# SkyTNT/midi-model

Hardware: AMD Instinct MI355X
Metric: MIDI events/sec, training step (fwd+bwd+clip+AdamW), tv2o-medium, seq=2048 (higher is better)
Workload: dtype bf16; 1 GPU; tv2o-medium bf16 training step, per-GPU batch 16 x 2048 events x 8 tokens (BASELINE.json configs[1]); random-init weights, synthetic events; global_batch=16, seq_len=2048, parallelism=dp1, accumulate_grad_batches=1, optimizer=AdamW bf16-true + global-norm clip 1.0

## Files before the change

### include/midihip.h

```cpp
#ifndef MIDIHIP_H
#define MIDIHIP_H
#include <stdint.h>
#ifdef __cplusplus
extern "C" {
#endif

#define MH_F32 0
#define MH_BF16 1

#define MH_OK 0
#define MH_ERR_ARG (-1)
#define MH_ERR_LAUNCH (-2)
#define MH_ERR_UNSUPPORTED (-3)

const char* mh_last_error(void);
int mh_version(void);
int mh_ab_builds(void);
int mh_set_option(const char* name, int value);
int mh_get_option(const char* name);

int mh_gemm_nt(const void* A, int64_t lda, const void* B, int64_t ldb, void* C, int64_t ldc, const void* R,
               int64_t ldr, int64_t M, int64_t N, int64_t K, float alpha, float beta, int dtype, int splitk,
               void* workspace, void* stream);
int mh_gemm(const void* A, int64_t lda, int transA, const void* B, int64_t ldb, int transB, void* C, int64_t ldc,
            const void* R, int64_t ldr, int64_t M, int64_t N, int64_t K, float alpha, float beta, int dtype, int splitk,
            void* workspace, void* stream);
int mh_gemm_swiglu(const void* A, int64_t lda, const void* W, int64_t ldw, void* GU, int64_t ldgu, void* ACT,
                   int64_t ldact, int64_t M, int64_t I, int64_t K, int dtype, void* stream);
int mh_gemm_rope(const void* A, int64_t lda, const void* W, int64_t ldw, void* C, int64_t ldc, const void* table,
                 int64_t npos, int64_t S, int64_t pos0, int head_dim, int64_t M, int64_t N, int64_t K, int dtype, void* stream);
int mh_gemm_dswiglu(const void* A, int64_t lda, const void* B, int64_t ldb, const void* GU, int64_t ldgu, void* DGU,
                    int64_t lddgu, int64_t M, int64_t I, int64_t K, int dtype, void* stream);
int mh_gemm_rowss(const void* A, int64_t lda, const void* B, int64_t ldb, void* C, int64_t ldc, const void* R, int64_t ldr,
                  float* rowss, int64_t M, int64_t N, int64_t K, int dtype, void* stream);
int mh_row_rstd(const void* x, int64_t ldx, const float* parts, int nparts, int64_t M, int D, float eps, float* rstd, int dtype,
                void* stream);
int mh_gemm_rope_scaled(const void* A, int64_t lda, const void* W, int64_t ldw, void* C, int64_t ldc, const void* table,
                        int64_t npos, int64_t S, int64_t pos0, int head_dim, const float* rowscale, int64_t M, int64_t N, int64_t K,
                        int dtype, void* stream);
int mh_gemm_swiglu_scaled(const void* A, int64_t lda, const void* W, int64_t ldw, void* GU, int64_t ldgu, void* ACT, int64_t ldact,
                          const float* rowscale, int64_t M, int64_t I, int64_t K, int dtype, void* stream);
int mh_gemm_nt_scaled(const void* A, int64_t lda, const void* B, int64_t ldb, void* C, int64_t ldc, const float* rowscale, int64_t M,
                      int64_t N, int64_t K, int dtype, void* stream);
int mh_gemm_dswiglu_scaled(const void* A, int64_t lda, const void* B, int64_t ldb, const void* GU, int64_t ldgu, void* DGU,
                           int64_t lddgu, const float* rowscale, int64_t M, int64_t I, int64_t K, int dtype, void* stream);
int mh_splitk_fold_blocks(int64_t M);
int mh_gemm_splitk_reduce_fold(const void* workspace, void* C, int64_t ldc, const void* R, int64_t ldr, int64_t M, int64_t N,
                               int splitk, float alpha, float beta, const void* wnorm, const void* W, int64_t ldw, float* colpart,
                               int dtype, void* stream);
int mh_rmsnorm_bwd_folded(const void* x, const float* rstd, const void* t, const void* dres, void* dx, int64_t M, int D, int dtype,
                          void* stream);
int mh_scale_cols(const void* W, int64_t ldw, const void* w, void* out, int64_t ldo, int64_t Nr, int K, int dtype, void* stream);
int mh_scale_cols_batched(const int64_t* jobs, int njobs, int K, int dtype, void* stream);
int mh_gemm_splitk_reduce(const void* workspace, void* C, int64_t ldc, const void* R, int64_t ldr, int64_t M,
                          int64_t N, int splitk, float alpha, float beta, int dtype, void* stream);
#define MH_SKINNY_PLAIN 0
#define MH_SKINNY_GATEUP 1
int mh_gemm_skinny(const void* A, int64_t lda, const void* W, int64_t ldw, void* C, int64_t ldc, const void* R,
                   int64_t ldr, int mode, float norm_eps, const int64_t* row_ids, const int64_t* res_ids, int64_t M,
                   int64_t N, int64_t K, int dtype, void* stream);
int mh_transpose(const void* in, int64_t ldi, void* out, int64_t ldo, int64_t rows, int64_t cols, int dtype,
                 void* stream);

int mh_embed_sum_fwd(const int64_t* tok, const void* table, void* out, int64_t M, int T, int64_t V, int D,
                     int dtype, void* stream);
int mh_concat_tok_fwd(const void* hidden, const int64_t* tok, int64_t ldtok, const void* table, void* out,
                      int64_t M, int T, int64_t V, int D, int dtype, void* stream);
int mh_embed_scatter_bwd(const int64_t* tok, int64_t ldtok, int T, const void* dout, int rows_per_m, int jstride,
                         int j0, float* dtable_f32, int64_t M, int64_t V, int D, int64_t pad_id, int dtype,
                         void* stream);
int mh_embed_segment_bwd(const int64_t* src_rows, const int64_t* seg_start, const void* dout, int64_t ld,
                         float* dtable_f32, int64_t V, int D, int64_t n_occ, int64_t pad_id, int dtype, void* stream);
int mh_token_segments_chunk(void);
int mh_token_segments(const int64_t* tok, int64_t ldtok, int64_t n_rows, int n_cols, int64_t V, int64_t row_mul,
                      int64_t col_mul, int64_t add, int64_t* src_rows, int64_t* seg_start, int32_t* work, void* stream);
int mh_cast_from_f32(const float* src, void* dst, int64_t n, int accumulate, int dtype, void* stream);
int mh_copy_rows(const void* src, int64_t src_ld, void* dst, int64_t dst_ld, int64_t M, int D, int accumulate,
                 int dtype, void* stream);

int mh_collate_windows(const int16_t* tokens, int64_t n_events, const int64_t* win_start, const int64_t* win_len,
                       int64_t* out, int64_t B, int64_t L, int T, int64_t pad_id, void* stream);

int mh_augment_piece_stats(const int16_t* tokens, const int64_t* piece_off, int64_t n_pieces, const int32_t* tab,
                           int32_t* stats, void* stream);
int mh_augment_collate_windows(const int16_t* tokens, int64_t n_events, const int64_t* win_start, const int64_t* win_len,
                               const int64_t* win_piece, const int32_t* shifts, const int32_t* stats, const int32_t* tab,
                               int64_t* out, int64_t B, int64_t L, int T, int64_t pad_id, void* stream);

int mh_rmsnorm_fwd(const void* x, const void* w, void* y, float* rstd, int64_t M, int D, float eps, int dtype,
                   void* stream);
int mh_rmsnorm_bwd_blocks(int64_t M);
int mh_rmsnorm_bwd(const void* x, const void* w, const float* rstd, const void* dy, const void* dres, void* dx,
                   float* dw_partial, int64_t M, int D, int dtype, void* stream);
int mh_colsum(float* partial , int64_t nblk, void* out, int D, int accumulate, int dtype, void* stream);

int mh_rope(void* qkv, const float* cos_t, const float* sin_t, int64_t M, int64_t S, int64_t pos0, int H, int hd,
            int dir, int dtype, void* stream);

int mh_attn_prep_fwd(const void* qkv, void* vt, int64_t B, int64_t S, int H, int dtype, void* stream);
int mh_attn_fwd(const void* qkv, const void* vt, void* o, float* lse, int64_t B, int64_t S, int H, float scale,
                int dtype, void* stream);
int mh_attn_prep_bwd(const void* qkv, const void* o, const void* dout, float* delta, void* qt, void* kt, void* dot,
                     int64_t B, int64_t S, int H, int dtype, void* stream);
int mh_attn_bwd(const void* qkv, const void* dout, const float* lse, const float* delta, const void* qt,
                const void* kt, const void* dot, void* dqkv, int64_t B, int64_t S, int H, float scale,
                const float* cos_t, const float* sin_t, int dtype, void* stream);
int mh_attn_bwd_o(const void* qkv, const void* o, const void* dout, const float* lse, float* delta, void* dqkv, int64_t B,
                  int64_t S, int H, float scale, const float* cos_t, const float* sin_t, int dtype, void* stream);
int mh_attn_bwd_o_scaled(const void* qkv, const void* o, const void* dout, const float* lse, float* delta, void* dqkv,
                         const float* rowscale, int64_t B, int64_t S, int H, float scale, const float* cos_t, const float* sin_t,
                         int dtype, void* stream);
int mh_attn_fwd_timeline(const void* qkv, void* o, float* lse, int64_t B, int64_t S, int H, float scale, int lazy,
                         uint32_t* stamps, void* stream);
int mh_attn_fwd_plain(const void* qkv, void* o, float* lse, int64_t B, int64_t S, int H, float scale, int dtype,
                      void* stream);
int mh_attn_bwd_plain(const void* qkv, const void* dout, const float* lse, const float* delta, void* dqkv, int64_t B,
                      int64_t S, int H, float scale, int dtype, void* stream);

int mh_tokattn_fwd(const void* qkv, void* o, int64_t N, int T, int H, float scale, const float* cos_t, const float* sin_t,
                   int dtype, void* stream);
int mh_tokattn_bwd(const void* qkv, const void* dout, void* dqkv, int64_t N, int T, int H, float scale, const float* cos_t,
                   const float* sin_t, int dtype, void* stream);
int mh_tokattn_bwd_scaled(const void* qkv, const void* dout, void* dqkv, const float* rowscale, int64_t N, int T, int H, float scale,
                          const float* cos_t, const float* sin_t, int dtype, void* stream);

int mh_swiglu_fwd(const void* gu, void* a, int64_t M, int I, int dtype, void* stream);
int mh_swiglu_bwd(const void* gu, const void* da, void* dgu, int64_t M, int I, int dtype, void* stream);

int mh_cross_entropy(const void* logits, int64_t ldl, const int64_t* target, float* row_loss, void* dlogits,
                     const float* scale_dev, int64_t* argmax_out, int64_t R, int V, int64_t ignore, int dtype,
                     void* stream);
int mh_sum_f32(const float* x, int64_t n, float* out, void* stream);
int mh_count_valid(const int64_t* target, int64_t n, int64_t ignore, float* count, float* inv, void* stream);

int mh_sumsq(const void* g, int64_t n, float* partial1024, float* out, int accumulate, int dtype, void* stream);
int mh_clip_coef(const float* sumsq, float max_norm, float* coef, float* norm, void* stream);
int mh_adamw(void* p, const void* g, void* m, void* v, int64_t n, float lr, float beta1, float beta2, float eps,
             float weight_decay, float bias_corr1, float bias_corr2, const float* coef_dev, int dtype, void* stream);
int mh_adamw_master(float* p32, void* p_lo, const float* g32, float* m, float* v, int64_t n, float lr, float beta1,
                    float beta2, float eps, float weight_decay, float bias_corr1, float bias_corr2, const float* coef_dev,
                    int dtype_lo, void* stream);
int mh_grad_fold_f32(const void* src, float* dst, int64_t n, int accumulate, int dtype, void* stream);

int mh_kv_append(void* qkv, const float* cos_t, const float* sin_t, void* kcache, void* vcache, int64_t B, int H,
                 int hd, int64_t Lmax, int64_t pos, const int32_t* pos_dev, int dtype, void* stream);
int mh_attn_decode(const void* qkv, const void* kcache, const void* vcache, void* o, int64_t B, int H, int hd,
                   int64_t Lmax, int64_t len, float scale, const int32_t* pos_dev, int dtype, void* stream);
int mh_attn_decode_append(const void* qkv, const float* cos_t, const float* sin_t, void* kcache, void* vcache, void* o,
                          int64_t B, int H, int hd, int64_t Lmax, int64_t pos, float scale, const int32_t* pos_dev,
                          int dtype, void* stream);
#define MH_ATTN_PREFIX_CHUNK 256
int mh_attn_prefix_chunk(void);
int mh_attn_prefix_partial(const void* qkv, const float* cos_t, const float* sin_t, const void* kpre, const void* vpre,
                           float* ws, int64_t ws_floats, int64_t B, int H, int hd, int64_t Pmax, int64_t pre_len, int64_t pos,
                           float scale, const int32_t* pre_len_dev, const int32_t* pos_dev, int dtype, void* stream);
int mh_attn_decode_append_shared(const void* qkv, const float* cos_t, const float* sin_t, void* ksuf, void* vsuf,
                                 const float* ws, int64_t ws_floats, void* o, int64_t B, int H, int hd, int64_t Lsuf,
                                 int64_t Pmax, int64_t pre_len, int64_t pos, float scale, const int32_t* pre_len_dev,
                                 const int32_t* pos_dev, int dtype, void* stream);
int mh_kv_store_rows(const void* qkv, void* kcache, void* vcache, int64_t B, int64_t S, int H, int hd, int64_t Lmax,
                     int64_t pos0, int dtype, void* stream);
int mh_kv_gather_rows(const void* kcache, const void* vcache, void* qkv, int64_t B, int64_t n, int64_t Stot, int H, int hd,
                      int64_t Lmax, int dtype, void* stream);
int mh_attn_fwd_tail(const void* qkv, void* o, float* lse, int64_t B, int64_t S, int H, float scale, int64_t q_start,
                     int dtype, void* stream);
int mh_kv_store_prefill(const void* qkv, void* kcache, void* vcache, int64_t B, int64_t S, int H, int hd,
                        int64_t Lmax, int dtype, void* stream);

int mh_masked_softmax(const void* logits, int64_t ldl, const int32_t* lo, const int32_t* hi,
                      const uint8_t* first_mask, float* probs, int64_t B, int V, float temp, int dtype,
                      void* stream);
int mh_sample_top_p_k(const void* logits, int64_t ldl, const uint8_t* first_mask, const uint8_t* ban_mask, int first_lo,
                      int first_hi,
                      const int32_t* lo_tab, const int32_t* hi_tab, int tab_stride, int max_range, const int64_t* ev,
                      int pos, const float* q, int64_t* out,
                      int64_t out_stride, int64_t* out_b, int64_t* out_c, int64_t B, int V, float temp, float top_p,
                      int top_k, int fill_rest, int64_t fill_id, int dtype, void* stream);
// ... 13 lines not shown
```

### midi-model_amd/csrc/attention_mfma3.hip

```cpp
#include <stdlib.h>

#include "attn_mfma_common.h"

static int attn_env_int(const char* name, int dflt) {
  const char* v = getenv(name);
  return (v && *v) ? atoi(v) : dflt;
}
thread_local int g_attn_v3 = attn_env_int("MH_ATTN_V3", 255);
thread_local int g_attn_passes = attn_env_int("MH_ATTN_PASSES", 5);
thread_local int g_attn_v3_wps = attn_env_int("MH_ATTN_V3_WPS", 0);
thread_local const float* g_attn_bwd_rowscale = nullptr;

__device__ inline bf16x8 ldsv(const char* p) { return *reinterpret_cast<const bf16x8*>(p); }
typedef __attribute__((ext_vector_type(2))) float f32x2;
typedef __attribute__((ext_vector_type(2))) __bf16 bf16x2;
__device__ inline bf16x8 pack8_pk(const f32x16& v, int base) {
  union {
    bf16x8 v;
    bf16x2 h[4];
  } r;
#pragma unroll
  for (int i = 0; i < 4; ++i) r.h[i] = __builtin_convertvector(f32x2{v[base + 2 * i], v[base + 2 * i + 1]}, bf16x2);
  return r.v;
}
__device__ inline float xhalf_max(float v) {
  const int iv = __float_as_int(v);
  const auto pr = __builtin_amdgcn_permlane32_swap(iv, iv, false, false);
  return fmaxf(__int_as_float(pr[0]), __int_as_float(pr[1]));
}

constexpr float LZ_BOUND = 1099511627776.f;
__device__ inline uint64_t tl_now() {
  uint64_t t;
  asm volatile("s_memtime %0" : "=s"(t));
  return t;
}
template <bool MASK, bool TR, bool LZ = false, bool TL = false>
__device__ inline void fwd3_tile(const char* tK, const char* tV, const int (&trof)[2][2], const int (&foff)[4],
                                 const bf16x8 (&qf)[4], f32x16 (&oacc)[2], float& m, float& l, int hi, int qrel, float sc,
                                 uint64_t* ts = nullptr) {
  bf16x8 kf[2][4];
#pragma unroll
  for (int s = 0; s < 4; ++s)
#pragma unroll
    for (int kb = 0; kb < 2; ++kb) kf[kb][s] = ldsv(tK + foff[s] + kb * 4096);
  __builtin_amdgcn_sched_barrier(0);
  if constexpr (TL) ts[2] = tl_now();
  f32x16 sacc[2] = {zero16(), zero16()};
#pragma unroll
  for (int s = 0; s < 4; ++s)
#pragma unroll
    for (int kb = 0; kb < 2; ++kb) sacc[kb] = mfma32(kf[kb][s], qf[s], sacc[kb]);
  bf16x8 vf[4][2];
  u32x2 vr[4][2][2];
  if (TR) {
    unsigned tv[2][2];
#pragma unroll
    for (int db = 0; db < 2; ++db)
#pragma unroll
      for (int half = 0; half < 2; ++half) tv[db][half] = lds_addr32(tV) + (unsigned)trof[db][half];
#pragma unroll
    for (int db = 0; db < 2; ++db)
#pragma unroll
// ... 338 lines not shown
  } else {
#pragma unroll
    for (int t = 0; t < 2; ++t)
#pragma unroll
      for (int hb = 0; hb < 2; ++hb) ktf[t][hb] = ldsv(tKT + foff[2 * KB + t] + hb * 4096);
  }
  __builtin_amdgcn_sched_barrier(0);
#pragma unroll
  for (int r = 0; r < 16; ++r) {
    float p = fast_exp2(__builtin_fmaf(sacc[r], sc, -lse2));
    if (MASK) {
      if (KB * 32 + 16 * (r >> 3) + (r & 7) > qrel - 8 * hi) p = 0.f;
    }
    sacc[r] = p * pacc[r];
  }
  const bf16x8 dsf0 = pack8_pk(sacc, 0), dsf1 = pack8_pk(sacc, 8);
  if (TR) {
    asm volatile("s_waitcnt lgkmcnt(0)" ::: "memory");
    __builtin_amdgcn_sched_barrier(0);
#pragma unroll
    for (int hb = 0; hb < 2; ++hb) dqacc[hb] = mfma32(join8(kr[0][hb][0], kr[0][hb][1]), dsf0, dqacc[hb]);
#pragma unroll
    for (int hb = 0; hb < 2; ++hb) dqacc[hb] = mfma32(join8(kr[1][hb][0], kr[1][hb][1]), dsf1, dqacc[hb]);
  } else {
#pragma unroll
    for (int hb = 0; hb < 2; ++hb) dqacc[hb] = mfma32(ktf[0][hb], dsf0, dqacc[hb]);
#pragma unroll
    for (int hb = 0; hb < 2; ++hb) dqacc[hb] = mfma32(ktf[1][hb], dsf1, dqacc[hb]);
  }
}

template <bool MASK, bool TR>
__device__ inline void dq3_tile(const char* tK, const char* tV, const char* tKT, const int (&trof)[2][2], const int (&foff)[4],
                                const bf16x8 (&qf)[4], const bf16x8 (&dof)[4], f32x16 (&dqacc)[2], int hi, int qrel, float sc,
                                float lse2, const f32x16& dlt) {
  unsigned tkt[2][2];
#pragma unroll
  for (int hb = 0; hb < 2; ++hb)
#pragma unroll
    for (int half = 0; half < 2; ++half) tkt[hb][half] = lds_addr32(tK) + (unsigned)trof[hb][half];
  dq3_half<MASK, TR, 0>(tK, tV, tKT, tkt, foff, qf, dof, dqacc, hi, qrel, sc, lse2, dlt);
  dq3_half<MASK, TR, 1>(tK, tV, tKT, tkt, foff, qf, dof, dqacc, hi, qrel, sc, lse2, dlt);
}

template <int WPS, bool TR>
__global__ __launch_bounds__(256, WPS) void attn_bwd_dq3_kernel(const bf16* __restrict__ qkv, const bf16* __restrict__ dout,
                                                              const float* __restrict__ lse, const float* __restrict__ delta,
                                                              const bf16* __restrict__ kt_, bf16* __restrict__ dqkv, int S,
                                                              int Sp, int H, float scale, int BH, int nqt,
                                                              const float* __restrict__ cos_t,
                                                              const float* __restrict__ sin_t,
                                                              const bf16* __restrict__ o_ ,
                                                              float* __restrict__ delta_w,
                                                              const float* __restrict__ rowscale ) {
  extern __shared__ __attribute__((aligned(16))) char smem[];
  constexpr int NT = TR ? 2 : 3;
  const int tid = threadIdx.x, lane = tid & 63;
  const int wave = __builtin_amdgcn_readfirstlane(tid >> 6);
  int bh_, tile_;
  if (!attn_work(BH, nqt, bh_, tile_)) return;
  const int64_t bh = bh_;
  const int64_t b = bh / H;
  const int h = (int)(bh - b * H);
  const int64_t D = (int64_t)H * HD, D3 = 3 * D;
  const int q0 = (nqt - 1 - tile_) * 128;
  const int qw0 = q0 + wave * 32;
  const int li = lane & 31, hi = lane >> 5;
  const int qrow = qw0 + li;
  const int qld = (qrow < S) ? qrow : S - 1;
  const float sc = scale * LOG2E;

  const bf16* kbase = qkv + b * S * D3 + D + (int64_t)h * HD;
  const bf16* vbase = kbase + D;
  const bf16* ktbase = TR ? nullptr : kt_ + bh * HD * Sp;

  bf16x8 qf[4], dof[4];
  float dl = 0.f;
  {
    const bf16* qp = qkv + (b * S + qld) * D3 + (int64_t)h * HD + 8 * hi;
    const bf16* dp = dout + (b * S + qld) * D + (int64_t)h * HD + 8 * hi;
    bf16x8 of[4];
    if (o_ != nullptr) {
      const bf16* op = o_ + (b * S + qld) * D + (int64_t)h * HD + 8 * hi;
#pragma unroll
      for (int s = 0; s < 4; ++s) of[s] = *reinterpret_cast<const bf16x8*>(op + 16 * s);
    }
#pragma unroll
    for (int s = 0; s < 4; ++s) {
      qf[s] = *reinterpret_cast<const bf16x8*>(qp + 16 * s);
      const bf16x8 d = *reinterpret_cast<const bf16x8*>(dp + 16 * s);
#pragma unroll
      for (int e = 0; e < 8; ++e) dof[s][e] = -d[e];
      if (o_ != nullptr) {
#pragma unroll
        for (int e = 0; e < 8; ++e) dl = __builtin_fmaf((float)d[e], (float)of[s][e], dl);
      }
    }
  }
  float lse2 = lse[bh * Sp + qld] * LOG2E;
  if (o_ != nullptr) {
    dl += __shfl_xor(dl, 32, 64);
    if (hi == 0 && qrow < S) {
      delta_w[bh * Sp + qrow] = dl;
      delta_w[(int64_t)BH * Sp + bh * Sp + qrow] = -lse2;
    }
  } else {
    dl = delta[bh * Sp + qld];
// ... 12 lines not shown
  {
    const int pli = pi32(li);
#pragma unroll
    for (int s = 0; s < 4; ++s) foff[s] = lds_tile_off(pli, 2 * s + hi);
  }

  const int iD3 = (int)D3;
  int trof[2][2];
  tr_frag_offsets(lane, trof);
  stage64u(kbase, iD3, 0, S - 1, 0, smem, wave, lane);
  stage64u(vbase, iD3, 0, S - 1, 0, smem + TILE64, wave, lane);
  if (!TR) stage64u(ktbase, Sp, 0, HD - 1, 0, smem + 2 * TILE64, wave, lane);
#pragma unroll
  for (int s = 0; s < 4; ++s) {
    asm volatile("" : "+v"(qf[s]));
    asm volatile("" : "+v"(dof[s]));
  }
  asm volatile("" : "+v"(lse2));
  asm volatile("" : "+v"(dlt));
  stage_wait_all();
    __syncthreads();
  auto stage_next = [&](int kt) {
    if (kt + 1 <= kt_last) {
      char* nxt = smem + ((kt + 1) & 1) * NT * TILE64;
      stage64u(kbase, iD3, (kt + 1) * 64, S - 1, 0, nxt, wave, lane);
      stage64u(vbase, iD3, (kt + 1) * 64, S - 1, 0, nxt + TILE64, wave, lane);
      if (!TR) stage64u(ktbase, Sp, 0, HD - 1, (kt + 1) * 64, nxt + 2 * TILE64, wave, lane);
    }
  };
  int kt = 0;
  for (; kt < n_full; ++kt) {
    stage_next(kt);
    const char* cur = smem + (kt & 1) * NT * TILE64;
    dq3_tile<false, TR>(cur, cur + TILE64, cur + 2 * TILE64, trof, foff, qf, dof, dqacc, hi, 0, sc, lse2, dlt);
    stage_wait_all();
    __syncthreads();
  }
  if (kt <= kt_last) {
    stage_next(kt);
    const char* cur = smem + (kt & 1) * NT * TILE64;
    dq3_tile<true, TR>(cur, cur + TILE64, cur + 2 * TILE64, trof, foff, qf, dof, dqacc, hi, qrow - kt * 64, sc, lse2, dlt);
    stage_wait_all();
    __syncthreads();
    ++kt;
  }
  for (; kt <= kt_last; ++kt) {
    stage_next(kt);
    stage_wait_all();
    __syncthreads();
  }
  if (qrow < S) {
    bf16* orow = dqkv + (b * S + qrow) * D3 + (int64_t)h * HD;
    const float rsc = rowscale != nullptr ? rowscale[b * S + qrow] : 1.f;
    store_grad_row(orow, dqacc, -scale * rsc, hi, cos_t, sin_t, qrow);
  }
}

template <bool MASK, bool TR, int QB, bool PS>
__device__ inline void dkv3_half(const char* tQ, const char* tDO, const char* tQT, const char* tDOT, const char* tLD,
                                 const unsigned (&tq)[2][2], const unsigned (&tdo)[2][2], const int (&foff)[4],
                                 const bf16x8 (&kf)[4], const bf16x8 (&vf)[4] , f32x16 (&dkacc)[2], f32x16 (&dvacc)[2],
                                 int hi, int krel, int qlim, float sc) {
  bf16x8 qf[4], dof[4];
#pragma unroll
  for (int s = 0; s < 4; ++s) {
    qf[s] = ldsv(tQ + foff[s] + QB * 4096);
    dof[s] = ldsv(tDO + foff[s] + QB * 4096);
  }
  __builtin_amdgcn_sched_barrier(0);
  f32x16 pacc;
#pragma unroll
  for (int i = 0; i < 4; ++i) {
    const f32x4 d4 = *reinterpret_cast<const f32x4*>(tLD + 1024 + (QB * 32 + 16 * (i >> 1) + 8 * hi + 4 * (i & 1)) * 4);
#pragma unroll
    for (int e = 0; e < 4; ++e) pacc[4 * i + e] = d4[e];
  }
  __builtin_amdgcn_sched_barrier(0);
  f32x16 sacc = zero16();
#pragma unroll
  for (int s = 0; s < 4; ++s) {
    sacc = mfma32(qf[s], kf[s], sacc);
    pacc = mfma32(dof[s], vf[s], pacc);
  }
  bf16x8 dotf[2][2], qtf[2][2];
  u32x2 dor[2][2][2], qr[2][2][2];
  f32x4 la[2][2];
#define MH_DKV_REQUEST(T)                                                                      \
  {                                                                                            \
    if (TR) {                                                                                  \
      _Pragma("unroll") for (int xb = 0; xb < 2; ++xb) _Pragma("unroll") for (int half = 0; half < 2; ++half) { \
        dor[T][xb][half] = ds_tr16<(2 * QB + (T)) * 2048>(tdo[xb][half]);                      \
        qr[T][xb][half] = ds_tr16<(2 * QB + (T)) * 2048>(tq[xb][half]);                        \
      }                                                                                        \
    } else {                                                                                   \
      _Pragma("unroll") for (int xb = 0; xb < 2; ++xb) {                                       \
        dotf[T][xb] = ldsv(tDOT + foff[2 * QB + (T)] + xb * 4096);                             \
        qtf[T][xb] = ldsv(tQT + foff[2 * QB + (T)] + xb * 4096);                               \
      }                                                                                        \
    }                                                                                          \
    _Pragma("unroll") for (int v4 = 0; v4 < 2; ++v4)                                           \
        la[T][v4] = *reinterpret_cast<const f32x4*>(tLD + (QB * 32 + 16 * (T) + 8 * hi + 4 * v4) * 4); \
  }
  MH_DKV_REQUEST(0)
  __builtin_amdgcn_sched_barrier(0);
#pragma unroll
  for (int t = 0; t < 2; ++t) {
#pragma unroll
// ... 2 lines not shown
      for (int e = 0; e < 4; ++e) {
        const int r = 8 * t + 4 * v4 + e;
        float p = fast_exp2(__builtin_fmaf(sacc[r], sc, PS ? la[t][v4][e] : -la[t][v4][e] * LOG2E));
        float ds = p * pacc[r];
        if (MASK) {
          const int q = QB * 32 + 16 * t + 4 * v4 + e;
          const bool ok = (q >= krel - 8 * hi) && (q < qlim - 8 * hi);
          p = ok ? p : 0.f;
          ds = ok ? ds : 0.f;
        }
        sacc[r] = p;
        pacc[r] = ds;
      }
    const bf16x8 pf = pack8_pk(sacc, 8 * t), dsf = pack8_pk(pacc, 8 * t);
    if (t == 0) {
      MH_DKV_REQUEST(1)
      if (TR) asm volatile("s_waitcnt lgkmcnt(10)" ::: "memory");
    } else if (TR) {
      asm volatile("s_waitcnt lgkmcnt(0)" ::: "memory");
    }
    __builtin_amdgcn_sched_barrier(0);
#pragma unroll
    for (int xb = 0; xb < 2; ++xb) {
      dvacc[xb] = mfma32(TR ? join8(dor[t][xb][0], dor[t][xb][1]) : dotf[t][xb], pf, dvacc[xb]);
      dkacc[xb] = mfma32(TR ? join8(qr[t][xb][0], qr[t][xb][1]) : qtf[t][xb], dsf, dkacc[xb]);
    }
  }
#undef MH_DKV_REQUEST
}

template <bool MASK, bool TR, bool PS>
__device__ inline void dkv3_tile(const char* tQ, const char* tDO, const char* tQT, const char* tDOT, const char* tLD,
                                 const int (&trof)[2][2], const int (&foff)[4], const bf16x8 (&kf)[4], const bf16x8 (&vf)[4],
                                 f32x16 (&dkacc)[2], f32x16 (&dvacc)[2], int hi, int krel, int qlim, float sc) {
  unsigned tq[2][2], tdo[2][2];
#pragma unroll
  for (int xb = 0; xb < 2; ++xb)
#pragma unroll
    for (int half = 0; half < 2; ++half) {
      tq[xb][half] = lds_addr32(tQ) + (unsigned)trof[xb][half];
      tdo[xb][half] = lds_addr32(tDO) + (unsigned)trof[xb][half];
    }
  dkv3_half<MASK, TR, 0, PS>(tQ, tDO, tQT, tDOT, tLD, tq, tdo, foff, kf, vf, dkacc, dvacc, hi, krel, qlim, sc);
  dkv3_half<MASK, TR, 1, PS>(tQ, tDO, tQT, tDOT, tLD, tq, tdo, foff, kf, vf, dkacc, dvacc, hi, krel, qlim, sc);
}

template <bool TR, bool PS = false >
__global__ __launch_bounds__(256, 2) void attn_bwd_dkv3_kernel(const bf16* __restrict__ qkv, const bf16* __restrict__ dout,
                                                               const float* __restrict__ lse, const float* __restrict__ delta,
                                                               const bf16* __restrict__ qt_, const bf16* __restrict__ dot_,
                                                               bf16* __restrict__ dqkv, int S, int Sp, int H, float scale,
                                                               int BH, int nkt, const float* __restrict__ cos_t,
                                                               const float* __restrict__ sin_t,
                                                               const float* __restrict__ rowscale ) {
  constexpr int NT = TR ? 2 : 4, STG = NT * TILE64 + 2048;
  extern __shared__ __attribute__((aligned(16))) char smem[];
  const int tid = threadIdx.x, lane = tid & 63;
  const int wave = __builtin_amdgcn_readfirstlane(tid >> 6);
  int bh_, tile_;
  if (!attn_work(BH, nkt, bh_, tile_)) return;
  const int64_t bh = bh_;
  const int64_t b = bh / H;
  const int h = (int)(bh - b * H);
  const int64_t D = (int64_t)H * HD, D3 = 3 * D;
  const int k0 = tile_ * 128;
  const int kw0 = k0 + wave * 32;
  const int li = lane & 31, hi = lane >> 5;
  const int krow = kw0 + li;
  const int kld = (krow < S) ? krow : S - 1;
  const float sc = scale * LOG2E;

  const bf16* qbase = qkv + b * S * D3 + (int64_t)h * HD;
  const bf16* dobase = dout + b * S * D + (int64_t)h * HD;
  const bf16* qtbase = TR ? nullptr : qt_ + bh * HD * Sp;
  const bf16* dotbase = TR ? nullptr : dot_ + bh * HD * Sp;
  const float* lse_b = lse + bh * Sp;
  const float* delta_b = delta + bh * Sp;

  bf16x8 kf[4], vf[4];
  {
    const bf16* kp = qkv + (b * S + kld) * D3 + D + (int64_t)h * HD + 8 * hi;
#pragma unroll
    for (int s = 0; s < 4; ++s) {
      kf[s] = *reinterpret_cast<const bf16x8*>(kp + 16 * s);
      const bf16x8 v = *reinterpret_cast<const bf16x8*>(kp + D + 16 * s);
#pragma unroll
      for (int e = 0; e < 8; ++e) vf[s][e] = -v[e];
    }
  }
  f32x16 dkacc[2] = {zero16(), zero16()}, dvacc[2] = {zero16(), zero16()};
  int foff[4];
  {
    const int pli = pi32(li);
#pragma unroll
    for (int s = 0; s < 4; ++s) foff[s] = lds_tile_off(pli, 2 * s + hi);
  }
  const int qt_first = k0 / 64, qt_last = (S - 1) / 64;

  auto stage_all = [&](int qt, char* dst) {
    stage64u(qbase, (int)D3, qt * 64, S - 1, 0, dst, wave, lane);
    stage64u(dobase, (int)D, qt * 64, S - 1, 0, dst + TILE64, wave, lane);
    if (!TR) {
      stage64u(qtbase, Sp, 0, HD - 1, qt * 64, dst + 2 * TILE64, wave, lane);
      stage64u(dotbase, Sp, 0, HD - 1, qt * 64, dst + 3 * TILE64, wave, lane);
    }
    if (wave < 2) {
      const float* base = (wave == 0 ? lse_b : delta_b) + (int64_t)qt * 64;
// ... 3 lines not shown
  int trof[2][2];
  tr_frag_offsets(lane, trof);
  if (qt_first <= qt_last) stage_all(qt_first, smem);
#pragma unroll
  for (int s = 0; s < 4; ++s) {
    asm volatile("" : "+v"(kf[s]));
    asm volatile("" : "+v"(vf[s]));
  }
  stage_wait_all();
    __syncthreads();
  const int nT = qt_last - qt_first + 1;
  const int a = kw0 >> 6;
  int n_skip = a - qt_first;
  if (n_skip > nT) n_skip = nT;
  const int n_mask = (a <= qt_last) ? 1 : 0;
  int n_full = ((S >> 6) < qt_last + 1 ? (S >> 6) : qt_last + 1) - (a + 1);
  if (n_full < 0) n_full = 0;
  const int n_tail = nT - n_skip - n_mask - n_full;
  int qt = qt_first;
  auto head = [&](int q) {
    if (q + 1 <= qt_last) stage_all(q + 1, smem + (((q - qt_first) & 1) ^ 1) * STG);
    return smem + ((q - qt_first) & 1) * STG;
  };
  for (int i = 0; i < n_skip; ++i, ++qt) {
    head(qt);
    stage_wait_all();
    __syncthreads();
  }
  if (n_mask) {
    const char* cur = head(qt);
    dkv3_tile<true, TR, PS>(cur, cur + TILE64, cur + 2 * TILE64, cur + 3 * TILE64, cur + NT * TILE64, trof, foff, kf, vf, dkacc, dvacc, hi,
                    krow - qt * 64, S - qt * 64, sc);
    stage_wait_all();
    __syncthreads();
    ++qt;
  }
  for (int i = 0; i < n_full; ++i, ++qt) {
    const char* cur = head(qt);
    dkv3_tile<false, TR, PS>(cur, cur + TILE64, cur + 2 * TILE64, cur + 3 * TILE64, cur + NT * TILE64, trof, foff, kf, vf, dkacc, dvacc, hi, 0,
                     64, sc);
    stage_wait_all();
    __syncthreads();
  }
  if (n_tail > 0) {
    const char* cur = head(qt);
    dkv3_tile<true, TR, PS>(cur, cur + TILE64, cur + 2 * TILE64, cur + 3 * TILE64, cur + NT * TILE64, trof, foff, kf, vf, dkacc, dvacc, hi,
                    krow - qt * 64, S - qt * 64, sc);
    stage_wait_all();
    __syncthreads();
  }
  if (krow < S) {
    bf16* krow_out = dqkv + (b * S + krow) * D3 + D + (int64_t)h * HD;
    const float rsc = rowscale != nullptr ? rowscale[b * S + krow] : 1.f;
    store_grad_row(krow_out, dkacc, -scale * rsc, hi, cos_t, sin_t, krow);
    store_grad_row(krow_out + D, dvacc, rsc, hi, nullptr, nullptr, 0);
  }
}

int mh_attn_fwd_mfma3(const void* qkv, const void* vt, void* o, float* lse, int64_t B, int64_t S, int H, float scale,
                      hipStream_t st, int64_t q_start) {
  MH_REQUIRE(S * 3 * H * HD < (int64_t(1) << 31), "attn_fwd: sequence too long (32-bit panel offsets)");
  MH_REQUIRE(q_start >= 0 && q_start < S, "attn_fwd: q_start %ld outside the sequence", (long)q_start);
  const int64_t Sp = (S + 63) / 64 * 64;
  const int nt_all = (int)((S + 127) / 128), BH0 = (int)(B * H);
  MH_REQUIRE(BH0 < (1 << 24), "attn_fwd: too many (batch, head) pairs");
  const int BH = BH0 | ((g_attn_passes & 127) << 24);
  const int nt = nt_all - (int)(q_start / 128);
  const unsigned grid = (unsigned)(nt * 8 * ((BH0 + 7) / 8));
#define MH_FWD(WPS, TR_, LZ_)                                                                                                    \
  attn_fwd3_kernel<WPS, TR_, 2, LZ_><<<grid, 256, 4 * TILE64, st>>>((const bf16*)qkv, (const bf16*)vt, (bf16*)o, lse, (int)S, (int)Sp, H, \
                                                                 scale * LOG2E, BH, nt, nt_all)
#define MH_FWD3S(WPS, TR_, LZ_)                                                                                                  \
  attn_fwd3_kernel<WPS, TR_, 3, LZ_><<<grid, 256, 6 * TILE64, st>>>((const bf16*)qkv, (const bf16*)vt, (bf16*)o, lse, (int)S, (int)Sp, \
                                                                  H, scale * LOG2E, BH, nt, nt_all)
  const bool tr = (vt == nullptr);
  const bool lz = (g_attn_v3 & 128) != 0;
  if (tr && g_attn_v3_wps == 4) {
    if (lz) MH_FWD(4, true, true); else MH_FWD(4, true, false);
  } else if (tr && (g_attn_v3 & 64)) {
    if (lz) {
      if (g_attn_v3_wps == 3) MH_FWD3S(3, true, true); else MH_FWD3S(2, true, true);
    } else {
      if (g_attn_v3_wps == 3) MH_FWD3S(3, true, false); else MH_FWD3S(2, true, false);
    }
  } else if (tr) {
    if (g_attn_v3_wps == 3) MH_FWD(3, true, false); else MH_FWD(2, true, false);
  } else {
    if (g_attn_v3_wps == 2) MH_FWD(2, false, false); else MH_FWD(3, false, false);
  }
#undef MH_FWD
#undef MH_FWD3S
  MH_LAUNCH_CHECK();
  return MH_OK;
}

extern "C" int mh_attn_fwd_timeline(const void* qkv, void* o, float* lse, int64_t B, int64_t S, int H, float scale, int lazy,
                                    uint32_t* stamps, void* stream) {
#ifdef MH_AB_BUILDS
  MH_REQUIRE(stamps != nullptr && S >= 128 && S * 3 * H * HD < (int64_t(1) << 31), "attn_fwd_timeline: bad arguments");
  hipStream_t st = (hipStream_t)stream;
  const int64_t Sp = (S + 63) / 64 * 64;
  const int nt_all = (int)((S + 127) / 128), BH0 = (int)(B * H), nt = nt_all;
  const int BH = BH0 | ((g_attn_passes & 127) << 24);
  const unsigned grid = (unsigned)(nt * 8 * ((BH0 + 7) / 8));
  if (lazy)
    attn_fwd3_kernel<2, true, 3, true, true><<<grid, 256, 6 * TILE64 + TL_BYTES, st>>>((const bf16*)qkv, (const bf16*)stamps, (bf16*)o, lse, (int)S,
                                                                                   (int)Sp, H, scale * LOG2E, BH, nt, nt_all);
  else
    attn_fwd3_kernel<2, true, 3, false, true><<<grid, 256, 6 * TILE64 + TL_BYTES, st>>>((const bf16*)qkv, (const bf16*)stamps, (bf16*)o, lse, (int)S,
                                                                                    (int)Sp, H, scale * LOG2E, BH, nt, nt_all);
  MH_LAUNCH_CHECK();
  return MH_OK;
#else
  mh_set_error("attn_fwd_timeline: only in the A/B library (libmidihip_ab.so)");
  return MH_ERR_UNSUPPORTED;
#endif
}

int mh_attn_bwd_mfma3(const void* qkv, const void* dout, const float* lse, const float* delta, const void* qt, const void* kt,
                      const void* dot, void* dqkv, int64_t B, int64_t S, int H, float scale, const float* cos_t,
                      const float* sin_t, int which ,
                      hipStream_t st, const void* o ) {
  MH_REQUIRE(o == nullptr || (which & 14) == 14, "attn_bwd: delta inside the dQ kernel needs the third form of both kernels");
  MH_REQUIRE(S * 3 * H * HD < (int64_t(1) << 31), "attn_bwd: sequence too long (32-bit panel offsets)");
  const bool tr = (which & 8) != 0;
  MH_REQUIRE(tr || (qt != nullptr && kt != nullptr && dot != nullptr), "attn_bwd(bf16): needs the transposed copies (mh_attn_prep_bwd)");
  const int64_t Sp = (S + 63) / 64 * 64;
  const int nt = (int)((S + 127) / 128), BH0 = (int)(B * H);
  MH_REQUIRE(BH0 < (1 << 24), "attn_bwd: too many (batch, head) pairs");
  const int BH = BH0 | ((g_attn_passes & 127) << 24);
  const unsigned grid = (unsigned)(nt * 8 * ((BH0 + 7) / 8));
#define MH_DQ(WPS, TR_)                                                                                                     \
  attn_bwd_dq3_kernel<WPS, TR_><<<grid, 256, (TR_ ? 4 : 6) * TILE64, st>>>((const bf16*)qkv, (const bf16*)dout, lse, delta,     \
                                                                        (const bf16*)kt, (bf16*)dqkv, (int)S, (int)Sp, H, scale, \
                                                                        BH, nt, cos_t, sin_t, (const bf16*)o,         \
                                                                        const_cast<float*>(delta), g_attn_bwd_rowscale)
  if (which & 2) {
    if (g_attn_v3_wps == 2) {
      if (tr) MH_DQ(2, true); else MH_DQ(2, false);
    } else {
      if (tr) MH_DQ(3, true); else MH_DQ(3, false);
    }
    MH_LAUNCH_CHECK();
  }
#undef MH_DQ
  if (which & 4) {
    if (tr && o != nullptr)
      attn_bwd_dkv3_kernel<true, true><<<grid, 256, 2 * (2 * TILE64 + 2048), st>>>((const bf16*)qkv, (const bf16*)dout,
                                                                                 delta + (int64_t)BH0 * Sp, delta, nullptr, nullptr,
                                                                                 (bf16*)dqkv, (int)S, (int)Sp, H, scale, BH, nt,
                                                                                 cos_t, sin_t, g_attn_bwd_rowscale);
    else if (tr)
      attn_bwd_dkv3_kernel<true><<<grid, 256, 2 * (2 * TILE64 + 2048), st>>>((const bf16*)qkv, (const bf16*)dout, lse, delta, nullptr,
                                                                           nullptr, (bf16*)dqkv, (int)S, (int)Sp, H, scale, BH, nt,
                                                                           cos_t, sin_t, g_attn_bwd_rowscale);
    else
      attn_bwd_dkv3_kernel<false><<<grid, 256, 2 * DKV_STAGE, st>>>((const bf16*)qkv, (const bf16*)dout, lse, delta, (const bf16*)qt,
                                                                  (const bf16*)dot, (bf16*)dqkv, (int)S, (int)Sp, H, scale, BH, nt,
                                                                  cos_t, sin_t, g_attn_bwd_rowscale);
    MH_LAUNCH_CHECK();
  }
  return MH_OK;
}
```

### midi-model_amd/csrc/attention_small.hip

```cpp
#include "common.h"

#define DISPATCH_T(dtype, CALL)                                    \
  do {                                                             \
    if ((dtype) == MH_BF16) { using T = bf16; CALL; }              \
    else if ((dtype) == MH_F32) { using T = float; CALL; }         \
    else { mh_set_error("bad dtype %d", (int)(dtype)); return MH_ERR_ARG; } \
  } while (0)

template <typename T> __device__ inline void ld4(const T* p, float (&o)[4]);
template <> __device__ inline void ld4<float>(const float* p, float (&o)[4]) {
  f32x4 v = *reinterpret_cast<const f32x4*>(p);
  o[0] = v[0]; o[1] = v[1]; o[2] = v[2]; o[3] = v[3];
}
template <> __device__ inline void ld4<bf16>(const bf16* p, float (&o)[4]) {
  bf16x4 v = *reinterpret_cast<const bf16x4*>(p);
  o[0] = (float)v[0]; o[1] = (float)v[1]; o[2] = (float)v[2]; o[3] = (float)v[3];
}
template <typename T> __device__ inline void st4(T* p, const float (&o)[4]);
template <> __device__ inline void st4<float>(float* p, const float (&o)[4]) {
  *reinterpret_cast<f32x4*>(p) = f32x4{o[0], o[1], o[2], o[3]};
}
template <> __device__ inline void st4<bf16>(bf16* p, const float (&o)[4]) {
  bf16x4 v;
  v[0] = (bf16)o[0]; v[1] = (bf16)o[1]; v[2] = (bf16)o[2]; v[3] = (bf16)o[3];
// ... 86 lines not shown
      }
#pragma unroll
      for (int t = 0; t < TN; ++t) qraw[t] = ldraw<T>(base + t * D3, lane);
#pragma unroll
      for (int t = 0; t < TN; ++t) {
        unpack(kraw[t], k[t]);
        unpack(vraw[t], v[t]);
        if (rot) rope_row<T>(k[t], rope_c, rope_s, t, lane, 1.f, true);
      }
    } else {
#pragma unroll
      for (int t = 0; t < TK; ++t) {
        if (t < Tn) {
          ldp<T>(base + t * D3 + D, lane, k[t]);
          ldp<T>(base + t * D3 + 2 * D, lane, v[t]);
          if (rot) rope_row<T>(k[t], rope_c, rope_s, t, lane, 1.f, true);
        }
      }
    }
#pragma unroll
    for (int i = 0; i < TK; ++i) {
      if (TN ? i >= TN : i >= Tn) break;
      float q[4];
      if constexpr (TN != 0) unpack(qraw[i], q);
      else ldp<T>(base + i * D3, lane, q);
      if (rot) rope_row<T>(q, rope_c, rope_s, i, lane, 1.f, true);
      float s[TK];
      float mx = -INFINITY;
#pragma unroll
      for (int j = 0; j <= i; ++j) {
        float p = q[0] * k[j][0] + q[1] * k[j][1] + q[2] * k[j][2] + q[3] * k[j][3];
        s[j] = wave_sum_fast(p) * scale;
        mx = fmaxf(mx, s[j]);
      }
      float den = 0.f;
#pragma unroll
      for (int j = 0; j <= i; ++j) {
        s[j] = __expf(s[j] - mx);
        den += s[j];
      }
      const float inv = 1.f / den;
      float acc[4] = {0.f, 0.f, 0.f, 0.f};
#pragma unroll
      for (int j = 0; j <= i; ++j) {
        const float p = s[j] * inv;
#pragma unroll
        for (int e = 0; e < 4; ++e) acc[e] += p * v[j][e];
      }
      stp<T>(o + (n * Tn + i) * D + (int64_t)h * 256, lane, acc);
    }
  }
}

template <typename T, int TN, bool BR>
__global__ __launch_bounds__(256) void tokattn_bwd_kernel(const T* __restrict__ qkv, const T* __restrict__ dout,
                                                          T* __restrict__ dqkv, int64_t NH, int Tn, int H, float scale,
                                                          const float* __restrict__ cos_t, const float* __restrict__ sin_t,
                                                          const float* __restrict__ rowscale ) {
  const int lane = threadIdx.x & 63;
  const int64_t D = (int64_t)H * 256, D3 = 3 * D;
  __shared__ float rope_c[TK * 128], rope_s[TK * 128];
  const bool rot = cos_t != nullptr;
  if (rot) {
    for (int i = threadIdx.x; i < Tn * 128; i += 256) {
      rope_c[i] = rnd<T>(cos_t[i]);
      rope_s[i] = rnd<T>(sin_t[i]);
    }
    __syncthreads();
  }
  for (int64_t w = (int64_t)blockIdx.x * 4 + (threadIdx.x >> 6); w < NH; w += (int64_t)gridDim.x * 4) {
    const int64_t n = w / H;
    const int h = (int)(w - n * H);
    const int64_t off = (int64_t)h * 256;
    const T* base = qkv + n * Tn * D3 + off;
    T* ob = dqkv + n * Tn * D3 + off;
    float k[TK][4], v[TK][4], dk[TK][4], dv[TK][4];
    RawRow<T> qraw[TN ? TN : 1], doraw[TN ? TN : 1];
    const float rs_lane = (rowscale != nullptr && lane < Tn) ? rowscale[n * Tn + lane] : 1.f;
#pragma unroll
    for (int t = 0; t < TK; ++t)
#pragma unroll
      for (int e = 0; e < 4; ++e) dk[t][e] = dv[t][e] = 0.f;
    if constexpr (TN != 0) {
      RawRow<T> kraw[TN ? TN : 1], vraw[TN ? TN : 1];
#pragma unroll
      for (int t = 0; t < TN; ++t) {
        kraw[t] = ldraw<T>(base + t * D3 + D, lane);
        vraw[t] = ldraw<T>(base + t * D3 + 2 * D, lane);
      }
#pragma unroll
      for (int t = 0; t < TN; ++t) {
        qraw[t] = ldraw<T>(base + t * D3, lane);
        doraw[t] = ldraw<T>(dout + (n * Tn + t) * D + off, lane);
      }
#pragma unroll
      for (int t = 0; t < TN; ++t) {
        unpack(kraw[t], k[t]);
        unpack(vraw[t], v[t]);
        if (rot) rope_row<T>(k[t], rope_c, rope_s, t, lane, 1.f, true);
      }
    } else {
#pragma unroll
      for (int t = 0; t < TK; ++t) {
        if (t < Tn) {
          ldp<T>(base + t * D3 + D, lane, k[t]);
          ldp<T>(base + t * D3 + 2 * D, lane, v[t]);
          if (rot) rope_row<T>(k[t], rope_c, rope_s, t, lane, 1.f, true);
        }
      }
    }
#pragma unroll
    for (int i = 0; i < TK; ++i) {
      if (TN ? i >= TN : i >= Tn) break;
      float q[4], dO[4], dq[4] = {0.f, 0.f, 0.f, 0.f};
      if constexpr (TN != 0) {
        unpack(qraw[i], q);
        unpack(doraw[i], dO);
      } else {
        ldp<T>(base + i * D3, lane, q);
        ldp<T>(dout + (n * Tn + i) * D + off, lane, dO);
      }
      if (rot) rope_row<T>(q, rope_c, rope_s, i, lane, 1.f, true);
      float p[TK], dp[TK];
      float mx = -INFINITY;
      if constexpr (BR) {
#pragma unroll
        for (int j = 0; j <= i; j += 2) {
          const bool two = j + 1 <= i;
          const int j1 = two ? j + 1 : j;
          const float a0 = q[0] * k[j][0] + q[1] * k[j][1] + q[2] * k[j][2] + q[3] * k[j][3];
          const float b0 = dO[0] * v[j][0] + dO[1] * v[j][1] + dO[2] * v[j][2] + dO[3] * v[j][3];
          const float a1 = two ? q[0] * k[j1][0] + q[1] * k[j1][1] + q[2] * k[j1][2] + q[3] * k[j1][3] : 0.f;
          const float b1 = two ? dO[0] * v[j1][0] + dO[1] * v[j1][1] + dO[2] * v[j1][2] + dO[3] * v[j1][3] : 0.f;
          const float r4 = wave_sum4(a0, b0, a1, b1);
          p[j] = wave_sum4_get<0>(r4) * scale;
          dp[j] = wave_sum4_get<1>(r4);
          mx = fmaxf(mx, p[j]);
          if (two) {
            p[j1] = wave_sum4_get<2>(r4) * scale;
            dp[j1] = wave_sum4_get<3>(r4);
            mx = fmaxf(mx, p[j1]);
          }
        }
      } else {
#pragma unroll
      for (int j = 0; j <= i; ++j) {
        float a = q[0] * k[j][0] + q[1] * k[j][1] + q[2] * k[j][2] + q[3] * k[j][3];
        float b = dO[0] * v[j][0] + dO[1] * v[j][1] + dO[2] * v[j][2] + dO[3] * v[j][3];
        p[j] = wave_sum_fast(a) * scale;
        dp[j] = wave_sum_fast(b);
        mx = fmaxf(mx, p[j]);
      }
      }
      float den = 0.f;
#pragma unroll
      for (int j = 0; j <= i; ++j) {
        p[j] = __expf(p[j] - mx);
        den += p[j];
      }
      const float inv = 1.f / den;
      float dsum = 0.f;
#pragma unroll
      for (int j = 0; j <= i; ++j) {
        p[j] *= inv;
        dsum += p[j] * dp[j];
      }
#pragma unroll
      for (int j = 0; j <= i; ++j) {
        const float ds = p[j] * (dp[j] - dsum) * scale;
#pragma unroll
        for (int e = 0; e < 4; ++e) {
          dq[e] += ds * k[j][e];
          dk[j][e] += ds * q[e];
          dv[j][e] += p[j] * dO[e];
        }
      }
      if (rot) rope_row<T>(dq, rope_c, rope_s, i, lane, -1.f, false);
      if (rowscale != nullptr) {
        const float rsc = __shfl(rs_lane, i, 64);
#pragma unroll
        for (int e = 0; e < 4; ++e) dq[e] *= rsc;
      }
      stp<T>(ob + i * D3, lane, dq);
    }
#pragma unroll
    for (int t = 0; t < TK; ++t) {
      if (TN ? t < TN : t < Tn) {
        if (rot) rope_row<T>(dk[t], rope_c, rope_s, t, lane, -1.f, false);
        if (rowscale != nullptr) {
          const float rsc = __shfl(rs_lane, t, 64);
#pragma unroll
          for (int e = 0; e < 4; ++e) {
            dk[t][e] *= rsc;
            dv[t][e] *= rsc;
          }
        }
        stp<T>(ob + t * D3 + D, lane, dk[t]);
        stp<T>(ob + t * D3 + 2 * D, lane, dv[t]);
      }
    }
  }
}

extern "C" int mh_tokattn_fwd(const void* qkv, void* o, int64_t N, int Tn, int H, float scale, const float* cos_t,
                              const float* sin_t, int dtype, void* stream) {
  MH_REQUIRE(N > 0 && Tn >= 1 && Tn <= TK && H >= 1, "tokattn_fwd: bad shape N=%ld T=%d H=%d", (long)N, Tn, H);
  const int64_t NH = N * H;
  int64_t g = (NH + 3) / 4;
  if (g > 32768) g = 32768;
  if (Tn == TK)
    DISPATCH_T(dtype, (tokattn_fwd_kernel<T, TK><<<(int)g, 256, 0, (hipStream_t)stream>>>((const T*)qkv, (T*)o, NH, Tn, H, scale,
                                                                                          cos_t, sin_t)));
  else
    DISPATCH_T(dtype, (tokattn_fwd_kernel<T, 0><<<(int)g, 256, 0, (hipStream_t)stream>>>((const T*)qkv, (T*)o, NH, Tn, H, scale,
                                                                                         cos_t, sin_t)));
  MH_LAUNCH_CHECK();
  return MH_OK;
}

thread_local int g_tokattn_bwd_batched = 1;
static int tokattn_bwd_any(const void* qkv, const void* dout, void* dqkv, const float* rowscale, int64_t N, int Tn, int H, float scale,
                           const float* cos_t, const float* sin_t, int dtype, void* stream) {
  MH_REQUIRE(N > 0 && Tn >= 1 && Tn <= TK && H >= 1, "tokattn_bwd: bad shape");
  const int64_t NH = N * H;
  int64_t g = (NH + 3) / 4;
  if (g > 32768) g = 32768;
  if (Tn == TK && g_tokattn_bwd_batched)
    DISPATCH_T(dtype, (tokattn_bwd_kernel<T, TK, true><<<(int)g, 256, 0, (hipStream_t)stream>>>(
                          (const T*)qkv, (const T*)dout, (T*)dqkv, NH, Tn, H, scale, cos_t, sin_t, rowscale)));
  else if (Tn == TK)
    DISPATCH_T(dtype, (tokattn_bwd_kernel<T, TK, false><<<(int)g, 256, 0, (hipStream_t)stream>>>(
                          (const T*)qkv, (const T*)dout, (T*)dqkv, NH, Tn, H, scale, cos_t, sin_t, rowscale)));
  else
    DISPATCH_T(dtype, (tokattn_bwd_kernel<T, 0, false><<<(int)g, 256, 0, (hipStream_t)stream>>>(
                          (const T*)qkv, (const T*)dout, (T*)dqkv, NH, Tn, H, scale, cos_t, sin_t, rowscale)));
  MH_LAUNCH_CHECK();
  return MH_OK;
}
extern "C" int mh_tokattn_bwd(const void* qkv, const void* dout, void* dqkv, int64_t N, int Tn, int H, float scale,
                              const float* cos_t, const float* sin_t, int dtype, void* stream) {
  return tokattn_bwd_any(qkv, dout, dqkv, nullptr, N, Tn, H, scale, cos_t, sin_t, dtype, stream);
}
extern "C" int mh_tokattn_bwd_scaled(const void* qkv, const void* dout, void* dqkv, const float* rowscale, int64_t N, int Tn, int H,
                                     float scale, const float* cos_t, const float* sin_t, int dtype, void* stream) {
  MH_REQUIRE(rowscale != nullptr, "tokattn_bwd_scaled: rowscale is NULL");
  return tokattn_bwd_any(qkv, dout, dqkv, rowscale, N, Tn, H, scale, cos_t, sin_t, dtype, stream);
}

template <typename T>
__global__ __launch_bounds__(256) void kv_append_kernel(T* __restrict__ qkv, const float* __restrict__ cos_t,
                                                        const float* __restrict__ sin_t, T* __restrict__ kc,
                                                        T* __restrict__ vc, int64_t B, int H, int hd, int64_t Lmax,
                                                        int64_t pos, const int32_t* __restrict__ pos_dev) {
  if (pos_dev != nullptr) pos = *pos_dev;
  if (pos >= Lmax) return;
  const int half = hd / 2;
  const int64_t total = B * H * half;
  const int64_t D = (int64_t)H * hd;
  for (int64_t it = (int64_t)blockIdx.x * 256 + threadIdx.x; it < total; it += (int64_t)gridDim.x * 256) {
    const int i = (int)(it % half);
    const int64_t bh = it / half;
    const int h = (int)(bh % H);
    const int64_t b = bh / H;
    const float c = rnd<T>(cos_t[pos * half + i]), s = rnd<T>(sin_t[pos * half + i]);
    T* row = qkv + b * 3 * D + (int64_t)h * hd;
    const float q1 = to_f(row[i]), q2 = to_f(row[i + half]);
    row[i] = from_f<T>(q1 * c - q2 * s);
    row[i + half] = from_f<T>(q2 * c + q1 * s);
    const float k1 = to_f(row[D + i]), k2 = to_f(row[D + i + half]);
    const T kr1 = from_f<T>(k1 * c - k2 * s), kr2 = from_f<T>(k2 * c + k1 * s);
    row[D + i] = kr1;
    row[D + i + half] = kr2;
    T* kd = kc + ((b * H + h) * Lmax + pos) * hd;
    T* vd = vc + ((b * H + h) * Lmax + pos) * hd;
    kd[i] = kr1;
    kd[i + half] = kr2;
    vd[i] = row[2 * D + i];
    vd[i + half] = row[2 * D + i + half];
  }
}

extern "C" int mh_kv_append(void* qkv, const float* cos_t, const float* sin_t, void* kcache, void* vcache, int64_t B,
                            int H, int hd, int64_t Lmax, int64_t pos, const int32_t* pos_dev, int dtype, void* stream) {
  MH_REQUIRE(B > 0 && H > 0 && hd % 2 == 0 && ((pos >= 0 && pos < Lmax) || pos_dev != nullptr),
             "kv_append: bad args (pos=%ld Lmax=%ld)", (long)pos, (long)Lmax);
  const int64_t total = B * H * (hd / 2);
  DISPATCH_T(dtype, (kv_append_kernel<T><<<(int)((total + 255) / 256), 256, 0, (hipStream_t)stream>>>(
                        (T*)qkv, cos_t, sin_t, (T*)kcache, (T*)vcache, B, H, hd, Lmax, pos, pos_dev)));
  MH_LAUNCH_CHECK();
  return MH_OK;
}

template <typename T>
__global__ __launch_bounds__(256) void kv_store_prefill_kernel(const T* __restrict__ qkv, T* __restrict__ kc,
                                                               T* __restrict__ vc, int64_t B, int64_t S, int H, int hd,
                                                               int64_t Lmax, int64_t pos0) {
  constexpr int N = Pack<T>::N;
  const int cph = hd / N;
  const int64_t total = B * S * H * cph;
// ... 651 lines not shown
  return MH_OK;
}

extern "C" int mh_attn_fwd_plain(const void* qkv, void* o, float* lse, int64_t B, int64_t S, int H, float scale,
                                 int dtype, void* stream) {
  MH_REQUIRE(B > 0 && S > 0 && H > 0 && B * H < 65536, "attn_fwd: bad shape");
  DISPATCH_T(dtype, return attn_plain_fwd<T>(qkv, o, lse, B, S, H, scale, (hipStream_t)stream));
}

extern "C" int mh_attn_bwd_plain(const void* qkv, const void* dout, const float* lse, const float* delta, void* dqkv,
                                 int64_t B, int64_t S, int H, float scale, int dtype, void* stream) {
  MH_REQUIRE(B > 0 && S > 0 && H > 0 && B * H < 65536, "attn_bwd: bad shape");
  DISPATCH_T(dtype, return attn_plain_bwd<T>(qkv, dout, lse, delta, dqkv, B, S, H, scale, (hipStream_t)stream));
}

extern "C" int mh_attn_fwd(const void* qkv, const void* vt, void* o, float* lse, int64_t B, int64_t S, int H, float scale,
                           int dtype, void* stream) {
  MH_REQUIRE(B > 0 && S > 0 && H > 0 && B * H < 65536, "attn_fwd: bad shape");
  if (dtype == MH_BF16) return mh_attn_fwd_mfma(qkv, vt, o, lse, B, S, H, scale, (hipStream_t)stream, 0);
  if (dtype == MH_F32) return attn_plain_fwd<float>(qkv, o, lse, B, S, H, scale, (hipStream_t)stream);
  mh_set_error("attn_fwd: bad dtype");
  return MH_ERR_ARG;
}

extern "C" int mh_attn_fwd_tail(const void* qkv, void* o, float* lse, int64_t B, int64_t S, int H, float scale, int64_t q_start,
                                int dtype, void* stream) {
  MH_REQUIRE(B > 0 && S > 0 && H > 0 && B * H < 65536 && q_start >= 0 && q_start < S, "attn_fwd_tail: bad shape");
  if (dtype == MH_BF16) return mh_attn_fwd_mfma(qkv, nullptr, o, lse, B, S, H, scale, (hipStream_t)stream, q_start);
  if (dtype == MH_F32) return attn_plain_fwd<float>(qkv, o, lse, B, S, H, scale, (hipStream_t)stream, q_start);
  mh_set_error("attn_fwd_tail: bad dtype");
  return MH_ERR_ARG;
}

extern "C" int mh_rope(void* qkv, const float* cos_t, const float* sin_t, int64_t M, int64_t S, int64_t pos0, int H, int hd,
                       int dir, int dtype, void* stream);

extern "C" int mh_attn_bwd(const void* qkv, const void* dout, const float* lse, const float* delta, const void* qt,
                           const void* kt, const void* dot, void* dqkv, int64_t B, int64_t S, int H, float scale,
                           const float* cos_t, const float* sin_t, int dtype, void* stream) {
  MH_REQUIRE(B > 0 && S > 0 && H > 0 && B * H < 65536, "attn_bwd: bad shape");
  MH_REQUIRE((cos_t == nullptr) == (sin_t == nullptr), "attn_bwd: cos and sin tables come together");
  if (dtype == MH_BF16)
    return mh_attn_bwd_mfma(qkv, dout, lse, delta, qt, kt, dot, dqkv, B, S, H, scale, cos_t, sin_t, (hipStream_t)stream);
  if (dtype == MH_F32) {
    int rc = attn_plain_bwd<float>(qkv, dout, lse, delta, dqkv, B, S, H, scale, (hipStream_t)stream);
    if (rc == MH_OK && cos_t != nullptr) rc = mh_rope(dqkv, cos_t, sin_t, B * S, S, 0, H, 64, -1, dtype, stream);
    return rc;
  }
  mh_set_error("attn_bwd: bad dtype");
  return MH_ERR_ARG;
}

extern thread_local const float* g_attn_bwd_rowscale;
extern thread_local int g_attn_v3;
extern "C" int mh_attn_bwd_o_scaled(const void* qkv, const void* o, const void* dout, const float* lse, float* delta, void* dqkv,
                                    const float* rowscale, int64_t B, int64_t S, int H, float scale, const float* cos_t,
                                    const float* sin_t, int dtype, void* stream) {
  MH_REQUIRE(rowscale != nullptr, "attn_bwd_o_scaled: rowscale is NULL");
  MH_REQUIRE((g_attn_v3 & 46) == 46, "attn_bwd_o_scaled: needs the third form of the backward kernels (attn_v3 bits 1, 2, 3, 5)");
  g_attn_bwd_rowscale = rowscale;
  const int rc = mh_attn_bwd_o(qkv, o, dout, lse, delta, dqkv, B, S, H, scale, cos_t, sin_t, dtype, stream);
  g_attn_bwd_rowscale = nullptr;
  return rc;
}

extern "C" int mh_attn_bwd_o(const void* qkv, const void* o, const void* dout, const float* lse, float* delta, void* dqkv,
                             int64_t B, int64_t S, int H, float scale, const float* cos_t, const float* sin_t, int dtype,
                             void* stream) {
  MH_REQUIRE(B > 0 && S > 0 && H > 0 && B * H < 65536, "attn_bwd_o: bad shape");
  MH_REQUIRE((cos_t == nullptr) == (sin_t == nullptr), "attn_bwd_o: cos and sin tables come together");
  MH_REQUIRE(dtype == MH_BF16, "attn_bwd_o: bf16 only (fp32: mh_attn_prep_bwd + mh_attn_bwd)");
  return mh_attn_bwd_o_mfma(qkv, o, dout, lse, delta, dqkv, B, S, H, scale, cos_t, sin_t, (hipStream_t)stream);
}
```

### midi-model_amd/csrc/attn_mfma_common.h

```cpp
#pragma once
#include "common.h"

constexpr int HD = 64;
constexpr int TILE64 = 64 * 128;
constexpr int DKV_STAGE = 4 * TILE64 + 2048;
constexpr float LOG2E = 1.4426950408889634f;
constexpr float RESCALE_THR = 4.0f;

__device__ inline f32x16 mfma32(const bf16x8& a, const bf16x8& b, f32x16 c) {
  return __builtin_amdgcn_mfma_f32_32x32x16_bf16(a, b, c, 0, 0, 0);
}
__device__ inline f32x16 zero16() {
  f32x16 z;
#pragma unroll
  for (int i = 0; i < 16; ++i) z[i] = 0.f;
  return z;
}
__device__ inline bf16x8 lds_frag(const char* tile, int row, int chunk) {
  return *reinterpret_cast<const bf16x8*>(tile + lds_tile_off(row, chunk));
}
__device__ inline bf16x8 pack8(const f32x16& v, int base) {
  bf16x8 o;
#pragma unroll
  for (int e = 0; e < 8; ++e) o[e] = (bf16)v[base + e];
// ... 26 lines not shown
}
__device__ inline void stage_wait_all() { asm volatile("s_waitcnt vmcnt(0)" ::: "memory"); }
__device__ inline unsigned lds_u32(const void* p) {
  return (unsigned)(uintptr_t)(__attribute__((address_space(3))) const char*)p;
}
__device__ inline void stage64u(const bf16* __restrict__ base, int ld, int row0, int row_clamp, int col0, char* lds_tile,
                                int wave, int lane) {
  const int rsub = lane >> 3, pc = lane & 7;
  const unsigned lds0 = __builtin_amdgcn_readfirstlane(lds_u32(lds_tile));
#pragma unroll
  for (int it = 0; it < 2; ++it) {
    const int g8 = wave + 4 * it;
    const int r = g8 * 8 + rsub;
    const int c = pc ^ lds_swz(r);
    int grow = row0 + r;
    grow = grow > row_clamp ? row_clamp : grow;
    const unsigned off = (unsigned)(grow * ld + col0 + c * 8) * 2u;
    glds16_s(base, off, lds0 + g8 * 1024);
  }
}

typedef __attribute__((ext_vector_type(2))) unsigned int u32x2;
template <int OFF>
__device__ inline u32x2 ds_tr16(unsigned lds_addr) {
  u32x2 r;
  asm volatile("ds_read_b64_tr_b16 %0, %1 offset:%2" : "=v"(r) : "v"(lds_addr), "i"(OFF));
  return r;
}
__device__ inline unsigned lds_addr32(const char* p) {
  return (unsigned)(uintptr_t)(__attribute__((address_space(3))) const char*)p;
}
__device__ inline bf16x8 join8(const u32x2& a, const u32x2& b) {
  union {
    bf16x8 v;
    u32x2 h[2];
  } u;
  u.h[0] = a;
  u.h[1] = b;
  return u.v;
}

__device__ inline void tr_frag_offsets(int lane, int (&voff)[2][2]) {
  const int p = lane & 15, gb = (lane >> 4) & 1, hi = lane >> 5;
#pragma unroll
  for (int xb = 0; xb < 2; ++xb)
#pragma unroll
    for (int half = 0; half < 2; ++half) {
      const int row = 8 * hi + 4 * half + (p >> 2);
      const int col = xb * 32 + 16 * gb + 8 * (p & 1) + 4 * ((p >> 1) & 1);
      voff[xb][half] = lds_tile_off(row, col >> 3) + (col & 7) * 2;
    }
}

__device__ inline void store_grad_row(bf16* orow, const f32x16 (&acc)[2], float scale, int hi, const float* cos_t,
                                      const float* sin_t, int pos) {
#pragma unroll
  for (int r8 = 0; r8 < 2; ++r8) {
    bf16x8 v0, v1;
#pragma unroll
    for (int e = 0; e < 8; ++e) {
      v0[e] = (bf16)(acc[0][8 * r8 + e] * scale);
      v1[e] = (bf16)(acc[1][8 * r8 + e] * scale);
    }
    if (cos_t != nullptr) {
      const int i0 = 16 * r8 + 8 * hi;
      const f32x4 c0 = *reinterpret_cast<const f32x4*>(cos_t + pos * 32 + i0), c1 = *reinterpret_cast<const f32x4*>(cos_t + pos * 32 + i0 + 4);
      const f32x4 s0 = *reinterpret_cast<const f32x4*>(sin_t + pos * 32 + i0), s1 = *reinterpret_cast<const f32x4*>(sin_t + pos * 32 + i0 + 4);
#pragma unroll
      for (int e = 0; e < 8; ++e) {
        const float c = (float)(bf16)(e < 4 ? c0[e] : c1[e - 4]), sn = -(float)(bf16)(e < 4 ? s0[e] : s1[e - 4]);
        const float x1 = (float)v0[e], x2 = (float)v1[e];
        v0[e] = (bf16)(x1 * c - x2 * sn);
        v1[e] = (bf16)(x2 * c + x1 * sn);
      }
    }
    *reinterpret_cast<bf16x8*>(orow + 16 * r8 + 8 * hi) = v0;
    *reinterpret_cast<bf16x8*>(orow + 32 + 16 * r8 + 8 * hi) = v1;
  }
}

__device__ inline bool attn_work(int& BH, int ntile, int& bh, int& tile) {
  int P = BH >> 24;
  BH &= 0xffffff;
  P = P < 1 ? 1 : (P > ntile ? ntile : P);
  const int lin = blockIdx.x, xcd = lin & 7;
  int i = lin >> 3;
  const int nG = (BH + 7) >> 3;
  int lo = 0, n = ntile;
  for (int p = 0; p < P; ++p) {
    lo = p * ntile / P;
    n = (p + 1) * ntile / P - lo;
    if (i < nG * n) break;
    i -= nG * n;
  }
  const int g = i / n;
  bh = g * 8 + xcd;
  tile = lo + (i - g * n);
  return bh < BH;
}
```

### midi-model_amd/csrc/elementwise.hip

```cpp
#include "common.h"

#define DISPATCH_T(dtype, CALL)                                    \
  do {                                                             \
    if ((dtype) == MH_BF16) { using T = bf16; CALL; }              \
    else if ((dtype) == MH_F32) { using T = float; CALL; }         \
    else { mh_set_error("bad dtype %d", (int)(dtype)); return MH_ERR_ARG; } \
  } while (0)

static inline int grid_for(int64_t items, int per_block, int cap = 1 << 20) {
  int64_t g = (items + per_block - 1) / per_block;
  if (g < 1) g = 1;
  if (g > cap) g = cap;
  return (int)g;
}

template <typename T>
__global__ __launch_bounds__(256) void embed_sum_fwd_kernel(const int64_t* __restrict__ tok, const T* __restrict__ table,
                                                            T* __restrict__ out, int64_t M, int TT, int D, int64_t V) {
  constexpr int N = Pack<T>::N;
  const int lane = threadIdx.x & 63;
  const int64_t wave0 = (int64_t)blockIdx.x * 4 + (threadIdx.x >> 6);
  for (int64_t m = wave0; m < M; m += (int64_t)gridDim.x * 4) {
    constexpr int TMAXI = 8;
    int64_t ids[TMAXI];
// ... 489 lines not shown
  else
    DISPATCH_T(dtype, (rmsnorm_fwd_kernel<T><<<grid_for(M, 4, 65536), 256, 0, (hipStream_t)stream>>>(
                          (const T*)x, (const T*)w, (T*)y, rstd, M, D, eps)));
#undef MH_RMSF
  MH_LAUNCH_CHECK();
  return MH_OK;
}

__global__ __launch_bounds__(256) void rstd_from_parts_kernel(const float* __restrict__ parts, int nparts, int64_t M, float inv_d,
                                                              float eps, float* __restrict__ rstd) {
  __shared__ float acc[4][64];
  const int r = threadIdx.x & 63, q = threadIdx.x >> 6;
  const int64_t m = (int64_t)blockIdx.x * 64 + r;
  float ss = 0.f;
  if (m < M) {
#pragma unroll 4
    for (int p = q; p < nparts; p += 4) ss += parts[(int64_t)p * M + m];
  }
  acc[q][r] = ss;
  __syncthreads();
  if (q == 0 && m < M) rstd[m] = rsqrtf((acc[0][r] + acc[1][r] + acc[2][r] + acc[3][r]) * inv_d + eps);
}
template <typename T>
__global__ __launch_bounds__(256) void row_rstd_kernel(const T* __restrict__ x, int64_t ldx, int64_t M, int D, float eps,
                                                       float* __restrict__ rstd) {
  constexpr int N = Pack<T>::N;
  const int lane = threadIdx.x & 63;
  for (int64_t m = (int64_t)blockIdx.x * 4 + (threadIdx.x >> 6); m < M; m += (int64_t)gridDim.x * 4) {
    const T* xr = x + m * ldx;
    float ss = 0.f;
    for (int c = lane * N; c < D; c += 64 * N) {
      Pack<T> v = ld16(xr + c);
#pragma unroll
      for (int e = 0; e < N; ++e) ss += v.get(e) * v.get(e);
    }
    ss = wave_sum(ss);
    if (lane == 0) rstd[m] = rsqrtf(ss / (float)D + eps);
  }
}
extern "C" int mh_row_rstd(const void* x, int64_t ldx, const float* parts, int nparts, int64_t M, int D, float eps, float* rstd,
                           int dtype, void* stream) {
  MH_REQUIRE(M > 0 && D > 0 && rstd != nullptr && ((x != nullptr) != (parts != nullptr)), "row_rstd: give x OR parts (M=%ld D=%d)", (long)M, D);
  if (parts != nullptr) {
    MH_REQUIRE(nparts > 0 && (int64_t)nparts * 64 == D, "row_rstd: nparts = %d must be D / 64 (D = %d): one sum of squares per 64 columns", nparts, D);
    rstd_from_parts_kernel<<<(unsigned)((M + 63) / 64), 256, 0, (hipStream_t)stream>>>(parts, nparts, M, 1.0f / (float)D, eps, rstd);
  } else {
    MH_REQUIRE(D % 8 == 0 && ldx % 8 == 0 && ldx >= D && ((uintptr_t)x & 15) == 0, "row_rstd: rows must be 16-byte aligned");
    DISPATCH_T(dtype, (row_rstd_kernel<T><<<grid_for(M, 4, 65536), 256, 0, (hipStream_t)stream>>>((const T*)x, ldx, M, D, eps, rstd)));
  }
  MH_LAUNCH_CHECK();
  return MH_OK;
}

constexpr int RMS_BWD_MAX_BLOCKS = 1024;
extern "C" int mh_rmsnorm_bwd_blocks(int64_t M) {
  int64_t g = (M + 3) / 4;
  return (int)(g < RMS_BWD_MAX_BLOCKS ? (g < 1 ? 1 : g) : RMS_BWD_MAX_BLOCKS);
}

template <typename T>
__global__ __launch_bounds__(256) void rmsnorm_bwd_kernel(const T* __restrict__ x, const T* __restrict__ w,
                                                          const float* __restrict__ rstd, const T* __restrict__ dy,
                                                          const T* dres, T* dx, float* __restrict__ dw_partial,
                                                          int64_t M, int D) {
  constexpr int N = Pack<T>::N;
  extern __shared__ __attribute__((aligned(16))) float dw_acc[];
  const int lane = threadIdx.x & 63, wv = threadIdx.x >> 6;
  float* mine = dw_acc + wv * D;
  for (int c = lane; c < D; c += 64) mine[c] = 0.f;
  __syncthreads();
  for (int64_t m = (int64_t)blockIdx.x * 4 + wv; m < M; m += (int64_t)gridDim.x * 4) {
    const T* xr = x + m * D;
    const T* gr = dy + m * D;
    const float r = rstd[m];
    float dot = 0.f;
    for (int c = lane * N; c < D; c += 64 * N) {
      Pack<T> xv = ld16(xr + c), gv = ld16(gr + c), wv_ = ld16(w + c);
#pragma unroll
      for (int e = 0; e < N; ++e) dot += gv.get(e) * wv_.get(e) * (xv.get(e) * r);
    }
    dot = wave_sum(dot) / (float)D;
    for (int c = lane * N; c < D; c += 64 * N) {
      Pack<T> xv = ld16(xr + c), gv = ld16(gr + c), wv_ = ld16(w + c), o;
      Pack<T> rv;
      if (dres != nullptr) rv = ld16(dres + m * D + c);
#pragma unroll
      for (int e = 0; e < N; ++e) {
        const float xh = xv.get(e) * r;
        float d = r * (gv.get(e) * wv_.get(e) - xh * dot);
        if (dres != nullptr) d += rv.get(e);
        o.set(e, d);
        mine[c + e] += gv.get(e) * rnd<T>(xh);
      }
      st16(dx + m * D + c, o);
    }
  }
  __syncthreads();
  for (int c = threadIdx.x; c < D; c += 256)
    dw_partial[(int64_t)blockIdx.x * D + c] = dw_acc[c] + dw_acc[D + c] + dw_acc[2 * D + c] + dw_acc[3 * D + c];
}

template <typename T, int NCH, bool NT>
__global__ __launch_bounds__(256) void rmsnorm_bwd_reg_kernel(const T* __restrict__ x, const T* __restrict__ w,
                                                              const float* __restrict__ rstd, const T* __restrict__ dy,
                                                              const T* dres, T* dx, float* __restrict__ dw_partial,
                                                              int64_t M, int D) {
// ... 388 lines not shown
```

### midi-model_amd/csrc/gemm.hip

```cpp
#include <type_traits>

#include "common.h"

__device__ __attribute__((aligned(16))) char g_zero16[16];

template <typename T> struct Mma;
template <> struct Mma<bf16> {
  __device__ static inline f32x4 run(const Pack<bf16>& a, const Pack<bf16>& b, f32x4 c) {
    return __builtin_amdgcn_mfma_f32_16x16x32_bf16(a.v, b.v, c, 0, 0, 0);
  }
};
template <> struct Mma<float> {
  __device__ static inline f32x4 run(const Pack<float>& a, const Pack<float>& b, f32x4 c) {
#pragma unroll
    for (int e = 0; e < 4; ++e) c = __builtin_amdgcn_mfma_f32_16x16x4f32(a.v[e], b.v[e], c, 0, 0, 0);
    return c;
  }
};

constexpr int BM = 128, BN = 128;
constexpr int TILE_BYTES = 128 * 128;

template <typename T>
__device__ inline void stage_tile(const T* __restrict__ base, int64_t ld, int64_t row0, int64_t nrows, int64_t k0,
// ... 250 lines not shown
}

template <bool FOLD>
__global__ __launch_bounds__(256) void splitk_reduce4_kernel(const float* __restrict__ ws, bf16* __restrict__ C, int64_t ldc,
                                                             const bf16* R, int64_t ldr, int64_t M, int64_t N, int splitk,
                                                             float alpha, float beta, const bf16* __restrict__ wnorm,
                                                             const bf16* __restrict__ W, int64_t ldw, float* __restrict__ colpart);

template <typename T>
static int splitk_reduce_launch(const void* workspace, void* C, int64_t ldc, const void* R, int64_t ldr, int64_t M,
                                int64_t N, int splitk, float alpha, float beta, hipStream_t st) {
  MH_REQUIRE(M > 0 && N > 0 && splitk >= 1 && workspace != nullptr, "splitk_reduce: bad args");
  if constexpr (std::is_same<T, bf16>::value) {
    if (N % 4 == 0 && ldc % 4 == 0 && (R == nullptr || ldr % 4 == 0) && (((uintptr_t)C | (uintptr_t)R) & 7) == 0 &&
        ((uintptr_t)workspace & 15) == 0) {
      const int64_t rows_y = M < 2048 ? M : 2048;
      dim3 grid((unsigned)((N / 4 + 255) / 256), (unsigned)rows_y);
      splitk_reduce4_kernel<false><<<grid, 256, 0, st>>>((const float*)workspace, (bf16*)C, ldc, (const bf16*)R, ldr, M, N, splitk, alpha,
                                                         beta, nullptr, nullptr, 0, nullptr);
      MH_LAUNCH_CHECK();
      return MH_OK;
    }
  }
  const int64_t total = M * N;
  const int blocks = (int)((total + 255) / 256 < 4096 ? (total + 255) / 256 : 4096);
  splitk_reduce_kernel<T><<<blocks, 256, 0, st>>>((const float*)workspace, (T*)C, ldc, (const T*)R, ldr, M, N, splitk,
                                                  alpha, beta);
  MH_LAUNCH_CHECK();
  return MH_OK;
}

extern "C" int mh_gemm_splitk_reduce(const void* workspace, void* C, int64_t ldc, const void* R, int64_t ldr, int64_t M,
                                     int64_t N, int splitk, float alpha, float beta, int dtype, void* stream) {
  hipStream_t st = (hipStream_t)stream;
  if (dtype == MH_BF16) return splitk_reduce_launch<bf16>(workspace, C, ldc, R, ldr, M, N, splitk, alpha, beta, st);
  if (dtype == MH_F32) return splitk_reduce_launch<float>(workspace, C, ldc, R, ldr, M, N, splitk, alpha, beta, st);
  mh_set_error("splitk_reduce: bad dtype %d", dtype);
  return MH_ERR_ARG;
}

extern "C" int mh_gemm(const void* A, int64_t lda, int transA, const void* B, int64_t ldb, int transB, void* C,
                       int64_t ldc, const void* R, int64_t ldr, int64_t M, int64_t N, int64_t K, float alpha, float beta,
                       int dtype, int splitk, void* workspace, void* stream) {
  hipStream_t st = (hipStream_t)stream;
  if (dtype == MH_BF16)
    return gemm_launch<bf16>(A, lda, transA, B, ldb, transB, C, ldc, R, ldr, M, N, K, alpha, beta, splitk, workspace, st);
  if (dtype == MH_F32)
    return gemm_launch<float>(A, lda, transA, B, ldb, transB, C, ldc, R, ldr, M, N, K, alpha, beta, splitk, workspace, st);
  mh_set_error("gemm: bad dtype %d", dtype);
  return MH_ERR_ARG;
}

int mh_gemm_pp256_dswiglu_bf16(const void* A, int64_t lda, const void* B, int64_t ldb, const void* GU, int64_t ldgu,
                               void* DGU, int64_t lddgu, int64_t M, int64_t I, int64_t K, hipStream_t st, const float* rowscale);
int mh_gemm_pp256_scaled_bf16(const void* A, int64_t lda, const void* B, int64_t ldb, void* C, int64_t ldc, int64_t M, int64_t N,
                              int64_t K, const float* rowscale, hipStream_t st);

int mh_gemm_pp256_swiglu_bf16(const void* A, int64_t lda, const void* W, int64_t ldw, void* GU, int64_t ldgu, void* ACT,
                              int64_t ldact, int64_t M, int64_t I, int64_t K, hipStream_t st, const float* rowscale);

static int gemm_swiglu_any(const void* A, int64_t lda, const void* W, int64_t ldw, void* GU, int64_t ldgu, void* ACT,
                           int64_t ldact, const float* rowscale, int64_t M, int64_t I, int64_t K, int dtype, void* stream);

extern "C" int mh_gemm_swiglu(const void* A, int64_t lda, const void* W, int64_t ldw, void* GU, int64_t ldgu, void* ACT,
                              int64_t ldact, int64_t M, int64_t I, int64_t K, int dtype, void* stream) {
  return gemm_swiglu_any(A, lda, W, ldw, GU, ldgu, ACT, ldact, nullptr, M, I, K, dtype, stream);
}
extern "C" int mh_gemm_swiglu_scaled(const void* A, int64_t lda, const void* W, int64_t ldw, void* GU, int64_t ldgu, void* ACT,
                                     int64_t ldact, const float* rowscale, int64_t M, int64_t I, int64_t K, int dtype, void* stream) {
  MH_REQUIRE(rowscale != nullptr && ((uintptr_t)rowscale & 15) == 0, "gemm_swiglu_scaled: rowscale must be a 16-byte aligned fp32 [M]");
  return gemm_swiglu_any(A, lda, W, ldw, GU, ldgu, ACT, ldact, rowscale, M, I, K, dtype, stream);
}

static int gemm_swiglu_any(const void* A, int64_t lda, const void* W, int64_t ldw, void* GU, int64_t ldgu, void* ACT,
                           int64_t ldact, const float* rowscale, int64_t M, int64_t I, int64_t K, int dtype, void* stream) {
  MH_REQUIRE(dtype == MH_BF16 && g_mh_gemm_variant != 0,
             "gemm_swiglu: served by the production bf16 kernel only (use mh_gemm + mh_swiglu_fwd otherwise)");
  MH_REQUIRE(M > 0 && I > 0 && K > 0 && I % 128 == 0, "gemm_swiglu: bad shape M=%ld I=%ld K=%ld (I must be a multiple of 128)",
             (long)M, (long)I, (long)K);
  MH_REQUIRE(lda % 8 == 0 && ldw % 8 == 0 && ldact % 8 == 0 && lda >= K && ldw >= K && ldact >= I &&
                 (GU == nullptr || (ldgu % 8 == 0 && ldgu >= 2 * I)),
             "gemm_swiglu: leading dimensions must be multiples of 8 elements and cover the rows");
  MH_REQUIRE((((uintptr_t)A | (uintptr_t)W | (uintptr_t)GU | (uintptr_t)ACT) & 15) == 0, "gemm_swiglu: 16-byte alignment");
  return mh_gemm_pp256_swiglu_bf16(A, lda, W, ldw, GU, ldgu, ACT, ldact, M, I, K, (hipStream_t)stream, rowscale);
}

int mh_gemm_pp256_rope_bf16(const void* A, int64_t lda, const void* W, int64_t ldw, void* C, int64_t ldc, const void* table,
                            int64_t S, int64_t pos0, int64_t M, int64_t N, int64_t K, hipStream_t st, const float* rowscale);

static int gemm_rope_any(const void* A, int64_t lda, const void* W, int64_t ldw, void* C, int64_t ldc, const void* table,
                         int64_t npos, int64_t S, int64_t pos0, int head_dim, const float* rowscale, int64_t M, int64_t N, int64_t K,
                         int dtype, void* stream);

extern "C" int mh_gemm_rope(const void* A, int64_t lda, const void* W, int64_t ldw, void* C, int64_t ldc, const void* table,
                            int64_t npos, int64_t S, int64_t pos0, int head_dim, int64_t M, int64_t N, int64_t K, int dtype,
                            void* stream) {
  return gemm_rope_any(A, lda, W, ldw, C, ldc, table, npos, S, pos0, head_dim, nullptr, M, N, K, dtype, stream);
}
extern "C" int mh_gemm_rope_scaled(const void* A, int64_t lda, const void* W, int64_t ldw, void* C, int64_t ldc, const void* table,
                                   int64_t npos, int64_t S, int64_t pos0, int head_dim, const float* rowscale, int64_t M, int64_t N,
                                   int64_t K, int dtype, void* stream) {
  MH_REQUIRE(rowscale != nullptr && ((uintptr_t)rowscale & 15) == 0, "gemm_rope_scaled: rowscale must be a 16-byte aligned fp32 [M]");
  return gemm_rope_any(A, lda, W, ldw, C, ldc, table, npos, S, pos0, head_dim, rowscale, M, N, K, dtype, stream);
}

static int gemm_rope_any(const void* A, int64_t lda, const void* W, int64_t ldw, void* C, int64_t ldc, const void* table,
                         int64_t npos, int64_t S, int64_t pos0, int head_dim, const float* rowscale, int64_t M, int64_t N, int64_t K,
                         int dtype, void* stream) {
  MH_REQUIRE(dtype == MH_BF16 && g_mh_gemm_variant != 0,
             "gemm_rope: served by the production bf16 kernel only (use mh_gemm + mh_rope otherwise)");
  MH_REQUIRE(M > 0 && K > 0 && N > 0 && N % 192 == 0 && head_dim == 64,
             "gemm_rope: bad shape M=%ld N=%ld K=%ld head_dim=%d (N = 3 * heads * 64)", (long)M, (long)N, (long)K, head_dim);
  MH_REQUIRE(S > 0 && pos0 >= 0 && pos0 + (S < M ? S : M) <= npos && npos < (int64_t(1) << 31), "gemm_rope: table too short");
  MH_REQUIRE(S < (int64_t(1) << 31), "gemm_rope: S = %ld does not fit the 32 bits it travels in", (long)S);
  MH_REQUIRE(lda % 8 == 0 && ldw % 8 == 0 && ldc % 8 == 0 && lda >= K && ldw >= K && ldc >= N,
             "gemm_rope: leading dimensions must be multiples of 8 elements and cover the rows");
  MH_REQUIRE((((uintptr_t)A | (uintptr_t)W | (uintptr_t)C | (uintptr_t)table) & 15) == 0, "gemm_rope: 16-byte alignment");
  return mh_gemm_pp256_rope_bf16(A, lda, W, ldw, C, ldc, table, S, pos0, M, N, K, (hipStream_t)stream, rowscale);
}

int mh_gemm_pp256_rowss_bf16(const void* A, int64_t lda, const void* B, int64_t ldb, void* C, int64_t ldc, const void* R,
                             int64_t ldr, int64_t M, int64_t N, int64_t K, float* rowss, hipStream_t st);

extern "C" int mh_gemm_rowss(const void* A, int64_t lda, const void* B, int64_t ldb, void* C, int64_t ldc, const void* R,
                             int64_t ldr, float* rowss, int64_t M, int64_t N, int64_t K, int dtype, void* stream) {
  MH_REQUIRE(dtype == MH_BF16 && g_mh_gemm_variant != 0, "gemm_rowss: served by the production bf16 kernel only");
  MH_REQUIRE(M > 0 && N > 0 && K > 0 && N % 64 == 0 && rowss != nullptr, "gemm_rowss: bad shape M=%ld N=%ld K=%ld (N must be a multiple of 64)",
             (long)M, (long)N, (long)K);
  MH_REQUIRE(lda % 8 == 0 && ldb % 8 == 0 && ldc % 8 == 0 && lda >= K && ldb >= K && ldc >= N && (R == nullptr || (ldr % 8 == 0 && ldr >= N)),
             "gemm_rowss: leading dimensions must be multiples of 8 elements and cover the rows");
  MH_REQUIRE((((uintptr_t)A | (uintptr_t)B | (uintptr_t)C | (uintptr_t)R) & 15) == 0, "gemm_rowss: 16-byte alignment");
  MH_REQUIRE(((M + 255) / 256) * ((N + 255) / 256) < (1ll << 30), "gemm_rowss: too many tiles");
  return mh_gemm_pp256_rowss_bf16(A, lda, B, ldb, C, ldc, R, ldr, M, N, K, rowss, (hipStream_t)stream);
}

extern "C" int mh_gemm_dswiglu(const void* A, int64_t lda, const void* B, int64_t ldb, const void* GU, int64_t ldgu,
                               void* DGU, int64_t lddgu, int64_t M, int64_t I, int64_t K, int dtype, void* stream) {
  MH_REQUIRE(dtype == MH_BF16 && g_mh_gemm_variant != 0,
             "gemm_dswiglu: served by the production bf16 kernel only (use mh_gemm + mh_swiglu_bwd otherwise)");
  MH_REQUIRE(M > 0 && I > 0 && K > 0 && I % 8 == 0, "gemm_dswiglu: bad shape M=%ld I=%ld K=%ld", (long)M, (long)I, (long)K);
  MH_REQUIRE(lda % 8 == 0 && ldb % 8 == 0 && ldgu % 8 == 0 && lddgu % 8 == 0 && lda >= K && ldb >= I && ldgu >= 2 * I &&
                 lddgu >= 2 * I,
             "gemm_dswiglu: leading dimensions must be multiples of 8 elements and cover the rows");
  MH_REQUIRE((((uintptr_t)A | (uintptr_t)B | (uintptr_t)GU | (uintptr_t)DGU) & 15) == 0, "gemm_dswiglu: 16-byte alignment");
  return mh_gemm_pp256_dswiglu_bf16(A, lda, B, ldb, GU, ldgu, DGU, lddgu, M, I, K, (hipStream_t)stream, nullptr);
}

extern "C" int mh_gemm_dswiglu_scaled(const void* A, int64_t lda, const void* B, int64_t ldb, const void* GU, int64_t ldgu,
                                      void* DGU, int64_t lddgu, const float* rowscale, int64_t M, int64_t I, int64_t K, int dtype,
                                      void* stream) {
  MH_REQUIRE(dtype == MH_BF16 && g_mh_gemm_variant != 0, "gemm_dswiglu_scaled: served by the production bf16 kernel only");
  MH_REQUIRE(rowscale != nullptr && ((uintptr_t)rowscale & 15) == 0, "gemm_dswiglu_scaled: rowscale must be a 16-byte aligned fp32 [M]");
  MH_REQUIRE(M > 0 && I > 0 && K > 0 && I % 8 == 0, "gemm_dswiglu_scaled: bad shape M=%ld I=%ld K=%ld", (long)M, (long)I, (long)K);
  MH_REQUIRE(lda % 8 == 0 && ldb % 8 == 0 && ldgu % 8 == 0 && lddgu % 8 == 0 && lda >= K && ldb >= I && ldgu >= 2 * I &&
                 lddgu >= 2 * I,
             "gemm_dswiglu_scaled: leading dimensions must be multiples of 8 elements and cover the rows");
  MH_REQUIRE((((uintptr_t)A | (uintptr_t)B | (uintptr_t)GU | (uintptr_t)DGU) & 15) == 0, "gemm_dswiglu_scaled: 16-byte alignment");
  return mh_gemm_pp256_dswiglu_bf16(A, lda, B, ldb, GU, ldgu, DGU, lddgu, M, I, K, (hipStream_t)stream, rowscale);
}

extern "C" int mh_gemm_nt_scaled(const void* A, int64_t lda, const void* B, int64_t ldb, void* C, int64_t ldc,
                                 const float* rowscale, int64_t M, int64_t N, int64_t K, int dtype, void* stream) {
  MH_REQUIRE(dtype == MH_BF16 && g_mh_gemm_variant != 0, "gemm_nt_scaled: served by the production bf16 kernel only");
  MH_REQUIRE(rowscale != nullptr && ((uintptr_t)rowscale & 15) == 0, "gemm_nt_scaled: rowscale must be a 16-byte aligned fp32 [M]");
  MH_REQUIRE(M > 0 && N > 0 && K > 0, "gemm_nt_scaled: empty problem");
  MH_REQUIRE(lda % 8 == 0 && ldb % 8 == 0 && lda >= K && ldb >= K && ldc >= N, "gemm_nt_scaled: leading dimensions");
  MH_REQUIRE((((uintptr_t)A | (uintptr_t)B) & 15) == 0, "gemm_nt_scaled: 16-byte alignment");
  MH_REQUIRE(((M + 255) / 256) * ((N + 255) / 256) < (1ll << 30), "gemm_nt_scaled: too many tiles");
  return mh_gemm_pp256_scaled_bf16(A, lda, B, ldb, C, ldc, M, N, K, rowscale, (hipStream_t)stream);
}

constexpr int SKF_MAX_BLOCKS = 1024;
extern "C" int mh_splitk_fold_blocks(int64_t M) { return (int)(M < SKF_MAX_BLOCKS ? (M < 1 ? 1 : M) : SKF_MAX_BLOCKS); }

template <bool FOLD>
__global__ __launch_bounds__(256) void splitk_reduce4_kernel(const float* __restrict__ ws, bf16* __restrict__ C, int64_t ldc,
                                                             const bf16* R, int64_t ldr, int64_t M, int64_t N, int splitk,
                                                             float alpha, float beta, const bf16* __restrict__ wnorm,
                                                             const bf16* __restrict__ W, int64_t ldw, float* __restrict__ colpart) {
  const int64_t c = ((int64_t)blockIdx.x * 256 + threadIdx.x) * 4;
  if (c >= N) return;
  const int64_t total = M * N;
  float wn[4] = {1.f, 1.f, 1.f, 1.f}, cs[4] = {0.f, 0.f, 0.f, 0.f};
  if constexpr (FOLD) {
    const bf16x4 w4 = *reinterpret_cast<const bf16x4*>(wnorm + c);
#pragma unroll
    for (int e = 0; e < 4; ++e) wn[e] = (float)w4[e];
  }
  const bool use_r = (R != nullptr && beta != 0.f);
  for (int64_t m = blockIdx.y; m < M; m += gridDim.y) {
    f32x4 s = *reinterpret_cast<const f32x4*>(ws + m * N + c);
    if (splitk <= 8) {
      f32x4 p[7];
#pragma unroll
      for (int z = 1; z < 8; ++z)
        if (z < splitk) p[z - 1] = *reinterpret_cast<const f32x4*>(ws + (int64_t)z * total + m * N + c);
#pragma unroll
      for (int z = 1; z < 8; ++z)
        if (z < splitk) {
#pragma unroll
          for (int e = 0; e < 4; ++e) s[e] += p[z - 1][e];
        }
    } else {
      for (int z = 1; z < splitk; ++z) {
        const f32x4 p = *reinterpret_cast<const f32x4*>(ws + (int64_t)z * total + m * N + c);
#pragma unroll
        for (int e = 0; e < 4; ++e) s[e] += p[e];
      }
    }
    float x[4];
#pragma unroll
// ... 100 lines not shown
```

### midi-model_amd/csrc/gemm_pp256.hip

```cpp
#include <limits.h>

#include <type_traits>

#include "common.h"

namespace {

__device__ __attribute__((aligned(16))) char g_zero16[16];

constexpr int QBM = 256, QBN = 256, QBK = 32;
constexpr int OP_BYTES = 256 * 64;
constexpr int STAGE_BYTES = 2 * OP_BYTES;
constexpr int NSTAGE = 4;
constexpr int LDS_BYTES = NSTAGE * STAGE_BYTES;
constexpr int NWAVE = 8;
constexpr int NI = 2;

typedef __attribute__((ext_vector_type(4))) short s16x4_t;

__device__ inline int tswz(int krow) { return (krow & 3) | ((krow >> 1) & 4); }
__device__ inline int xswz(int row) { return (0x1230 >> (((row >> 2) & 3) * 4)) & 3; }

struct StageCtx {
  const bf16* p[NI];
// ... 24 lines not shown
    c.klim[it] = (r < nrows) ? (int)kend - krow : INT_MIN;
  }
}
template <bool TR>
__device__ inline bf16x8 frag(const char* tile, int row0, int fi, int fg) {
  if constexpr (!TR) {
    const int row = row0 + fi;
    return *reinterpret_cast<const bf16x8*>(tile + row * 64 + ((fg ^ xswz(row)) << 4));
  } else {
    typedef __attribute__((ext_vector_type(2))) unsigned int u32x2_t;
    union {
      bf16x8 v;
      u32x2_t h[2];
    } u;
#pragma unroll
    for (int t = 0; t < 2; ++t) {
      const int krow = fg * 8 + t * 4 + (fi >> 2);
      const int off = krow * 512 + (((row0 >> 4) ^ tswz(krow)) << 5) + ((fi & 3) << 3);
      const unsigned addr = (unsigned)(uintptr_t)(__attribute__((address_space(3))) const char*)(tile + off);
      asm volatile("ds_read_b64_tr_b16 %0, %1" : "=v"(u.h[t]) : "v"(addr));
    }
    return u.v;
  }
}

typedef __attribute__((ext_vector_type(4))) unsigned int u32x4;
__device__ inline __amdgpu_buffer_rsrc_t tile_rsrc(const void* base, int64_t bytes) {
  const unsigned n = bytes <= 0 ? 0u : (bytes > 0xfffffff0ll ? 0xfffffff0u : (unsigned)bytes);
  const uint64_t b = (uint64_t)(uintptr_t)base;
  const uint64_t bu = (uint64_t)(unsigned)__builtin_amdgcn_readfirstlane((int)(unsigned)b) |
                      ((uint64_t)(unsigned)__builtin_amdgcn_readfirstlane((int)(unsigned)(b >> 32)) << 32);
  return __builtin_amdgcn_make_buffer_rsrc(reinterpret_cast<void*>((uintptr_t)bu), 0, (unsigned)__builtin_amdgcn_readfirstlane((int)n), 0x00020000);
}
template <int AUX>
__device__ inline void tile_store_(const u32x4& v, __amdgpu_buffer_rsrc_t r, unsigned voff) {
  __builtin_amdgcn_raw_buffer_store_b128(v, r, voff, 0, AUX);
}
#define tile_store(v, r, voff, aux) tile_store_<aux>(v, r, voff)
__device__ inline u32x4 as_u32x4(const bf16x8& v) {
  union {
    bf16x8 b;
    u32x4 u;
  } x;
  x.b = v;
  return x.u;
}
__device__ inline bf16x8 as_bf16x8(const u32x4& v) {
  union {
    bf16x8 b;
    u32x4 u;
  } x;
  x.u = v;
  return x.b;
}

constexpr int P8_REGION = 128 * 128;
constexpr int P8_BUF = 4 * P8_REGION;
constexpr int P8_DBG_BYTES = 8 * 2048;

template <int EPI, int ABL, bool TB>
__device__ __forceinline__ void p8_main_loop(char* smem, const bf16* __restrict__ A, int64_t lda, const bf16* __restrict__ B,
                                             int64_t ldb, int64_t M, int64_t N, int64_t m0, int64_t n0, int64_t kbeg, int64_t kend,
                                             int wave, int lane, const void* __restrict__ zero16, f32x4 (&acc)[4][8]) {
  constexpr bool TL = (ABL & 128) != 0;
  constexpr int LA = 7;
  const int grp = wave >> 2, wn = wave & 3;
  const int fi = lane & 15, fg = lane >> 4;
  const int nt = (kend > kbeg) ? (int)((kend - kbeg + 63) / 64) : 0;
  const int nreg = 4 * nt;

  int tl_n = 0;
  auto stamp = [&]() {
    if constexpr (TL) {
      const uint64_t c = __builtin_readcyclecounter();
      if (lane == 0 && tl_n < 252) *reinterpret_cast<uint64_t*>(smem + 2 * P8_BUF + wave * 2048 + tl_n * 8) = c;
      ++tl_n;
    }
  };
  auto mark = [&](int slot) {
    if constexpr (TL) {
      const uint64_t c = __builtin_readcyclecounter();
      if (lane == 0) *reinterpret_cast<uint64_t*>(smem + 2 * P8_BUF + wave * 2048 + slot * 8) = c;
    }
  };
  mark(252);

  const bf16* pa[2];
  const bf16* pb[2];
  int kla[2][2], klb[2][2];
  const int64_t hoff_a = 64 * lda, hoff_b = TB ? 32 * ldb : (EPI == 2) ? (N / 2) * ldb : 32 * ldb;
#pragma unroll
  for (int it = 0; it < 2; ++it) {
    const int lr = (wave * 2 + it) * 8 + (lane >> 3);
    const int ch = (lane & 7) ^ ((lr >> 1) & 7);
    const int64_t ra = m0 + (lr >> 6) * 128 + (lr & 63);
    pa[it] = A + (ra < M ? ra : 0) * lda + ch * 8;
    kla[0][it] = (ra < M) ? (int)kend - ch * 8 : INT_MIN;
    kla[1][it] = (ra + 64 < M) ? (int)kend - ch * 8 : INT_MIN;
    if constexpr (TB) {
      const int krow = (wave + NWAVE * it) * 2 + (lane >> 5), pc = lane & 31;
      const int lg = (pc >> 1) ^ tswz(krow);
      const int64_t r = n0 + lg * 16 + (pc & 1) * 8;
      pb[it] = B + (int64_t)krow * ldb + (r < N ? r : 0);
      klb[0][it] = (r < N) ? (int)kend - krow : INT_MIN;
      klb[1][it] = (r < N) ? (int)kend - krow - 32 : INT_MIN;
    } else {
// ... 115 lines not shown
  };
  auto wait_next = [&](int q, auto steady) {
    if constexpr (decltype(steady)::value) asm volatile("s_waitcnt vmcnt(8)" ::: "memory");
    else if (q + 1 < 2 * nt) wait_out(issued_after(q) - need(q + 1));
    stamp();
  };
  auto tile_g0 = [&](int t, auto steady) {
#pragma unroll
    for (int p = 0; p < 2; ++p) {
      stamp();
      load_slot(t, p, steady);
      bar();
      stamp();
      mfma_phase(p);
      wait_next(2 * t + p, steady);
      bar();
    }
  };
  auto tile_g1 = [&](int t, auto steady) {
#pragma unroll
    for (int p = 0; p < 2; ++p) {
      stamp();
      if (2 * t + p > 0) mfma_phase(p ^ 1);
      else stamp();
      bar();
      stamp();
      load_slot(t, p, steady);
      wait_next(2 * t + p, steady);
      bar();
    }
  };

#pragma unroll
  for (int s = 0; s < LA; ++s)
    if (s < nreg) issue(s);
  if (nt > 0) wait_out((nreg < LA ? nreg : LA) - need(0));
  bar();
  mark(253);
  const int nsteady = nt > 2 ? nt - 2 : 0;
  if (grp == 0) {
    for (int t = 0; t < nsteady; ++t) tile_g0(t, std::true_type{});
    for (int t = nsteady; t < nt; ++t) tile_g0(t, std::false_type{});
  } else {
    for (int t = 0; t < nsteady; ++t) tile_g1(t, std::true_type{});
    for (int t = nsteady; t < nt; ++t) tile_g1(t, std::false_type{});
    if (nt > 0) mfma_phase(1);
  }
  mark(254);
  if constexpr (TL) {
    asm volatile("s_waitcnt lgkmcnt(0)" ::: "memory");
  }
}

template <bool TA, bool TB, int ABL, int EPI, int ML, int NRM>
__global__ __launch_bounds__(512, 2) void gemm_pp256_kernel(const bf16* __restrict__ A, int64_t lda,
                                                            const bf16* __restrict__ B, int64_t ldb, bf16* C, int64_t ldc,
                                                            const bf16* R, int64_t ldr, int64_t M, int64_t N, int64_t K,
                                                            float alpha, float beta, int tiles_n, int nwg,
                                                            int64_t k_per_split, float* __restrict__ ws,
                                                            const void* __restrict__ zero16, float* aux, int lean_epi) {
  static_assert(NRM == 0 || (ML == 1 && ABL == 0 && !TA && (!TB || (EPI == 1 && NRM == 2))), "the norm forms ride on the K-step-64 loops only");
  static_assert(NRM != 1 || EPI == 0, "sum-of-squares partials come out of the plain epilogue");
  extern __shared__ __attribute__((aligned(16))) char smem[];
  const int tid = threadIdx.x, lane = tid & 63;
  const int wave = __builtin_amdgcn_readfirstlane(tid >> 6);
  const int grp = wave >> 2;
  const int wn = wave & 3;

  const int nitems = nwg * (int)gridDim.z;
  const int lin = blockIdx.x + nwg * (int)blockIdx.z;
  const int q = nitems >> 3, r8 = nitems & 7, xcd = lin & 7;
  const int item = (xcd < r8 ? xcd * (q + 1) : r8 * (q + 1) + (xcd - r8) * q) + (lin >> 3);
  const int zslice = item / nwg;
  int tm, tn;
  gemm_tile_of(item - zslice * nwg, nwg / tiles_n, tiles_n, 4, tm, tn);
  const int64_t m0 = (int64_t)tm * QBM, n0 = (int64_t)tn * (EPI == 2 ? 128 : QBN);

  const int64_t kbeg = (int64_t)zslice * k_per_split;
  const int64_t kend = (kbeg + k_per_split < K) ? kbeg + k_per_split : K;

  f32x4 acc[4][8];
#pragma unroll
  for (int a = 0; a < 4; ++a)
#pragma unroll
    for (int b = 0; b < 8; ++b) acc[a][b] = f32x4{0.f, 0.f, 0.f, 0.f};
  const int fi = lane & 15, fg = lane >> 4;
  auto bar = [&]() {
    __builtin_amdgcn_sched_barrier(0);
    __builtin_amdgcn_s_barrier();
    __builtin_amdgcn_sched_barrier(0);
  };

  if constexpr (ML >= 1) {
    if constexpr (NRM == 2) {
      if (wave == 0) {
        const int64_t r = m0 + lane * 4;
        glds16((r + 4 <= M) ? (const void*)(aux + r) : zero16, smem + LDS_BYTES);
      }
    }
    p8_main_loop<EPI, ABL, TB>(smem, A, lda, B, ldb, M, N, m0, n0, kbeg, kend, wave, lane, zero16, acc);
    if constexpr ((ABL & 128) != 0) {
      __syncthreads();
      if (blockIdx.x == 0 && blockIdx.z == 0)
        for (int i = tid; i < P8_DBG_BYTES / 8; i += 512)
          reinterpret_cast<uint64_t*>(ws)[i] = reinterpret_cast<const uint64_t*>(smem + 2 * P8_BUF)[i];
      __syncthreads();
    }
  } else {
  const int nt = (kend > kbeg) ? (int)((kend - kbeg + QBK - 1) / QBK) : 0;
  StageCtx ca, cb;
  if constexpr (TA) stage_init_t(ca, A, lda, m0, M, kend, wave, lane);
  else stage_init_n(ca, A, lda, m0, M, kend, wave, lane, (ABL & 8) != 0);
  if constexpr (TB) stage_init_t(cb, B, ldb, n0, N, kend, wave, lane);
  else stage_init_n(cb, B, ldb, n0, N, kend, wave, lane, (ABL & 8) != 0, EPI == 2 ? N / 2 - 128 : 0);
  auto issue_one = [&](int t, int j) {
    char* buf = smem + (t & (NSTAGE - 1)) * STAGE_BYTES + (j >> 1) * OP_BYTES + (wave + NWAVE * (j & 1)) * 1024;
    const int k0 = (int)kbeg + t * QBK;
    const StageCtx& c = (j >> 1) ? cb : ca;
    const bool tr = (j >> 1) ? TB : TA;
    const int64_t ld = (j >> 1) ? ldb : lda;
    const bf16* p = c.p[j & 1] + (tr ? (int64_t)k0 * ld : (int64_t)k0);
    const void* src = (k0 < c.klim[j & 1]) ? (const void*)p : zero16;
    glds16(src, buf);
  };
#pragma unroll
  for (int s0 = 0; s0 < 3; ++s0)
    if (s0 < nt) {
#pragma unroll
      for (int j = 0; j < 4; ++j) issue_one(s0, j);
    }

  bf16x8 fx[8], fw[4];
  auto load_frags = [&](int t) {
    const char* tA = smem + (t & (NSTAGE - 1)) * STAGE_BYTES;
    const char* tB = tA + OP_BYTES;
    if ((ABL & 2) && t > 0) return;
#pragma unroll
    for (int f = 0; f < 4; ++f)
      fw[f] = frag<TB>(tB, EPI == 2 ? (f >> 1) * 128 + wn * 32 + (f & 1) * 16 : wn * 64 + f * 16, fi, fg);
#pragma unroll
    for (int f = 0; f < 8; ++f) fx[f] = frag<TA>(tA, grp * 128 + f * 16, fi, fg);
  };
  auto mfma_all = [&](int t) {
    __builtin_amdgcn_s_setprio(1);
#pragma unroll
    for (int fn = 0; fn < 4; ++fn) {
#pragma unroll
// ... 9 lines not shown
  };
  auto load_segment = [&](int t) {
    load_frags(t);
    if (t + 3 < nt && !(ABL & 1)) {
#pragma unroll
      for (int j = 0; j < 4; ++j) issue_one(t + 3, j);
    }
    asm volatile("s_waitcnt lgkmcnt(0)" ::: "memory");
    __builtin_amdgcn_sched_barrier(0);
  };
  constexpr bool MIDBAR = ((ABL & 64) != 0) == (TA || TB);
  if (grp == 0) {
    for (int t = 0; t < nt; ++t) {
      wait_step(t);
      bar();
      load_segment(t);
      if (MIDBAR) bar();
      mfma_all(t);
    }
    bar();
  } else {
    for (int t = 0; t < nt; ++t) {
      wait_step(t);
      bar();
      if (t > 0) mfma_all(t - 1);
      if (MIDBAR) bar();
      load_segment(t);
    }
    bar();
    if (nt > 0) mfma_all(nt - 1);
  }
  }

  float rs[8];
  if constexpr (NRM == 2) {
    const float* rl = reinterpret_cast<const float*>(smem + LDS_BYTES);
#pragma unroll
    for (int fm = 0; fm < 8; ++fm) rs[fm] = rl[grp * 128 + fm * 16 + fi];
  }
  const bool partial = (gridDim.z > 1);
  float* wsz = partial ? ws + (int64_t)zslice * M * N : nullptr;
  if constexpr ((ABL & 32) != 0) {
    if (acc[0][0][0] != 1.2345e38f) return;
  }
  if constexpr (EPI == 1) {
    if (lean_epi && m0 + QBM <= M && n0 + QBN <= N && ldc < (1 << 22) && ldr < (1 << 22)) {
      char* wreg = smem + wave * 16384;
      const int lrow = lane >> 3, c = lane & 7;
      const __amdgpu_buffer_rsrc_t rg = tile_rsrc(R + m0 * ldr + n0 + wn * 64, (255 * ldr + N + 64) * 2);
      const __amdgpu_buffer_rsrc_t rc = tile_rsrc(C + m0 * ldc + n0 + wn * 64, (255 * ldc + N + 64) * 2);
      const unsigned vo_r = (unsigned)(((grp * 128 + lrow) * (int)ldr + c * 8) * 2), so_r = (unsigned)ldr * 16u;
      const unsigned vo_c = (unsigned)(((grp * 128 + lrow) * (int)ldc + c * 8) * 2), so_c = (unsigned)ldc * 16u;
      const unsigned up_off = (unsigned)N * 2u;
      bf16x8 gq[2][8], uq[2][8];
      auto request = [&](int half, int i0) {
#pragma unroll
        for (int i = i0; i < i0 + 4; ++i) {
          gq[half][i] = as_bf16x8(__builtin_amdgcn_raw_buffer_load_b128(rg, vo_r, (unsigned)(half * 8 + i) * so_r, 0));
          uq[half][i] = as_bf16x8(__builtin_amdgcn_raw_buffer_load_b128(rg, vo_r, (unsigned)(half * 8 + i) * so_r + up_off, 0));
        }
      };
      request(0, 0);
      request(0, 4);
#pragma unroll
      for (int half = 0; half < 2; ++half) {
#pragma unroll
        for (int fmh = 0; fmh < 4; ++fmh)
#pragma unroll
          for (int fn = 0; fn < 4; ++fn) {
            const int row = fmh * 16 + fi, ch = fn * 4 + fg;
            f32x4 t4 = acc[fn][half * 4 + fmh];
            if constexpr (NRM == 2) t4 *= rs[half * 4 + fmh];
            *reinterpret_cast<f32x4*>(wreg + row * 256 + ((ch ^ (row & 15)) << 4)) = t4;
          }
#pragma unroll
        for (int i = 0; i < 8; ++i) {
          if (half == 0 && (i == 2 || i == 6)) request(1, i == 2 ? 0 : 4);
          const int row = i * 8 + lrow;
          const f32x4 lo = *reinterpret_cast<const f32x4*>(wreg + row * 256 + (((2 * c) ^ (row & 15)) << 4));
          const f32x4 hi = *reinterpret_cast<const f32x4*>(wreg + row * 256 + (((2 * c + 1) ^ (row & 15)) << 4));
          const float v[8] = {lo[0], lo[1], lo[2], lo[3], hi[0], hi[1], hi[2], hi[3]};
          float dv[8], g[8], u[8], dg[8], du[8];
          expand8_bf16(cvt8_bf16(v), dv);
          expand8_bf16(gq[half][i], g);
          expand8_bf16(uq[half][i], u);
          mh_dswiglu8(dv, g, u, dg, du);
          const unsigned so = (unsigned)(half * 8 + i) * so_c;
          tile_store(as_u32x4(cvt8_bf16(dg)), rc, vo_c + so, 2 );
          tile_store(as_u32x4(cvt8_bf16(du)), rc, vo_c + so + up_off, 2);
        }
      }
      return;
    }
    char* wreg = smem + wave * 16384;
    const int lrow = lane >> 3, c = lane & 7;
    const int64_t n = n0 + wn * 64 + c * 8;
    const bool n_ok = (n + 8 <= N);
    bf16x8 gq[2][8], uq[2][8];
    auto request = [&](int half) {
#pragma unroll
      for (int i = 0; i < 8; ++i) {
        const int64_t m = m0 + grp * 128 + half * 64 + i * 8 + lrow;
        if (m < M && n_ok) {
          gq[half][i] = *reinterpret_cast<const bf16x8*>(R + m * ldr + n);
          uq[half][i] = *reinterpret_cast<const bf16x8*>(R + m * ldr + N + n);
        }
      }
    };
    request(0);
#pragma unroll
    for (int half = 0; half < 2; ++half) {
      const bf16x8 (&gv)[8] = gq[half];
      const bf16x8 (&uv)[8] = uq[half];
#pragma unroll
      for (int fmh = 0; fmh < 4; ++fmh)
#pragma unroll
        for (int fn = 0; fn < 4; ++fn) {
          const int row = fmh * 16 + fi, ch = fn * 4 + fg;
          f32x4 t4 = acc[fn][half * 4 + fmh];
          if constexpr (NRM == 2) t4 *= rs[half * 4 + fmh];
          *reinterpret_cast<f32x4*>(wreg + row * 256 + ((ch ^ (row & 15)) << 4)) = t4;
        }
      if (half == 0) request(1);
#pragma unroll
      for (int i = 0; i < 8; ++i) {
        const int row = i * 8 + lrow;
        const f32x4 lo = *reinterpret_cast<const f32x4*>(wreg + row * 256 + (((2 * c) ^ (row & 15)) << 4));
        const f32x4 hi = *reinterpret_cast<const f32x4*>(wreg + row * 256 + (((2 * c + 1) ^ (row & 15)) << 4));
        const int64_t m = m0 + grp * 128 + half * 64 + row;
        if (m >= M || !n_ok) continue;
        const float v[8] = {lo[0], lo[1], lo[2], lo[3], hi[0], hi[1], hi[2], hi[3]};
        float dv[8], g[8], u[8], dg[8], du[8];
        expand8_bf16(cvt8_bf16(v), dv);
        expand8_bf16(gv[i], g);
        expand8_bf16(uv[i], u);
#pragma unroll
        for (int e = 0; e < 8; ++e) {
          const float sig = mh_sigmoid(g[e]);
          const float silu = g[e] * sig;
          dg[e] = dv[e] * u[e] * (sig * (1.f + g[e] * (1.f - sig)));
          du[e] = dv[e] * silu;
        }
        const bf16x8 og = cvt8_bf16(dg), ou = cvt8_bf16(du);
        __builtin_nontemporal_store(og, reinterpret_cast<bf16x8*>(C + m * ldc + n));
        __builtin_nontemporal_store(ou, reinterpret_cast<bf16x8*>(C + m * ldc + N + n));
      }
    }
    return;
  }
  if constexpr (EPI == 2 && ML == 1) {
    char* wreg = smem + wave * 16384;
    const int64_t I = N >> 1, colw = n0 + wn * 32;
    bf16* act = const_cast<bf16*>(R);
    const int64_t rows_left = (M - m0 < QBM) ? M - m0 : QBM;
    const __amdgpu_buffer_rsrc_t ra = tile_rsrc(act + m0 * ldr + colw, ((rows_left - 1) * ldr + 32) * 2);
    const __amdgpu_buffer_rsrc_t rc = tile_rsrc(C != nullptr ? C + m0 * ldc + colw : nullptr, C != nullptr ? ((rows_left - 1) * ldc + I + 32) * 2 : 0);
    const int r4 = lane >> 2, c4 = lane & 3;
    const unsigned vo_a = (unsigned)(((grp * 128 + r4) * (int)ldr + c4 * 8) * 2), so_a = (unsigned)ldr * 32u;
    const unsigned vo_c = (unsigned)(((grp * 128 + r4) * (int)ldc + c4 * 8) * 2), so_c = (unsigned)ldc * 32u;
    const bool keep = (C != nullptr);
#pragma unroll
    for (int half = 0; half < 2; ++half) {
#pragma unroll
      for (int fmh = 0; fmh < 4; ++fmh) {
        const int fm = half * 4 + fmh;
        float gf[8], uf[8];
#pragma unroll
        for (int e = 0; e < 4; ++e) {
          gf[e] = acc[0][fm][e];
          gf[4 + e] = acc[1][fm][e];
          uf[e] = acc[2][fm][e];
          uf[4 + e] = acc[3][fm][e];
        }
        if constexpr (NRM == 2) {
#pragma unroll
          for (int e = 0; e < 8; ++e) {
            gf[e] *= rs[fm];
            uf[e] *= rs[fm];
          }
        }
        const bf16x8 og = cvt8_bf16(gf), ou = cvt8_bf16(uf);
        float gr[8], ur[8], sv[8], sr[8], av[8];
        expand8_bf16(og, gr);
        expand8_bf16(ou, ur);
        mh_silu8(gr, sv);
        expand8_bf16(cvt8_bf16(sv), sr);
#pragma unroll
        for (int e = 0; e < 8; ++e) av[e] = sr[e] * ur[e];
        const bf16x8 oa = cvt8_bf16(av);
        const int row = fmh * 16 + fi, off = row * 64 + ((fg ^ ((row >> 1) & 3)) << 4);
        *reinterpret_cast<u32x4*>(wreg + off) = as_u32x4(oa);
        if (keep) {
          *reinterpret_cast<u32x4*>(wreg + 4096 + off) = as_u32x4(og);
          *reinterpret_cast<u32x4*>(wreg + 8192 + off) = as_u32x4(ou);
        }
      }
#pragma unroll
      for (int i = 0; i < 4; ++i) {
// ... 140 lines not shown
    bf16x8 cq[2][8], sq[2][8];
    auto request = [&](int half) {
      if (rot) {
#pragma unroll
        for (int i = 0; i < 8; ++i) {
          const int64_t m = m0 + grp * 128 + half * 64 + i * 8 + lrow;
          const int64_t pos = pos0 + (m < M ? m : M - 1) % S_;
          cq[half][i] = *reinterpret_cast<const bf16x8*>(tab + pos * 96 + fo);
          sq[half][i] = *reinterpret_cast<const bf16x8*>(tab + pos * 96 + so);
        }
      }
    };
    request(0);
#pragma unroll
    for (int half = 0; half < 2; ++half) {
      const bf16x8 (&cv)[8] = cq[half];
      const bf16x8 (&sv)[8] = sq[half];
#pragma unroll
      for (int fmh = 0; fmh < 4; ++fmh)
#pragma unroll
        for (int fn = 0; fn < 4; ++fn) {
          const int row = fmh * 16 + fi, ch = fn * 4 + fg;
          f32x4 a4 = acc[fn][half * 4 + fmh];
          if constexpr (NRM == 2) a4 *= rs[half * 4 + fmh];
          const bf16x2 lo = __builtin_convertvector(f32x2{a4[0], a4[1]}, bf16x2), hi2 = __builtin_convertvector(f32x2{a4[2], a4[3]}, bf16x2);
          f32x4 r4;
          r4[0] = (float)lo[0];
          r4[1] = (float)lo[1];
          r4[2] = (float)hi2[0];
          r4[3] = (float)hi2[1];
          *reinterpret_cast<f32x4*>(wreg + row * 256 + ((ch ^ (row & 15)) << 4)) = r4;
        }
      if (half == 0) request(1);
#pragma unroll
      for (int i = 0; i < 8; ++i) {
        const int row = i * 8 + lrow;
        const f32x4 lo = *reinterpret_cast<const f32x4*>(wreg + row * 256 + (((2 * c) ^ (row & 15)) << 4));
        const f32x4 hi = *reinterpret_cast<const f32x4*>(wreg + row * 256 + (((2 * c + 1) ^ (row & 15)) << 4));
        const int64_t m = m0 + grp * 128 + half * 64 + row;
        float v[8] = {lo[0], lo[1], lo[2], lo[3], hi[0], hi[1], hi[2], hi[3]};
        if (rot) {
          const int pc = c ^ 4;
          const f32x4 plo = *reinterpret_cast<const f32x4*>(wreg + row * 256 + (((2 * pc) ^ (row & 15)) << 4));
          const f32x4 phi = *reinterpret_cast<const f32x4*>(wreg + row * 256 + (((2 * pc + 1) ^ (row & 15)) << 4));
          const float pv[8] = {plo[0], plo[1], plo[2], plo[3], phi[0], phi[1], phi[2], phi[3]};
          float cf[8], sf[8];
          expand8_bf16(cv[i], cf);
          expand8_bf16(sv[i], sf);
#pragma unroll
          for (int e = 0; e < 8; ++e) v[e] = __builtin_fmaf(v[e], cf[e], pv[e] * sf[e]);
        }
        if (m >= M || n + 8 > N) continue;
        __builtin_nontemporal_store(cvt8_bf16(v), reinterpret_cast<bf16x8*>(C + m * ldc + n));
      }
    }
    return;
  }
  const bool use_r = (R != nullptr && beta != 0.f);
  const bool line_ok = !partial && (ldc & 7) == 0 && ((uintptr_t)C & 15) == 0 &&
                       (!use_r || ((ldr & 7) == 0 && ((uintptr_t)R & 15) == 0));
  if (lean_epi && line_ok && m0 + QBM <= M && n0 + QBN <= N && ldc < (1 << 22) && ldr < (1 << 22)) {
    char* wreg = smem + wave * 16384;
    const int lrow = lane >> 3, c = lane & 7;
    const __amdgpu_buffer_rsrc_t rc = tile_rsrc(C + m0 * ldc + n0 + wn * 64, (255 * ldc + 64) * 2);
    const __amdgpu_buffer_rsrc_t rr = tile_rsrc(use_r ? R + m0 * ldr + n0 + wn * 64 : nullptr, use_r ? (255 * ldr + 64) * 2 : 0);
    const unsigned vo_c = (unsigned)(((grp * 128 + lrow) * (int)ldc + c * 8) * 2), so_c = (unsigned)ldc * 16u;
    const unsigned vo_r = (unsigned)(((grp * 128 + lrow) * (int)ldr + c * 8) * 2), so_r = (unsigned)ldr * 16u;
    float* auxp = nullptr;
    if constexpr (NRM == 1) auxp = aux + ((n0 + wn * 64) >> 6) * M + m0 + grp * 128 + lrow;
    auto turn = [&](auto with_r) {
    constexpr bool use_r = decltype(with_r)::value;
    bf16x8 rv[2][8];
    if (use_r) {
#pragma unroll
      for (int half = 0; half < 2; ++half)
#pragma unroll
        for (int i = 0; i < 8; ++i)
          rv[half][i] = as_bf16x8(__builtin_amdgcn_raw_buffer_load_b128(rr, vo_r, (unsigned)(half * 8 + i) * so_r, 0));
    }
#pragma unroll
    for (int half = 0; half < 2; ++half) {
#pragma unroll
      for (int fmh = 0; fmh < 4; ++fmh)
#pragma unroll
        for (int fn = 0; fn < 4; ++fn) {
          const int row = fmh * 16 + fi, ch = fn * 4 + fg;
          f32x4 t4 = acc[fn][half * 4 + fmh];
          if constexpr (NRM == 2) t4 *= rs[half * 4 + fmh];
          *reinterpret_cast<f32x4*>(wreg + row * 256 + ((ch ^ (row & 15)) << 4)) = t4;
        }
#pragma unroll
      for (int i = 0; i < 8; ++i) {
        const int row = i * 8 + lrow;
        const f32x4 lo = *reinterpret_cast<const f32x4*>(wreg + row * 256 + (((2 * c) ^ (row & 15)) << 4));
        const f32x4 hi = *reinterpret_cast<const f32x4*>(wreg + row * 256 + (((2 * c + 1) ^ (row & 15)) << 4));
        float v[8] = {lo[0], lo[1], lo[2], lo[3], hi[0], hi[1], hi[2], hi[3]};
        if (use_r) {
#pragma unroll
          for (int e = 0; e < 8; ++e) v[e] = alpha * v[e] + beta * (float)rv[half][i][e];
        } else {
#pragma unroll
          for (int e = 0; e < 8; ++e) v[e] = alpha * v[e];
        }
        bf16x8 o;
#pragma unroll
        for (int e = 0; e < 8; ++e) o[e] = (bf16)v[e];
// ... 89 lines not shown
      }
    }
    return;
  }
  const bool vec_ok = partial ? ((N & 3) == 0)
                              : ((ldc & 3) == 0 && ((uintptr_t)C & 15) == 0 &&
                                 (R == nullptr || ((ldr & 3) == 0 && ((uintptr_t)R & 15) == 0)));
#pragma unroll
  for (int fm = 0; fm < 8; ++fm) {
    const int64_t m = m0 + grp * 128 + fm * 16 + fi;
    if (m >= M) continue;
#pragma unroll
    for (int fn = 0; fn < 4; ++fn) {
      const int64_t n = n0 + wn * 64 + fn * 16 + fg * 4;
      if (n >= N) continue;
      f32x4 v = acc[fn][fm];
      if constexpr (NRM == 2) v *= rs[fm];
      if (partial) {
        float* dst = wsz + m * N + n;
        if (vec_ok && n + 3 < N) {
          *reinterpret_cast<f32x4*>(dst) = v;
        } else {
          for (int e = 0; e < 4 && n + e < N; ++e) dst[e] = v[e];
        }
        continue;
      }
      if (vec_ok && n + 3 < N) {
        if (R != nullptr && beta != 0.f) {
          bf16x4 rv = *reinterpret_cast<const bf16x4*>(R + m * ldr + n);
#pragma unroll
          for (int e = 0; e < 4; ++e) v[e] = alpha * v[e] + beta * (float)rv[e];
        } else {
#pragma unroll
          for (int e = 0; e < 4; ++e) v[e] = alpha * v[e];
        }
        bf16x4 o;
#pragma unroll
        for (int e = 0; e < 4; ++e) o[e] = (bf16)v[e];
        *reinterpret_cast<bf16x4*>(C + m * ldc + n) = o;
      } else {
        for (int e = 0; e < 4 && n + e < N; ++e) {
          float x = alpha * v[e];
          if (R != nullptr && beta != 0.f) x += beta * (float)R[m * ldr + n + e];
          C[m * ldc + n + e] = (bf16)x;
        }
      }
    }
  }
}

}
extern thread_local int g_mh_gemm_lean_epi;
namespace {
template <bool TA, bool TB, int ABL, int EPI = 0, int ML = 0, int NRM = 0>
int launch_one(const void* A, int64_t lda, const void* B, int64_t ldb, void* C, int64_t ldc, const void* R, int64_t ldr,
               int64_t M, int64_t N, int64_t K, float alpha, float beta, int splitk, void* workspace, hipStream_t st,
               float* aux = nullptr) {
  constexpr int LDSB = LDS_BYTES + ((ABL & 128) ? P8_DBG_BYTES : 0) + (NRM == 2 ? 1024 : 0);
  constexpr int MAX_DEV = 64;
  static void* zero16_of[MAX_DEV] = {};
  static bool attr_set_of[MAX_DEV] = {};
  int dev = 0;
  if (hipGetDevice(&dev) != hipSuccess || dev < 0 || dev >= MAX_DEV) {
    mh_set_error("gemm_pp256: no current device (or ordinal %d beyond %d)", dev, MAX_DEV - 1);
    return MH_ERR_LAUNCH;
  }
  void* zero16 = __atomic_load_n(&zero16_of[dev], __ATOMIC_ACQUIRE);
  if (zero16 == nullptr) {
    if (hipGetSymbolAddress(&zero16, HIP_SYMBOL(g_zero16)) != hipSuccess) {
      mh_set_error("gemm_pp256: hipGetSymbolAddress(g_zero16) failed");
      return MH_ERR_LAUNCH;
    }
    __atomic_store_n(&zero16_of[dev], zero16, __ATOMIC_RELEASE);
  }
  if (!__atomic_load_n(&attr_set_of[dev], __ATOMIC_ACQUIRE)) {
    hipError_t e = hipFuncSetAttribute(reinterpret_cast<const void*>(&gemm_pp256_kernel<TA, TB, ABL, EPI, ML, NRM>),
                                       hipFuncAttributeMaxDynamicSharedMemorySize, LDSB);
    if (e != hipSuccess) {
      mh_set_error("gemm_pp256: cannot raise dynamic LDS to %d bytes: %s", LDSB, hipGetErrorString(e));
      return MH_ERR_LAUNCH;
    }
    __atomic_store_n(&attr_set_of[dev], true, __ATOMIC_RELEASE);
  }
  const int64_t tiles_m = (M + QBM - 1) / QBM, tiles_n = (EPI == 2) ? N / 256 : (N + QBN - 1) / QBN;
  const int nwg = (int)(tiles_m * tiles_n);
  constexpr int KSTEP = (ML == 1) ? 64 : QBK;
  const int64_t kps = ((K + splitk - 1) / splitk + KSTEP - 1) / KSTEP * KSTEP;
  dim3 grid(nwg, 1, splitk);
  gemm_pp256_kernel<TA, TB, ABL, EPI, ML, NRM><<<grid, 512, LDSB, st>>>((const bf16*)A, lda, (const bf16*)B, ldb, (bf16*)C, ldc,
                                                          (const bf16*)R, ldr, M, N, K, alpha, beta, (int)tiles_n, nwg, kps,
                                                          (float*)workspace, zero16, aux, g_mh_gemm_lean_epi);
  MH_LAUNCH_CHECK();
  return MH_OK;
}

}

extern thread_local int g_mh_gemm_ablate;
extern thread_local int g_mh_gemm_k64;

int mh_gemm_pp256_bf16(const void* A, int64_t lda, int ta, const void* B, int64_t ldb, int tb, void* C, int64_t ldc,
                       const void* R, int64_t ldr, int64_t M, int64_t N, int64_t K, float alpha, float beta, int splitk,
                       void* workspace, hipStream_t st) {
#define MH_PP(TA_, TB_, ABL_) \
  return launch_one<TA_, TB_, ABL_>(A, lda, B, ldb, C, ldc, R, ldr, M, N, K, alpha, beta, splitk, workspace, st)
#ifndef MH_AB_BUILDS
  MH_REQUIRE(g_mh_gemm_ablate == 0, "gemm: option gemm_ablate = %d selects a micro-benchmark build, which is only in the A/B test "
             "library (libmidihip_ab.so)", g_mh_gemm_ablate);
#else
  MH_REQUIRE(g_mh_gemm_ablate != 128 || (workspace != nullptr && splitk == 1), "gemm_ablate 128 (timeline) needs a workspace and splitk 1");
  MH_REQUIRE(!(g_mh_gemm_k64 && !ta && !tb) || g_mh_gemm_ablate == 0 || g_mh_gemm_ablate == 1 || g_mh_gemm_ablate == 4 ||
                 g_mh_gemm_ablate == 128 || g_mh_gemm_ablate == 64,
             "gemm_ablate %d is not built for the K-step-64 main loop (set gemm_k64 = 0 for the K-step-32 ablations)", g_mh_gemm_ablate);
  if (ta == tb && g_mh_gemm_ablate && !(g_mh_gemm_k64 && !ta)) {
#define MH_AB(X_) \
  case X_:        \
    if (ta) MH_PP(true, true, X_); \
    MH_PP(false, false, X_);
    switch (g_mh_gemm_ablate) { MH_AB(1) MH_AB(3) MH_AB(4) MH_AB(5) MH_AB(8) MH_AB(12) MH_AB(32) default: break; }
#undef MH_AB
  }
  if (g_mh_gemm_ablate == 64) {
    if (ta && tb) MH_PP(true, true, 64);
    if (ta) MH_PP(true, false, 64);
    if (tb) MH_PP(false, true, 64);
    MH_PP(false, false, 64);
  }
#endif
  if (ta && tb) MH_PP(true, true, 0);
  if (ta) MH_PP(true, false, 0);
  if (tb && g_mh_gemm_k64 == 1)
    return launch_one<false, true, 0, 0, 1>(A, lda, B, ldb, C, ldc, R, ldr, M, N, K, alpha, beta, splitk, workspace, st);
  if (tb) MH_PP(false, true, 0);
  if (g_mh_gemm_k64) {
#define MH_P8(ABL_) \
  return launch_one<false, false, ABL_, 0, 1>(A, lda, B, ldb, C, ldc, R, ldr, M, N, K, alpha, beta, splitk, workspace, st)
#ifdef MH_AB_BUILDS
    switch (g_mh_gemm_ablate) {
      case 1: MH_P8(1);
      case 4: MH_P8(4);
      case 128: MH_P8(128);
      default: break;
    }
#endif
    MH_P8(0);
#undef MH_P8
  }
  MH_PP(false, false, 0);
#undef MH_PP
}

int mh_gemm_pp256_swiglu_bf16(const void* A, int64_t lda, const void* W, int64_t ldw, void* GU, int64_t ldgu, void* ACT,
                              int64_t ldact, int64_t M, int64_t I, int64_t K, hipStream_t st, const float* rowscale) {
  MH_REQUIRE(ldgu < (1 << 22) && ldact < (1 << 22), "gemm_swiglu: row strides beyond 2^22 elements are not supported (32-bit tile offsets)");
  if (rowscale != nullptr) {
    MH_REQUIRE(g_mh_gemm_k64 != 0 && M % 4 == 0, "gemm_swiglu: the row-scaled form needs the K-step-64 main loop and M %% 4 == 0");
    return launch_one<false, false, 0, 2, 1, 2>(A, lda, W, ldw, GU, ldgu, ACT, ldact, M, 2 * I, K, 1.f, 0.f, 1, nullptr, st,
                                                const_cast<float*>(rowscale));
  }
  if (g_mh_gemm_k64) return launch_one<false, false, 0, 2, 1>(A, lda, W, ldw, GU, ldgu, ACT, ldact, M, 2 * I, K, 1.f, 0.f, 1, nullptr, st);
  return launch_one<false, false, 0, 2>(A, lda, W, ldw, GU, ldgu, ACT, ldact, M, 2 * I, K, 1.f, 0.f, 1, nullptr, st);
}

int mh_gemm_pp256_rope_bf16(const void* A, int64_t lda, const void* W, int64_t ldw, void* C, int64_t ldc, const void* table,
                            int64_t S, int64_t pos0, int64_t M, int64_t N, int64_t K, hipStream_t st, const float* rowscale) {
  MH_REQUIRE(ldc < (1 << 22) && M < (int64_t(1) << 31) - 256, "gemm_rope: row stride beyond 2^22 elements / more than 2^31 rows are not supported (32-bit tile offsets and positions)");
  if (rowscale != nullptr) {
    MH_REQUIRE(g_mh_gemm_k64 != 0 && M % 4 == 0, "gemm_rope: the row-scaled form needs the K-step-64 main loop and M %% 4 == 0");
    return launch_one<false, false, 0, 3, 1, 2>(A, lda, W, ldw, C, ldc, table, S | (pos0 << 32), M, N, K, 1.f, 0.f, 1, nullptr, st,
                                                const_cast<float*>(rowscale));
  }
  if (g_mh_gemm_k64) return launch_one<false, false, 0, 3, 1>(A, lda, W, ldw, C, ldc, table, S | (pos0 << 32), M, N, K, 1.f, 0.f, 1, nullptr, st);
  return launch_one<false, false, 0, 3>(A, lda, W, ldw, C, ldc, table, S | (pos0 << 32), M, N, K, 1.f, 0.f, 1, nullptr, st);
}

int mh_gemm_pp256_scaled_bf16(const void* A, int64_t lda, const void* B, int64_t ldb, void* C, int64_t ldc, int64_t M, int64_t N,
                              int64_t K, const float* rowscale, hipStream_t st) {
  MH_REQUIRE(g_mh_gemm_k64 != 0 && M % 4 == 0, "gemm_nt_scaled: needs the K-step-64 main loop and M %% 4 == 0");
  return launch_one<false, false, 0, 0, 1, 2>(A, lda, B, ldb, C, ldc, nullptr, 0, M, N, K, 1.f, 0.f, 1, nullptr, st,
                                              const_cast<float*>(rowscale));
}

int mh_gemm_pp256_dswiglu_bf16(const void* A, int64_t lda, const void* B, int64_t ldb, const void* GU, int64_t ldgu,
                               void* DGU, int64_t lddgu, int64_t M, int64_t I, int64_t K, hipStream_t st, const float* rowscale) {
  if (rowscale != nullptr) {
    MH_REQUIRE(g_mh_gemm_k64 == 1 && M % 4 == 0, "gemm_dswiglu_scaled: needs the K-step-64 dgrad loop and M %% 4 == 0");
    return launch_one<false, true, 0, 1, 1, 2>(A, lda, B, ldb, DGU, lddgu, GU, ldgu, M, I, K, 1.f, 0.f, 1, nullptr, st,
                                               const_cast<float*>(rowscale));
  }
  if (g_mh_gemm_k64 == 1) return launch_one<false, true, 0, 1, 1>(A, lda, B, ldb, DGU, lddgu, GU, ldgu, M, I, K, 1.f, 0.f, 1, nullptr, st);
  return launch_one<false, true, 0, 1>(A, lda, B, ldb, DGU, lddgu, GU, ldgu, M, I, K, 1.f, 0.f, 1, nullptr, st);
}

int mh_gemm_pp256_rowss_bf16(const void* A, int64_t lda, const void* B, int64_t ldb, void* C, int64_t ldc, const void* R,
                             int64_t ldr, int64_t M, int64_t N, int64_t K, float* rowss, hipStream_t st) {
  MH_REQUIRE(g_mh_gemm_k64 != 0, "gemm_rowss: needs the K-step-64 main loop (option gemm_k64)");
  return launch_one<false, false, 0, 0, 1, 1>(A, lda, B, ldb, C, ldc, R, ldr, M, N, K, 1.f, R ? 1.f : 0.f, 1, nullptr, st, rowss);
}
```

### midi-model_amd/engine.py

```python
from __future__ import annotations

import math
from dataclasses import dataclass, field
from typing import Callable, List, NamedTuple, Optional

import os

import torch

from . import ops


@dataclass
class StackSpec:
    name: str
    D: int
    H: int
    I: int
    L: int
    eps: float
    theta: float
    kind: str

    @property
    def hd(self) -> int:
        return self.D // self.H

    @property
    def scale(self) -> float:
        return self.hd ** -0.5


@dataclass
class LayerTensors:
    wqkv: torch.Tensor = None
    wo: torch.Tensor = None
    wgu: torch.Tensor = None
    wd: torch.Tensor = None
    n1: torch.Tensor = None
    n2: torch.Tensor = None


@dataclass
class StackTensors:
    embed: torch.Tensor = None
    layers: List[LayerTensors] = field(default_factory=list)
    norm: torch.Tensor = None


class RopeTable:

    def __init__(self, hd: int, theta: float, device, npos: int = 0):
        self.hd, self.theta, self.device = hd, theta, device
        self.cos = self.sin = None
        self._fused = None
        self.n = 0
        if npos:
            self.ensure(npos)

    def ensure(self, npos: int):
        if npos <= self.n:
            return
        npos = max(npos, 2 * self.n, 64)
# ... 164 lines not shown

def runs_folded(spec: StackSpec, x: torch.Tensor, save: bool, kv_out: Optional[list], fold_kept: bool) -> bool:
    if save:
        return fold_kept and kv_out is None and train_fold_ok(spec, x)
    return (spec.kind == "event" and x.shape[0] >= (FOLD_MIN_ROWS_PREFOLDED if fold_kept else FOLD_MIN_ROWS_ON_THE_FLY)
            and ops.norm_fold_ok(x, spec.D, spec.hd, spec.I))


def layer_backward(spec: StackSpec, lw: LayerTensors, lg: LayerTensors, keep: LayerSaved, dx: torch.Tensor, nseq: int, slen: int,
                   rope: RopeTable, accumulate: bool) -> torch.Tensor:
    M, D = dx.shape
    H, I = spec.H, spec.I
    a = keep.a
    if a is None:
        a = _empty((M, I), dx)
        ops.swiglu_fwd(keep.gu, a)
    dgu = _empty((M, 2 * I), dx)
    if ops.dswiglu_ok(dx, I):
        ops.gemm_dswiglu(dx, lw.wd, keep.gu, dgu)
    else:
        da = _empty((M, I), dx)
        ops.gemm_nt(dx, lw.wd, da, tb=True)
        ops.swiglu_bwd(keep.gu, da, dgu)
        del da
    linear_wgrad(dx, a, lg.wd, accumulate)
    del a
    dh2 = _empty((M, D), dx)
    ops.gemm_nt(dgu, lw.wgu, dh2, tb=True)
    linear_wgrad(dgu, keep.h2, lg.wgu, accumulate)
    del dgu
    dx2 = _empty((M, D), dx)
    ops.rmsnorm_bwd(keep.x2, lw.n2, keep.rstd2, dh2, dx, dx2, lg.n2, accumulate)
    do = dh2
    ops.gemm_nt(dx2, lw.wo, do, tb=True)
    linear_wgrad(dx2, keep.o, lg.wo, accumulate)
    dqkv = _empty((M, 3 * D), dx)
    if spec.kind == "event":
        ops.attn_bwd(keep.qkv, keep.o, do, keep.lse, dqkv, nseq, slen, H, spec.scale, rope.cos, rope.sin)
    else:
        ops.tokattn_bwd(keep.qkv, do, dqkv, nseq, slen, H, spec.scale, rope.cos, rope.sin)
    dh1 = do
    ops.gemm_nt(dqkv, lw.wqkv, dh1, tb=True)
    linear_wgrad(dqkv, keep.h1, lg.wqkv, accumulate)
    del dqkv
    ops.rmsnorm_bwd(keep.x, lw.n1, keep.rstd1, dh1, dx2, dx, lg.n1, accumulate)
    return dx


def layer_backward_folded(spec: StackSpec, lw: LayerTensors, lg: LayerTensors, fold, keep: LayerSaved, dx: torch.Tensor, nseq: int,
                          slen: int, rope: RopeTable, accumulate: bool) -> torch.Tensor:
    M, D = dx.shape
    H, I = spec.H, spec.I
    wq_n, wgu_n = fold
    a = keep.a
    if a is None:
        a = _empty((M, I), dx)
        ops.swiglu_fwd(keep.gu, a)
    dz2 = _empty((M, 2 * I), dx)
    ops.gemm_dswiglu(dx, lw.wd, keep.gu, dz2, rowscale=keep.rstd2)
    linear_wgrad(dx, a, lg.wd, accumulate)
    del a
    t2 = _empty((M, D), dx)
    ops.gemm_nt(dz2, wgu_n, t2, tb=True)
    ops.wgrad_folded(dz2, keep.x2, lg.wgu, lw.n2, lw.wgu, lg.n2, accumulate)
    del dz2
    dx2 = _empty((M, D), dx)
    ops.rmsnorm_bwd_folded(keep.x2, keep.rstd2, t2, dx, dx2)
    do = t2
    ops.gemm_nt(dx2, lw.wo, do, tb=True)
    linear_wgrad(dx2, keep.o, lg.wo, accumulate)
    dz1 = _empty((M, 3 * D), dx)
    if spec.kind == "event":
        ops.attn_bwd(keep.qkv, keep.o, do, keep.lse, dz1, nseq, slen, H, spec.scale, rope.cos, rope.sin, rowscale=keep.rstd1)
    else:
        ops.tokattn_bwd(keep.qkv, do, dz1, nseq, slen, H, spec.scale, rope.cos, rope.sin, rowscale=keep.rstd1)
    t1 = do
    ops.gemm_nt(dz1, wq_n, t1, tb=True)
    ops.wgrad_folded(dz1, keep.x, lg.wqkv, lw.n1, lw.wqkv, lg.n1, accumulate)
    del dz1
    ops.rmsnorm_bwd_folded(keep.x, keep.rstd1, t1, dx2, dx)
    return dx


def stack_forward(spec: StackSpec, W: StackTensors, x: torch.Tensor, nseq: int, slen: int, rope: RopeTable,
                  save: bool, kv_out: Optional[list] = None, lean: bool = False, folded=None):
    _check_heads(spec)
    M, D = x.shape
    assert M == nseq * slen
    rope.ensure(slen)
    if runs_folded(spec, x, save, kv_out, folded is not None):
        if folded is None:
            folded = fold_norm_weights(W)
    else:
        folded = None
    saved = [] if save else None
    parts = None
    for li, lw in enumerate(W.layers):
        if folded is not None:
            x, parts = layer_forward_folded(spec, lw, folded[li], x, nseq, slen, rope, parts, kv_out, saved, lean)
        else:
            x, keep = layer_forward(spec, lw, x, nseq, slen, rope, kv_out, save, lean and save)
            if save:
                saved.append(keep)
    y = _empty((M, D), x)
    rstdf = _empty((M,), x, torch.float32) if save or folded is None else None
    ops.rmsnorm_fwd(x, W.norm, y, rstdf, spec.eps)
    return y, (StackSaved(saved, x, rstdf, nseq, slen, folded) if save else None)


def stack_backward(spec: StackSpec, W: StackTensors, G: StackTensors, ctx: StackSaved, dy: torch.Tensor,
                   rope: RopeTable, accumulate: bool, on_layer_done: Optional[Callable[[int], None]] = None):
    M, D = dy.shape
    dx = _empty((M, D), dy)
    ops.rmsnorm_bwd(ctx.x_last, W.norm, ctx.rstdf, dy, None, dx, G.norm, accumulate)
    for li in range(len(W.layers) - 1, -1, -1):
        lw, lg = W.layers[li], G.layers[li]
        if ctx.folded is not None:
            dx = layer_backward_folded(spec, lw, lg, ctx.folded[li], ctx.layers[li], dx, ctx.nseq, ctx.slen, rope, accumulate)
        else:
            dx = layer_backward(spec, lw, lg, ctx.layers[li], dx, ctx.nseq, ctx.slen, rope, accumulate)
        ctx.layers[li] = None
        if on_layer_done is not None:
            on_layer_done(li)
    return dx


class KVState:

    def __init__(self, spec: StackSpec, B: int, capacity: int, like: torch.Tensor):
        self.spec, self.B, self.cap, self.len = spec, B, capacity, 0
        shape = (spec.L, B, spec.H, capacity, spec.hd)
        self.k = torch.empty(shape, dtype=like.dtype, device=like.device)
        self.v = torch.empty(shape, dtype=like.dtype, device=like.device)
# ... 168 lines not shown
```

Before: 359,500 events/s.

## Fuse RMSNorm backward into dgrad GEMM epilogue using row-dot partials

The producer kernels for each folded layer (the dswiglu GEMM and the attention/token-attention backward) now also emit per-row partial dot products of the gradient with the pre-norm activations. A small coef kernel reduces those partials into a per-row coefficient. A new GEMM epilogue then computes dx = rstd*(t - coef*x) + dres directly, which removes the separate rmsnorm_bwd_folded passes and the t intermediate tensor. The cost is extra epilogue work, small partial buffers, an extra launch per norm, and a somewhat different accumulation order for the row dot.

```diff
diff --git a/include/midihip.h b/include/midihip.h
--- a/include/midihip.h
+++ b/include/midihip.h
@@ -50,6 +50,13 @@
                                int dtype, void* stream);
 int mh_rmsnorm_bwd_folded(const void* x, const float* rstd, const void* t, const void* dres, void* dx, int64_t M, int D, int dtype,
                           void* stream);
+int mh_gemm_dswiglu_scaled_dots(const void* A, int64_t lda, const void* B, int64_t ldb, const void* GU, int64_t ldgu, void* DGU,
+                                int64_t lddgu, const float* rowscale, float* dots, int64_t M, int64_t I, int64_t K, int dtype,
+                                void* stream);
+int mh_norm_coef(const float* dots, int nslots, const float* rstd, int64_t M, int D, float* coef, void* stream);
+int mh_gemm_normbwd(const void* dz, int64_t lddz, const void* W, int64_t ldw, const void* x, int64_t ldx, const void* dres,
+                    int64_t lddres, const float* coef, void* dx, int64_t lddx, int64_t M, int64_t N, int64_t K, int dtype,
+                    void* stream);
 int mh_scale_cols(const void* W, int64_t ldw, const void* w, void* out, int64_t ldo, int64_t Nr, int K, int dtype, void* stream);
 int mh_scale_cols_batched(const int64_t* jobs, int njobs, int K, int dtype, void* stream);
 int mh_gemm_splitk_reduce(const void* workspace, void* C, int64_t ldc, const void* R, int64_t ldr, int64_t M,
@@ -110,6 +117,9 @@
 int mh_attn_bwd_o_scaled(const void* qkv, const void* o, const void* dout, const float* lse, float* delta, void* dqkv,
                          const float* rowscale, int64_t B, int64_t S, int H, float scale, const float* cos_t, const float* sin_t,
                          int dtype, void* stream);
+int mh_attn_bwd_o_scaled_dots(const void* qkv, const void* o, const void* dout, const float* lse, float* delta, void* dqkv,
+                              const float* rowscale, float* dots, int64_t B, int64_t S, int H, float scale, const float* cos_t,
+                              const float* sin_t, int dtype, void* stream);
 int mh_attn_fwd_timeline(const void* qkv, void* o, float* lse, int64_t B, int64_t S, int H, float scale, int lazy,
                          uint32_t* stamps, void* stream);
 int mh_attn_fwd_plain(const void* qkv, void* o, float* lse, int64_t B, int64_t S, int H, float scale, int dtype,
@@ -123,6 +133,8 @@
                    const float* sin_t, int dtype, void* stream);
 int mh_tokattn_bwd_scaled(const void* qkv, const void* dout, void* dqkv, const float* rowscale, int64_t N, int T, int H, float scale,
                           const float* cos_t, const float* sin_t, int dtype, void* stream);
+int mh_tokattn_bwd_scaled_dots(const void* qkv, const void* dout, void* dqkv, const float* rowscale, float* dots, int64_t N, int T,
+                               int H, float scale, const float* cos_t, const float* sin_t, int dtype, void* stream);
 
 int mh_swiglu_fwd(const void* gu, void* a, int64_t M, int I, int dtype, void* stream);
 int mh_swiglu_bwd(const void* gu, const void* da, void* dgu, int64_t M, int I, int dtype, void* stream);
diff --git a/midi-model_amd/csrc/attention_mfma3.hip b/midi-model_amd/csrc/attention_mfma3.hip
--- a/midi-model_amd/csrc/attention_mfma3.hip
+++ b/midi-model_amd/csrc/attention_mfma3.hip
@@ -9,6 +9,7 @@
 thread_local int g_attn_v3 = attn_env_int("MH_ATTN_V3", 255);
 thread_local int g_attn_passes = attn_env_int("MH_ATTN_PASSES", 5);
 thread_local int g_attn_v3_wps = attn_env_int("MH_ATTN_V3_WPS", 0);
+thread_local float* g_attn_bwd_dots = nullptr;
 thread_local const float* g_attn_bwd_rowscale = nullptr;
 
 __device__ inline bf16x8 ldsv(const char* p) { return *reinterpret_cast<const bf16x8*>(p); }
@@ -453,7 +454,8 @@
                                                               const float* __restrict__ sin_t,
                                                               const bf16* __restrict__ o_ ,
                                                               float* __restrict__ delta_w,
-                                                              const float* __restrict__ rowscale ) {
+                                                              const float* __restrict__ rowscale ,
+                                                              float* __restrict__ dots ) {
   extern __shared__ __attribute__((aligned(16))) char smem[];
   constexpr int NT = TR ? 2 : 3;
   const int tid = threadIdx.x, lane = tid & 63;
@@ -572,7 +574,12 @@
   if (qrow < S) {
     bf16* orow = dqkv + (b * S + qrow) * D3 + (int64_t)h * HD;
     const float rsc = rowscale != nullptr ? rowscale[b * S + qrow] : 1.f;
-    store_grad_row(orow, dqacc, -scale * rsc, hi, cos_t, sin_t, qrow);
+    const bf16* yrow = dots != nullptr ? qkv + (b * S + qrow) * D3 + (int64_t)h * HD : nullptr;
+    float d = store_grad_row(orow, dqacc, -scale * rsc, hi, cos_t, sin_t, qrow, yrow);
+    if (dots != nullptr) {
+      d += __shfl_xor(d, 32, 64);
+      if (hi == 0) dots[(int64_t)h * (BH / H) * S + b * S + qrow] = d;
+    }
   }
 }
 
@@ -681,7 +688,8 @@
                                                                bf16* __restrict__ dqkv, int S, int Sp, int H, float scale,
                                                                int BH, int nkt, const float* __restrict__ cos_t,
                                                                const float* __restrict__ sin_t,
-                                                               const float* __restrict__ rowscale ) {
+                                                               const float* __restrict__ rowscale ,
+                                                               float* __restrict__ dots ) {
   constexpr int NT = TR ? 2 : 4, STG = NT * TILE64 + 2048;
   extern __shared__ __attribute__((aligned(16))) char smem[];
   const int tid = threadIdx.x, lane = tid & 63;
@@ -791,8 +799,13 @@
   if (krow < S) {
     bf16* krow_out = dqkv + (b * S + krow) * D3 + D + (int64_t)h * HD;
     const float rsc = rowscale != nullptr ? rowscale[b * S + krow] : 1.f;
-    store_grad_row(krow_out, dkacc, -scale * rsc, hi, cos_t, sin_t, krow);
-    store_grad_row(krow_out + D, dvacc, rsc, hi, nullptr, nullptr, 0);
+    const bf16* yrow = dots != nullptr ? qkv + (b * S + krow) * D3 + D + (int64_t)h * HD : nullptr;
+    float d = store_grad_row(krow_out, dkacc, -scale * rsc, hi, cos_t, sin_t, krow, yrow);
+    d += store_grad_row(krow_out + D, dvacc, rsc, hi, nullptr, nullptr, 0, yrow != nullptr ? yrow + D : nullptr);
+    if (dots != nullptr) {
+      d += __shfl_xor(d, 32, 64);
+      if (hi == 0) dots[(int64_t)(H + h) * (BH / H) * S + b * S + krow] = d;
+    }
   }
 }
 
@@ -873,7 +886,7 @@
   attn_bwd_dq3_kernel<WPS, TR_><<<grid, 256, (TR_ ? 4 : 6) * TILE64, st>>>((const bf16*)qkv, (const bf16*)dout, lse, delta,     \
                                                                         (const bf16*)kt, (bf16*)dqkv, (int)S, (int)Sp, H, scale, \
                                                                         BH, nt, cos_t, sin_t, (const bf16*)o,         \
-                                                                        const_cast<float*>(delta), g_attn_bwd_rowscale)
+                                                                        const_cast<float*>(delta), g_attn_bwd_rowscale, g_attn_bwd_dots)
   if (which & 2) {
     if (g_attn_v3_wps == 2) {
       if (tr) MH_DQ(2, true); else MH_DQ(2, false);
@@ -888,15 +901,15 @@
       attn_bwd_dkv3_kernel<true, true><<<grid, 256, 2 * (2 * TILE64 + 2048), st>>>((const bf16*)qkv, (const bf16*)dout,
                                                                                  delta + (int64_t)BH0 * Sp, delta, nullptr, nullptr,
                                                                                  (bf16*)dqkv, (int)S, (int)Sp, H, scale, BH, nt,
-                                                                                 cos_t, sin_t, g_attn_bwd_rowscale);
+                                                                                 cos_t, sin_t, g_attn_bwd_rowscale, g_attn_bwd_dots);
     else if (tr)
       attn_bwd_dkv3_kernel<true><<<grid, 256, 2 * (2 * TILE64 + 2048), st>>>((const bf16*)qkv, (const bf16*)dout, lse, delta, nullptr,
                                                                            nullptr, (bf16*)dqkv, (int)S, (int)Sp, H, scale, BH, nt,
-                                                                           cos_t, sin_t, g_attn_bwd_rowscale);
+                                                                           cos_t, sin_t, g_attn_bwd_rowscale, g_attn_bwd_dots);
     else
       attn_bwd_dkv3_kernel<false><<<grid, 256, 2 * DKV_STAGE, st>>>((const bf16*)qkv, (const bf16*)dout, lse, delta, (const bf16*)qt,
                                                                   (const bf16*)dot, (bf16*)dqkv, (int)S, (int)Sp, H, scale, BH, nt,
-                                                                  cos_t, sin_t, g_attn_bwd_rowscale);
+                                                                  cos_t, sin_t, g_attn_bwd_rowscale, g_attn_bwd_dots);
     MH_LAUNCH_CHECK();
   }
   return MH_OK;
diff --git a/midi-model_amd/csrc/attention_small.hip b/midi-model_amd/csrc/attention_small.hip
--- a/midi-model_amd/csrc/attention_small.hip
+++ b/midi-model_amd/csrc/attention_small.hip
@@ -162,11 +162,12 @@
   }
 }
 
-template <typename T, int TN, bool BR>
+template <typename T, int TN, bool BR, bool DOTS = false>
 __global__ __launch_bounds__(256) void tokattn_bwd_kernel(const T* __restrict__ qkv, const T* __restrict__ dout,
                                                           T* __restrict__ dqkv, int64_t NH, int Tn, int H, float scale,
                                                           const float* __restrict__ cos_t, const float* __restrict__ sin_t,
-                                                          const float* __restrict__ rowscale ) {
+                                                          const float* __restrict__ rowscale ,
+                                                          float* __restrict__ dots = nullptr) {
   const int lane = threadIdx.x & 63;
   const int64_t D = (int64_t)H * 256, D3 = 3 * D;
   __shared__ float rope_c[TK * 128], rope_s[TK * 128];
@@ -185,6 +186,7 @@
     const T* base = qkv + n * Tn * D3 + off;
     T* ob = dqkv + n * Tn * D3 + off;
     float k[TK][4], v[TK][4], dk[TK][4], dv[TK][4];
+    float rd[DOTS ? TK : 1];
     RawRow<T> qraw[TN ? TN : 1], doraw[TN ? TN : 1];
     const float rs_lane = (rowscale != nullptr && lane < Tn) ? rowscale[n * Tn + lane] : 1.f;
 #pragma unroll
@@ -285,6 +287,7 @@
           dv[j][e] += p[j] * dO[e];
         }
       }
+      if constexpr (DOTS) rd[i] = dq[0] * q[0] + dq[1] * q[1] + dq[2] * q[2] + dq[3] * q[3];
       if (rot) rope_row<T>(dq, rope_c, rope_s, i, lane, -1.f, false);
       if (rowscale != nullptr) {
         const float rsc = __shfl(rs_lane, i, 64);
@@ -296,6 +299,11 @@
 #pragma unroll
     for (int t = 0; t < TK; ++t) {
       if (TN ? t < TN : t < Tn) {
+        if constexpr (DOTS) {
+#pragma unroll
+          for (int e = 0; e < 4; ++e) rd[t] += dk[t][e] * k[t][e] + dv[t][e] * v[t][e];
+          rd[t] *= __shfl(rs_lane, t, 64);
+        }
         if (rot) rope_row<T>(dk[t], rope_c, rope_s, t, lane, -1.f, false);
         if (rowscale != nullptr) {
           const float rsc = __shfl(rs_lane, t, 64);
@@ -307,6 +315,22 @@
         }
         stp<T>(ob + t * D3 + D, lane, dk[t]);
         stp<T>(ob + t * D3 + 2 * D, lane, dv[t]);
+      } else if constexpr (DOTS) {
+        rd[t] = 0.f;
+      }
+    }
+    if constexpr (DOTS) {
+      float* dp = dots + (int64_t)h * (NH / H) * Tn + n * Tn;
+#pragma unroll
+      for (int t = 0; t < TK; t += 4) {
+        const float r4 = wave_sum4(rd[t], rd[t + 1], rd[t + 2], rd[t + 3]);
+        const float s0 = wave_sum4_get<0>(r4), s1 = wave_sum4_get<1>(r4), s2 = wave_sum4_get<2>(r4), s3 = wave_sum4_get<3>(r4);
+        if (lane == 0) {
+          if (t < Tn) dp[t] = s0;
+          if (t + 1 < Tn) dp[t + 1] = s1;
+          if (t + 2 < Tn) dp[t + 2] = s2;
+          if (t + 3 < Tn) dp[t + 3] = s3;
+        }
       }
     }
   }
@@ -330,11 +354,24 @@
 
 thread_local int g_tokattn_bwd_batched = 1;
 static int tokattn_bwd_any(const void* qkv, const void* dout, void* dqkv, const float* rowscale, int64_t N, int Tn, int H, float scale,
-                           const float* cos_t, const float* sin_t, int dtype, void* stream) {
+                           const float* cos_t, const float* sin_t, int dtype, void* stream, float* dots = nullptr) {
   MH_REQUIRE(N > 0 && Tn >= 1 && Tn <= TK && H >= 1, "tokattn_bwd: bad shape");
   const int64_t NH = N * H;
   int64_t g = (NH + 3) / 4;
   if (g > 32768) g = 32768;
+  if (dots != nullptr) {
+    if (Tn == TK && g_tokattn_bwd_batched)
+      DISPATCH_T(dtype, (tokattn_bwd_kernel<T, TK, true, true><<<(int)g, 256, 0, (hipStream_t)stream>>>(
+                            (const T*)qkv, (const T*)dout, (T*)dqkv, NH, Tn, H, scale, cos_t, sin_t, rowscale, dots)));
+    else if (Tn == TK)
+      DISPATCH_T(dtype, (tokattn_bwd_kernel<T, TK, false, true><<<(int)g, 256, 0, (hipStream_t)stream>>>(
+                            (const T*)qkv, (const T*)dout, (T*)dqkv, NH, Tn, H, scale, cos_t, sin_t, rowscale, dots)));
+    else
+      DISPATCH_T(dtype, (tokattn_bwd_kernel<T, 0, false, true><<<(int)g, 256, 0, (hipStream_t)stream>>>(
+                            (const T*)qkv, (const T*)dout, (T*)dqkv, NH, Tn, H, scale, cos_t, sin_t, rowscale, dots)));
+    MH_LAUNCH_CHECK();
+    return MH_OK;
+  }
   if (Tn == TK && g_tokattn_bwd_batched)
     DISPATCH_T(dtype, (tokattn_bwd_kernel<T, TK, true><<<(int)g, 256, 0, (hipStream_t)stream>>>(
                           (const T*)qkv, (const T*)dout, (T*)dqkv, NH, Tn, H, scale, cos_t, sin_t, rowscale)));
@@ -355,6 +392,11 @@
                                      float scale, const float* cos_t, const float* sin_t, int dtype, void* stream) {
   MH_REQUIRE(rowscale != nullptr, "tokattn_bwd_scaled: rowscale is NULL");
   return tokattn_bwd_any(qkv, dout, dqkv, rowscale, N, Tn, H, scale, cos_t, sin_t, dtype, stream);
+}
+extern "C" int mh_tokattn_bwd_scaled_dots(const void* qkv, const void* dout, void* dqkv, const float* rowscale, float* dots, int64_t N,
+                                          int Tn, int H, float scale, const float* cos_t, const float* sin_t, int dtype, void* stream) {
+  MH_REQUIRE(rowscale != nullptr && dots != nullptr, "tokattn_bwd_scaled_dots: rowscale or dots is NULL");
+  return tokattn_bwd_any(qkv, dout, dqkv, rowscale, N, Tn, H, scale, cos_t, sin_t, dtype, stream, dots);
 }
 
 template <typename T>
@@ -1112,6 +1154,7 @@
 }
 
 extern thread_local const float* g_attn_bwd_rowscale;
+extern thread_local float* g_attn_bwd_dots;
 extern thread_local int g_attn_v3;
 extern "C" int mh_attn_bwd_o_scaled(const void* qkv, const void* o, const void* dout, const float* lse, float* delta, void* dqkv,
                                     const float* rowscale, int64_t B, int64_t S, int H, float scale, const float* cos_t,
@@ -1123,6 +1166,15 @@
   g_attn_bwd_rowscale = nullptr;
   return rc;
 }
+extern "C" int mh_attn_bwd_o_scaled_dots(const void* qkv, const void* o, const void* dout, const float* lse, float* delta, void* dqkv,
+                                         const float* rowscale, float* dots, int64_t B, int64_t S, int H, float scale,
+                                         const float* cos_t, const float* sin_t, int dtype, void* stream) {
+  MH_REQUIRE(dots != nullptr, "attn_bwd_o_scaled_dots: dots is NULL");
+  g_attn_bwd_dots = dots;
+  const int rc = mh_attn_bwd_o_scaled(qkv, o, dout, lse, delta, dqkv, rowscale, B, S, H, scale, cos_t, sin_t, dtype, stream);
+  g_attn_bwd_dots = nullptr;
+  return rc;
+}
 
 extern "C" int mh_attn_bwd_o(const void* qkv, const void* o, const void* dout, const float* lse, float* delta, void* dqkv,
                              int64_t B, int64_t S, int H, float scale, const float* cos_t, const float* sin_t, int dtype,
diff --git a/midi-model_amd/csrc/attn_mfma_common.h b/midi-model_amd/csrc/attn_mfma_common.h
--- a/midi-model_amd/csrc/attn_mfma_common.h
+++ b/midi-model_amd/csrc/attn_mfma_common.h
@@ -102,8 +102,9 @@
     }
 }
 
-__device__ inline void store_grad_row(bf16* orow, const f32x16 (&acc)[2], float scale, int hi, const float* cos_t,
-                                      const float* sin_t, int pos) {
+__device__ inline float store_grad_row(bf16* orow, const f32x16 (&acc)[2], float scale, int hi, const float* cos_t,
+                                       const float* sin_t, int pos, const bf16* yrow = nullptr) {
+  float dot = 0.f;
 #pragma unroll
   for (int r8 = 0; r8 < 2; ++r8) {
     bf16x8 v0, v1;
@@ -111,6 +112,12 @@
     for (int e = 0; e < 8; ++e) {
       v0[e] = (bf16)(acc[0][8 * r8 + e] * scale);
       v1[e] = (bf16)(acc[1][8 * r8 + e] * scale);
+    }
+    if (yrow != nullptr) {
+      const bf16x8 y0 = *reinterpret_cast<const bf16x8*>(yrow + 16 * r8 + 8 * hi);
+      const bf16x8 y1 = *reinterpret_cast<const bf16x8*>(yrow + 32 + 16 * r8 + 8 * hi);
+#pragma unroll
+      for (int e = 0; e < 8; ++e) dot += (float)v0[e] * (float)y0[e] + (float)v1[e] * (float)y1[e];
     }
     if (cos_t != nullptr) {
       const int i0 = 16 * r8 + 8 * hi;
@@ -127,6 +134,7 @@
     *reinterpret_cast<bf16x8*>(orow + 16 * r8 + 8 * hi) = v0;
     *reinterpret_cast<bf16x8*>(orow + 32 + 16 * r8 + 8 * hi) = v1;
   }
+  return dot;
 }
 
 __device__ inline bool attn_work(int& BH, int ntile, int& bh, int& tile) {
diff --git a/midi-model_amd/csrc/elementwise.hip b/midi-model_amd/csrc/elementwise.hip
--- a/midi-model_amd/csrc/elementwise.hip
+++ b/midi-model_amd/csrc/elementwise.hip
@@ -565,6 +565,28 @@
   return MH_OK;
 }
 
+__global__ __launch_bounds__(256) void norm_coef_kernel(const float* __restrict__ dots, int nslots, const float* __restrict__ rstd,
+                                                        int64_t M, float inv_d, float* __restrict__ coef) {
+  __shared__ float acc[4][64];
+  const int r = threadIdx.x & 63, q = threadIdx.x >> 6;
+  const int64_t m = (int64_t)blockIdx.x * 64 + r;
+  float s = 0.f;
+  if (m < M) {
+#pragma unroll 4
+    for (int p = q; p < nslots; p += 4) s += dots[(int64_t)p * M + m];
+  }
+  acc[q][r] = s;
+  __syncthreads();
+  if (q == 0 && m < M) coef[m] = (acc[0][r] + acc[1][r] + acc[2][r] + acc[3][r]) * rstd[m] * inv_d;
+}
+extern "C" int mh_norm_coef(const float* dots, int nslots, const float* rstd, int64_t M, int D, float* coef, void* stream) {
+  MH_REQUIRE(M > 0 && D > 0 && nslots > 0 && dots != nullptr && rstd != nullptr && coef != nullptr, "norm_coef: bad arguments M=%ld D=%d nslots=%d",
+             (long)M, D, nslots);
+  norm_coef_kernel<<<(unsigned)((M + 63) / 64), 256, 0, (hipStream_t)stream>>>(dots, nslots, rstd, M, 1.0f / (float)D, coef);
+  MH_LAUNCH_CHECK();
+  return MH_OK;
+}
+
 constexpr int RMS_BWD_MAX_BLOCKS = 1024;
 extern "C" int mh_rmsnorm_bwd_blocks(int64_t M) {
   int64_t g = (M + 3) / 4;
diff --git a/midi-model_amd/csrc/gemm.hip b/midi-model_amd/csrc/gemm.hip
--- a/midi-model_amd/csrc/gemm.hip
+++ b/midi-model_amd/csrc/gemm.hip
@@ -326,7 +326,11 @@
 }
 
 int mh_gemm_pp256_dswiglu_bf16(const void* A, int64_t lda, const void* B, int64_t ldb, const void* GU, int64_t ldgu,
-                               void* DGU, int64_t lddgu, int64_t M, int64_t I, int64_t K, hipStream_t st, const float* rowscale);
+                               void* DGU, int64_t lddgu, int64_t M, int64_t I, int64_t K, hipStream_t st, const float* rowscale,
+                               float* dots);
+int mh_gemm_pp256_normbwd_bf16(const void* A, int64_t lda, const void* B, int64_t ldb, const void* X, int64_t ldx, const void* DRES,
+                               int64_t lddres, const float* coef, void* DX, int64_t lddx, int64_t M, int64_t N, int64_t K,
+                               hipStream_t st);
 int mh_gemm_pp256_scaled_bf16(const void* A, int64_t lda, const void* B, int64_t ldb, void* C, int64_t ldc, int64_t M, int64_t N,
                               int64_t K, const float* rowscale, hipStream_t st);
 
@@ -417,12 +421,26 @@
                  lddgu >= 2 * I,
              "gemm_dswiglu: leading dimensions must be multiples of 8 elements and cover the rows");
   MH_REQUIRE((((uintptr_t)A | (uintptr_t)B | (uintptr_t)GU | (uintptr_t)DGU) & 15) == 0, "gemm_dswiglu: 16-byte alignment");
-  return mh_gemm_pp256_dswiglu_bf16(A, lda, B, ldb, GU, ldgu, DGU, lddgu, M, I, K, (hipStream_t)stream, nullptr);
-}
-
+  return mh_gemm_pp256_dswiglu_bf16(A, lda, B, ldb, GU, ldgu, DGU, lddgu, M, I, K, (hipStream_t)stream, nullptr, nullptr);
+}
+
+static int gemm_dswiglu_scaled_any(const void* A, int64_t lda, const void* B, int64_t ldb, const void* GU, int64_t ldgu, void* DGU,
+                                   int64_t lddgu, const float* rowscale, float* dots, int64_t M, int64_t I, int64_t K, int dtype,
+                                   void* stream);
 extern "C" int mh_gemm_dswiglu_scaled(const void* A, int64_t lda, const void* B, int64_t ldb, const void* GU, int64_t ldgu,
                                       void* DGU, int64_t lddgu, const float* rowscale, int64_t M, int64_t I, int64_t K, int dtype,
                                       void* stream) {
+  return gemm_dswiglu_scaled_any(A, lda, B, ldb, GU, ldgu, DGU, lddgu, rowscale, nullptr, M, I, K, dtype, stream);
+}
+extern "C" int mh_gemm_dswiglu_scaled_dots(const void* A, int64_t lda, const void* B, int64_t ldb, const void* GU, int64_t ldgu,
+                                           void* DGU, int64_t lddgu, const float* rowscale, float* dots, int64_t M, int64_t I,
+                                           int64_t K, int dtype, void* stream) {
+  MH_REQUIRE(dots != nullptr, "gemm_dswiglu_scaled_dots: dots is NULL");
+  return gemm_dswiglu_scaled_any(A, lda, B, ldb, GU, ldgu, DGU, lddgu, rowscale, dots, M, I, K, dtype, stream);
+}
+static int gemm_dswiglu_scaled_any(const void* A, int64_t lda, const void* B, int64_t ldb, const void* GU, int64_t ldgu, void* DGU,
+                                   int64_t lddgu, const float* rowscale, float* dots, int64_t M, int64_t I, int64_t K, int dtype,
+                                   void* stream) {
   MH_REQUIRE(dtype == MH_BF16 && g_mh_gemm_variant != 0, "gemm_dswiglu_scaled: served by the production bf16 kernel only");
   MH_REQUIRE(rowscale != nullptr && ((uintptr_t)rowscale & 15) == 0, "gemm_dswiglu_scaled: rowscale must be a 16-byte aligned fp32 [M]");
   MH_REQUIRE(M > 0 && I > 0 && K > 0 && I % 8 == 0, "gemm_dswiglu_scaled: bad shape M=%ld I=%ld K=%ld", (long)M, (long)I, (long)K);
@@ -430,7 +448,22 @@
                  lddgu >= 2 * I,
              "gemm_dswiglu_scaled: leading dimensions must be multiples of 8 elements and cover the rows");
   MH_REQUIRE((((uintptr_t)A | (uintptr_t)B | (uintptr_t)GU | (uintptr_t)DGU) & 15) == 0, "gemm_dswiglu_scaled: 16-byte alignment");
-  return mh_gemm_pp256_dswiglu_bf16(A, lda, B, ldb, GU, ldgu, DGU, lddgu, M, I, K, (hipStream_t)stream, rowscale);
+  return mh_gemm_pp256_dswiglu_bf16(A, lda, B, ldb, GU, ldgu, DGU, lddgu, M, I, K, (hipStream_t)stream, rowscale, dots);
+}
+
+extern "C" int mh_gemm_normbwd(const void* dz, int64_t lddz, const void* W, int64_t ldw, const void* x, int64_t ldx,
+                               const void* dres, int64_t lddres, const float* coef, void* dx, int64_t lddx, int64_t M, int64_t N,
+                               int64_t K, int dtype, void* stream) {
+  MH_REQUIRE(dtype == MH_BF16 && g_mh_gemm_variant != 0, "gemm_normbwd: served by the production bf16 kernel only");
+  MH_REQUIRE(M > 0 && N > 0 && K > 0 && dz != nullptr && W != nullptr && x != nullptr && dres != nullptr && dx != nullptr,
+             "gemm_normbwd: bad arguments M=%ld N=%ld K=%ld", (long)M, (long)N, (long)K);
+  MH_REQUIRE(coef != nullptr && ((uintptr_t)coef & 15) == 0, "gemm_normbwd: coef must be a 16-byte aligned fp32 [M]");
+  MH_REQUIRE(lddz % 8 == 0 && ldw % 8 == 0 && ldx % 8 == 0 && lddres % 8 == 0 && lddx % 8 == 0 && lddz >= K && ldw >= N &&
+                 ldx >= N && lddres >= N && lddx >= N,
+             "gemm_normbwd: leading dimensions must be multiples of 8 elements and cover the rows");
+  MH_REQUIRE((((uintptr_t)dz | (uintptr_t)W | (uintptr_t)x | (uintptr_t)dres | (uintptr_t)dx) & 15) == 0, "gemm_normbwd: 16-byte alignment");
+  MH_REQUIRE(((M + 255) / 256) * ((N + 255) / 256) < (1ll << 30), "gemm_normbwd: too many tiles");
+  return mh_gemm_pp256_normbwd_bf16(dz, lddz, W, ldw, x, ldx, dres, lddres, coef, dx, lddx, M, N, K, (hipStream_t)stream);
 }
 
 extern "C" int mh_gemm_nt_scaled(const void* A, int64_t lda, const void* B, int64_t ldb, void* C, int64_t ldc,
diff --git a/midi-model_amd/csrc/gemm_pp256.hip b/midi-model_amd/csrc/gemm_pp256.hip
--- a/midi-model_amd/csrc/gemm_pp256.hip
+++ b/midi-model_amd/csrc/gemm_pp256.hip
@@ -100,6 +100,24 @@
   } x;
   x.u = v;
   return x.b;
+}
+
+__device__ inline float dot8_bf16(const bf16x8& a, const bf16x8& b, float s) {
+  union {
+    bf16x8 v8;
+    bf16x2 h[4];
+  } ua, ub;
+  ua.v8 = a;
+  ub.v8 = b;
+#pragma unroll
+  for (int e = 0; e < 4; ++e) s = __builtin_amdgcn_fdot2_f32_bf16(ua.h[e], ub.h[e], s, false);
+  return s;
+}
+__device__ inline float line_sum8(float s) {
+  s += dpp_move<0xB1>(s);
+  s += dpp_move<0x4E>(s);
+  s += dpp_move<0x141>(s);
+  return s;
 }
 
 constexpr int P8_REGION = 128 * 128;
@@ -321,15 +339,17 @@
   }
 }
 
-template <bool TA, bool TB, int ABL, int EPI, int ML, int NRM>
+template <bool TA, bool TB, int ABL, int EPI, int ML, int NRM, int DOT = 0>
 __global__ __launch_bounds__(512, 2) void gemm_pp256_kernel(const bf16* __restrict__ A, int64_t lda,
                                                             const bf16* __restrict__ B, int64_t ldb, bf16* C, int64_t ldc,
                                                             const bf16* R, int64_t ldr, int64_t M, int64_t N, int64_t K,
                                                             float alpha, float beta, int tiles_n, int nwg,
                                                             int64_t k_per_split, float* __restrict__ ws,
-                                                            const void* __restrict__ zero16, float* aux, int lean_epi) {
-  static_assert(NRM == 0 || (ML == 1 && ABL == 0 && !TA && (!TB || (EPI == 1 && NRM == 2))), "the norm forms ride on the K-step-64 loops only");
-  static_assert(NRM != 1 || EPI == 0, "sum-of-squares partials come out of the plain epilogue");
+                                                            const void* __restrict__ zero16, float* aux, int lean_epi,
+                                                            float* __restrict__ aux2, const bf16* __restrict__ X2, int64_t ldx2) {
+  static_assert(NRM == 0 || (ML == 1 && ABL == 0 && !TA && (!TB || (EPI == 1 && NRM == 2) || NRM == 3)), "the norm forms ride on the K-step-64 loops only");
+  static_assert((NRM != 1 && NRM != 3) || EPI == 0, "sum-of-squares partials and the norm backward come out of the plain epilogue");
+  static_assert(DOT == 0 || EPI == 1, "row-dot partials come out of the SwiGLU-backward epilogue");
   extern __shared__ __attribute__((aligned(16))) char smem[];
   const int tid = threadIdx.x, lane = tid & 63;
   const int wave = __builtin_amdgcn_readfirstlane(tid >> 6);
@@ -361,7 +381,7 @@
   };
 
   if constexpr (ML >= 1) {
-    if constexpr (NRM == 2) {
+    if constexpr (NRM == 2 || NRM == 3) {
       if (wave == 0) {
         const int64_t r = m0 + lane * 4;
         glds16((r + 4 <= M) ? (const void*)(aux + r) : zero16, smem + LDS_BYTES);
@@ -477,10 +497,12 @@
       const unsigned vo_r = (unsigned)(((grp * 128 + lrow) * (int)ldr + c * 8) * 2), so_r = (unsigned)ldr * 16u;
       const unsigned vo_c = (unsigned)(((grp * 128 + lrow) * (int)ldc + c * 8) * 2), so_c = (unsigned)ldc * 16u;
       const unsigned up_off = (unsigned)N * 2u;
+      float* dotp = nullptr;
+      if constexpr (DOT) dotp = aux2 + ((n0 + wn * 64) >> 6) * M + m0 + grp * 128 + lrow;
       bf16x8 gq[2][8], uq[2][8];
-      auto request = [&](int half, int i0) {
-#pragma unroll
-        for (int i = i0; i < i0 + 4; ++i) {
+      auto request = [&](int half, int i0, int n = 4) {
+#pragma unroll
+        for (int i = i0; i < i0 + n; ++i) {
           gq[half][i] = as_bf16x8(__builtin_amdgcn_raw_buffer_load_b128(rg, vo_r, (unsigned)(half * 8 + i) * so_r, 0));
           uq[half][i] = as_bf16x8(__builtin_amdgcn_raw_buffer_load_b128(rg, vo_r, (unsigned)(half * 8 + i) * so_r + up_off, 0));
         }
@@ -500,7 +522,12 @@
           }
 #pragma unroll
         for (int i = 0; i < 8; ++i) {
-          if (half == 0 && (i == 2 || i == 6)) request(1, i == 2 ? 0 : 4);
+          if constexpr (DOT) {
+            if (half == 0 && (i == 3 || i == 5 || i == 7)) request(1, i - 3, 2);
+            if (half == 1 && i == 0) request(1, 6, 2);
+          } else {
+            if (half == 0 && (i == 2 || i == 6)) request(1, i == 2 ? 0 : 4);
+          }
           const int row = i * 8 + lrow;
           const f32x4 lo = *reinterpret_cast<const f32x4*>(wreg + row * 256 + (((2 * c) ^ (row & 15)) << 4));
           const f32x4 hi = *reinterpret_cast<const f32x4*>(wreg + row * 256 + (((2 * c + 1) ^ (row & 15)) << 4));
@@ -511,8 +538,13 @@
           expand8_bf16(uq[half][i], u);
           mh_dswiglu8(dv, g, u, dg, du);
           const unsigned so = (unsigned)(half * 8 + i) * so_c;
-          tile_store(as_u32x4(cvt8_bf16(dg)), rc, vo_c + so, 2 );
-          tile_store(as_u32x4(cvt8_bf16(du)), rc, vo_c + so + up_off, 2);
+          const bf16x8 og = cvt8_bf16(dg), ou = cvt8_bf16(du);
+          tile_store(as_u32x4(og), rc, vo_c + so, 2 );
+          tile_store(as_u32x4(ou), rc, vo_c + so + up_off, 2);
+          if constexpr (DOT) {
+            const float d = line_sum8(dot8_bf16(ou, uq[half][i], dot8_bf16(og, gq[half][i], 0.f)));
+            if (c == 0) dotp[half * 64 + i * 8] = d;
+          }
         }
       }
       return;
@@ -569,6 +601,10 @@
         const bf16x8 og = cvt8_bf16(dg), ou = cvt8_bf16(du);
         __builtin_nontemporal_store(og, reinterpret_cast<bf16x8*>(C + m * ldc + n));
         __builtin_nontemporal_store(ou, reinterpret_cast<bf16x8*>(C + m * ldc + N + n));
+        if constexpr (DOT) {
+          const float d = line_sum8(dot8_bf16(ou, uv[i], dot8_bf16(og, gv[i], 0.f)));
+          if (c == 0) aux2[((n0 + wn * 64) >> 6) * M + m] = d;
+        }
       }
     }
     return;
@@ -815,6 +851,56 @@
         }
         if (m >= M || n + 8 > N) continue;
         __builtin_nontemporal_store(cvt8_bf16(v), reinterpret_cast<bf16x8*>(C + m * ldc + n));
+      }
+    }
+    return;
+  }
+  if constexpr (NRM == 3) {
+    const int64_t nw = n0 + wn * 64;
+    if (nw >= N) return;
+    char* wreg = smem + wave * 16384;
+    const int lrow = lane >> 3, c = lane & 7;
+    const int64_t rows_left = (M - m0 < QBM) ? M - m0 : QBM;
+    const __amdgpu_buffer_rsrc_t rc = tile_rsrc(C + m0 * ldc + nw, ((rows_left - 1) * ldc + 64) * 2);
+    const __amdgpu_buffer_rsrc_t rr = tile_rsrc(R + m0 * ldr + nw, ((rows_left - 1) * ldr + 64) * 2);
+    const __amdgpu_buffer_rsrc_t rx = tile_rsrc(X2 + m0 * ldx2 + nw, ((rows_left - 1) * ldx2 + 64) * 2);
+    const unsigned vo_c = (unsigned)(((grp * 128 + lrow) * (int)ldc + c * 8) * 2), so_c = (unsigned)ldc * 16u;
+    const unsigned vo_r = (unsigned)(((grp * 128 + lrow) * (int)ldr + c * 8) * 2), so_r = (unsigned)ldr * 16u;
+    const unsigned vo_x = (unsigned)(((grp * 128 + lrow) * (int)ldx2 + c * 8) * 2), so_x = (unsigned)ldx2 * 16u;
+    const float* cl = reinterpret_cast<const float*>(smem + LDS_BYTES) + grp * 128 + lrow;
+    bf16x8 rq[2][8], xq[2][8];
+    auto request = [&](int half, int i0) {
+#pragma unroll
+      for (int i = i0; i < i0 + 4; ++i) {
+        rq[half][i] = as_bf16x8(__builtin_amdgcn_raw_buffer_load_b128(rr, vo_r, (unsigned)(half * 8 + i) * so_r, 0));
+        xq[half][i] = as_bf16x8(__builtin_amdgcn_raw_buffer_load_b128(rx, vo_x, (unsigned)(half * 8 + i) * so_x, 0));
+      }
+    };
+    request(0, 0);
+    request(0, 4);
+#pragma unroll
+    for (int half = 0; half < 2; ++half) {
+#pragma unroll
+      for (int fmh = 0; fmh < 4; ++fmh)
+#pragma unroll
+        for (int fn = 0; fn < 4; ++fn) {
+          const int row = fmh * 16 + fi, ch = fn * 4 + fg;
+          *reinterpret_cast<f32x4*>(wreg + row * 256 + ((ch ^ (row & 15)) << 4)) = acc[fn][half * 4 + fmh];
+        }
+#pragma unroll
+      for (int i = 0; i < 8; ++i) {
+        if (half == 0 && (i == 2 || i == 6)) request(1, i == 2 ? 0 : 4);
+        const int row = i * 8 + lrow;
+        const f32x4 lo = *reinterpret_cast<const f32x4*>(wreg + row * 256 + (((2 * c) ^ (row & 15)) << 4));
+        const f32x4 hi = *reinterpret_cast<const f32x4*>(wreg + row * 256 + (((2 * c + 1) ^ (row & 15)) << 4));
+        const float ncf = -cl[half * 64 + i * 8];
+        float v[8] = {lo[0], lo[1], lo[2], lo[3], hi[0], hi[1], hi[2], hi[3]};
+        float xf[8], rf[8];
+        expand8_bf16(xq[half][i], xf);
+        expand8_bf16(rq[half][i], rf);
+#pragma unroll
+        for (int e = 0; e < 8; ++e) v[e] = __builtin_fmaf(ncf, xf[e], v[e]) + rf[e];
+        tile_store(as_u32x4(cvt8_bf16(v)), rc, vo_c + (unsigned)(half * 8 + i) * so_c, 2 );
       }
     }
     return;
@@ -1010,11 +1096,11 @@
 }
 extern thread_local int g_mh_gemm_lean_epi;
 namespace {
-template <bool TA, bool TB, int ABL, int EPI = 0, int ML = 0, int NRM = 0>
+template <bool TA, bool TB, int ABL, int EPI = 0, int ML = 0, int NRM = 0, int DOT = 0>
 int launch_one(const void* A, int64_t lda, const void* B, int64_t ldb, void* C, int64_t ldc, const void* R, int64_t ldr,
                int64_t M, int64_t N, int64_t K, float alpha, float beta, int splitk, void* workspace, hipStream_t st,
-               float* aux = nullptr) {
-  constexpr int LDSB = LDS_BYTES + ((ABL & 128) ? P8_DBG_BYTES : 0) + (NRM == 2 ? 1024 : 0);
+               float* aux = nullptr, float* aux2 = nullptr, const void* X2 = nullptr, int64_t ldx2 = 0) {
+  constexpr int LDSB = LDS_BYTES + ((ABL & 128) ? P8_DBG_BYTES : 0) + ((NRM == 2 || NRM == 3) ? 1024 : 0);
   constexpr int MAX_DEV = 64;
   static void* zero16_of[MAX_DEV] = {};
   static bool attr_set_of[MAX_DEV] = {};
@@ -1032,7 +1118,7 @@
     __atomic_store_n(&zero16_of[dev], zero16, __ATOMIC_RELEASE);
   }
   if (!__atomic_load_n(&attr_set_of[dev], __ATOMIC_ACQUIRE)) {
-    hipError_t e = hipFuncSetAttribute(reinterpret_cast<const void*>(&gemm_pp256_kernel<TA, TB, ABL, EPI, ML, NRM>),
+    hipError_t e = hipFuncSetAttribute(reinterpret_cast<const void*>(&gemm_pp256_kernel<TA, TB, ABL, EPI, ML, NRM, DOT>),
                                        hipFuncAttributeMaxDynamicSharedMemorySize, LDSB);
     if (e != hipSuccess) {
       mh_set_error("gemm_pp256: cannot raise dynamic LDS to %d bytes: %s", LDSB, hipGetErrorString(e));
@@ -1045,9 +1131,9 @@
   constexpr int KSTEP = (ML == 1) ? 64 : QBK;
   const int64_t kps = ((K + splitk - 1) / splitk + KSTEP - 1) / KSTEP * KSTEP;
   dim3 grid(nwg, 1, splitk);
-  gemm_pp256_kernel<TA, TB, ABL, EPI, ML, NRM><<<grid, 512, LDSB, st>>>((const bf16*)A, lda, (const bf16*)B, ldb, (bf16*)C, ldc,
+  gemm_pp256_kernel<TA, TB, ABL, EPI, ML, NRM, DOT><<<grid, 512, LDSB, st>>>((const bf16*)A, lda, (const bf16*)B, ldb, (bf16*)C, ldc,
                                                           (const bf16*)R, ldr, M, N, K, alpha, beta, (int)tiles_n, nwg, kps,
-                                                          (float*)workspace, zero16, aux, g_mh_gemm_lean_epi);
+                                                          (float*)workspace, zero16, aux, g_mh_gemm_lean_epi, aux2, (const bf16*)X2, ldx2);
   MH_LAUNCH_CHECK();
   return MH_OK;
 }
@@ -1140,9 +1226,16 @@
 }
 
 int mh_gemm_pp256_dswiglu_bf16(const void* A, int64_t lda, const void* B, int64_t ldb, const void* GU, int64_t ldgu,
-                               void* DGU, int64_t lddgu, int64_t M, int64_t I, int64_t K, hipStream_t st, const float* rowscale) {
+                               void* DGU, int64_t lddgu, int64_t M, int64_t I, int64_t K, hipStream_t st, const float* rowscale,
+                               float* dots) {
+  MH_REQUIRE(dots == nullptr || rowscale != nullptr, "gemm_dswiglu: row-dot partials come with the row-scaled form");
   if (rowscale != nullptr) {
     MH_REQUIRE(g_mh_gemm_k64 == 1 && M % 4 == 0, "gemm_dswiglu_scaled: needs the K-step-64 dgrad loop and M %% 4 == 0");
+    if (dots != nullptr) {
+      MH_REQUIRE(I % 64 == 0, "gemm_dswiglu_scaled_dots: I = %ld must be a multiple of 64 (one partial per 64 columns)", (long)I);
+      return launch_one<false, true, 0, 1, 1, 2, 1>(A, lda, B, ldb, DGU, lddgu, GU, ldgu, M, I, K, 1.f, 0.f, 1, nullptr, st,
+                                                    const_cast<float*>(rowscale), dots);
+    }
     return launch_one<false, true, 0, 1, 1, 2>(A, lda, B, ldb, DGU, lddgu, GU, ldgu, M, I, K, 1.f, 0.f, 1, nullptr, st,
                                                const_cast<float*>(rowscale));
   }
@@ -1155,3 +1248,12 @@
   MH_REQUIRE(g_mh_gemm_k64 != 0, "gemm_rowss: needs the K-step-64 main loop (option gemm_k64)");
   return launch_one<false, false, 0, 0, 1, 1>(A, lda, B, ldb, C, ldc, R, ldr, M, N, K, 1.f, R ? 1.f : 0.f, 1, nullptr, st, rowss);
 }
+
+int mh_gemm_pp256_normbwd_bf16(const void* A, int64_t lda, const void* B, int64_t ldb, const void* X, int64_t ldx, const void* DRES,
+                               int64_t lddres, const float* coef, void* DX, int64_t lddx, int64_t M, int64_t N, int64_t K,
+                               hipStream_t st) {
+  MH_REQUIRE(g_mh_gemm_k64 == 1 && M % 4 == 0 && N % 64 == 0, "gemm_normbwd: needs the K-step-64 dgrad loop, M %% 4 == 0 and N %% 64 == 0");
+  MH_REQUIRE(ldx < (1 << 22) && lddres < (1 << 22) && lddx < (1 << 22), "gemm_normbwd: row strides beyond 2^22 elements are not supported (32-bit tile offsets)");
+  return launch_one<false, true, 0, 0, 1, 3>(A, lda, B, ldb, DX, lddx, DRES, lddres, M, N, K, 1.f, 1.f, 1, nullptr, st,
+                                             const_cast<float*>(coef), nullptr, X, ldx);
+}
diff --git a/midi-model_amd/engine.py b/midi-model_amd/engine.py
--- a/midi-model_amd/engine.py
+++ b/midi-model_amd/engine.py
@@ -8,7 +8,7 @@
 
 import torch
 
-from . import ops
+from . import norm_bwd, ops
 
 
 @dataclass
@@ -279,6 +279,8 @@
     M, D = dx.shape
     H, I = spec.H, spec.I
     wq_n, wgu_n = fold
+    if dx.is_cuda and train_fold_ok(spec, dx) and norm_bwd.fused_ok(dx, D, I):
+        return _layer_backward_folded_fused(spec, lw, lg, fold, keep, dx, nseq, slen, rope, accumulate)
     a = keep.a
     if a is None:
         a = _empty((M, I), dx)
@@ -306,6 +308,37 @@
     ops.wgrad_folded(dz1, keep.x, lg.wqkv, lw.n1, lw.wqkv, lg.n1, accumulate)
     del dz1
     ops.rmsnorm_bwd_folded(keep.x, keep.rstd1, t1, dx2, dx)
+    return dx
+
+
+def _layer_backward_folded_fused(spec: StackSpec, lw: LayerTensors, lg: LayerTensors, fold, keep: LayerSaved, dx: torch.Tensor,
+                                 nseq: int, slen: int, rope: RopeTable, accumulate: bool) -> torch.Tensor:
+    M, D = dx.shape
+    H, I = spec.H, spec.I
+    wq_n, wgu_n = fold
+    a = keep.a
+    if a is None:
+        a = _empty((M, I), dx)
+        ops.swiglu_fwd(keep.gu, a)
+    dz2 = _empty((M, 2 * I), dx)
+    dots = norm_bwd.gemm_dswiglu_dots(dx, lw.wd, keep.gu, dz2, keep.rstd2)
+    linear_wgrad(dx, a, lg.wd, accumulate)
+    del a
+    dx2 = _empty((M, D), dx)
+    norm_bwd.gemm_normbwd(dz2, wgu_n, keep.x2, dx, norm_bwd.norm_coef(dots, keep.rstd2, D), dx2)
+    ops.wgrad_folded(dz2, keep.x2, lg.wgu, lw.n2, lw.wgu, lg.n2, accumulate)
+    del dz2, dots
+    do = _empty((M, D), dx)
+    ops.gemm_nt(dx2, lw.wo, do, tb=True)
+    linear_wgrad(dx2, keep.o, lg.wo, accumulate)
+    dz1 = _empty((M, 3 * D), dx)
+    if spec.kind == "event":
+        dots = norm_bwd.attn_bwd_dots(keep.qkv, keep.o, do, keep.lse, dz1, nseq, slen, H, spec.scale, rope.cos, rope.sin, keep.rstd1)
+    else:
+        dots = norm_bwd.tokattn_bwd_dots(keep.qkv, do, dz1, nseq, slen, H, spec.scale, rope.cos, rope.sin, keep.rstd1)
+    del do
+    norm_bwd.gemm_normbwd(dz1, wq_n, keep.x, dx2, norm_bwd.norm_coef(dots, keep.rstd1, D), dx)
+    ops.wgrad_folded(dz1, keep.x, lg.wqkv, lw.n1, lw.wqkv, lg.n1, accumulate)
     return dx
 
 
diff --git a/midi-model_amd/norm_bwd.py b/midi-model_amd/norm_bwd.py
--- /dev/null
+++ b/midi-model_amd/norm_bwd.py
@@ -0,0 +1,79 @@
+from __future__ import annotations
+
+import os
+
+import torch
+
+from . import ops
+from .lib import lib
+from .ops import _p, _rowmajor, _stream, dt
+
+
+def fused_ok(x: torch.Tensor, D: int, I: int) -> bool:
+    return (x.is_cuda and x.dtype == torch.bfloat16 and D % 64 == 0 and I % 64 == 0 and x.shape[0] % 4 == 0
+            and os.environ.get("MH_NORM_BWD_FUSED", "1") != "0")
+
+
+def _dots(slots: int, like: torch.Tensor) -> torch.Tensor:
+    return torch.empty((slots, like.shape[0]), dtype=torch.float32, device=like.device)
+
+
+def gemm_dswiglu_dots(dx: torch.Tensor, wd: torch.Tensor, gu: torch.Tensor, dgu: torch.Tensor, rowscale: torch.Tensor) -> torch.Tensor:
+    M, K = dx.shape
+    I = wd.shape[1]
+    assert wd.shape[0] == K and gu.shape == (M, 2 * I) and dgu.shape == (M, 2 * I) and dx.dtype == wd.dtype == gu.dtype and I % 64 == 0
+    assert rowscale.shape == (M,) and rowscale.dtype == torch.float32 and rowscale.is_contiguous()
+    dots = _dots(I // 64, dx)
+    prof = ops.gemm_profile
+    if prof is not None:
+        e0, e1 = torch.cuda.Event(enable_timing=True), torch.cuda.Event(enable_timing=True)
+        e0.record()
+    lib().call("mh_gemm_dswiglu_scaled_dots", _p(dx), _rowmajor(dx), _p(wd), _rowmajor(wd), _p(gu), _rowmajor(gu), _p(dgu),
+               _rowmajor(dgu), _p(rowscale), _p(dots), M, I, K, dt(dx), _stream())
+    if prof is not None:
+        e1.record()
+        prof.append((e0, e1, 2.0 * M * I * K, (M, I, K, 1, 0, 1, "+dswiglu")))
+    return dots
+
+
+def attn_bwd_dots(qkv, o, dout, lse, dqkv, B: int, S: int, H: int, scale: float, cos_t, sin_t, rowscale) -> torch.Tensor:
+    assert ops.attn_bwd_scaled_ok(qkv) and rowscale.shape == (B * S,) and rowscale.dtype == torch.float32 and rowscale.is_contiguous()
+    delta = torch.empty((2 * B * H * ops.round_up(S, 64),), dtype=torch.float32, device=qkv.device)
+    dots = _dots(2 * H, dqkv)
+    lib().call("mh_attn_bwd_o_scaled_dots", _p(qkv), _p(o), _p(dout), _p(lse), _p(delta), _p(dqkv), _p(rowscale), _p(dots), B, S, H,
+               scale, _p(cos_t), _p(sin_t), dt(qkv), _stream())
+    return dots
+
+
+def tokattn_bwd_dots(qkv, dout, dqkv, N: int, T: int, H: int, scale: float, cos_t, sin_t, rowscale) -> torch.Tensor:
+    assert rowscale.shape == (N * T,) and rowscale.dtype == torch.float32 and rowscale.is_contiguous()
+    dots = _dots(H, dqkv)
+    lib().call("mh_tokattn_bwd_scaled_dots", _p(qkv), _p(dout), _p(dqkv), _p(rowscale), _p(dots), N, T, H, scale, _p(cos_t),
+               _p(sin_t), dt(qkv), _stream())
+    return dots
+
+
+def norm_coef(dots: torch.Tensor, rstd: torch.Tensor, D: int) -> torch.Tensor:
+    M = rstd.shape[0]
+    assert dots.shape[1] == M and dots.dtype == rstd.dtype == torch.float32 and dots.is_contiguous() and rstd.is_contiguous()
+    coef = torch.empty_like(rstd)
+    lib().call("mh_norm_coef", _p(dots), dots.shape[0], _p(rstd), M, D, _p(coef), _stream())
+    return coef
+
+
+def gemm_normbwd(dz: torch.Tensor, w: torch.Tensor, x: torch.Tensor, dres: torch.Tensor, coef: torch.Tensor, dx: torch.Tensor):
+    M, D = dx.shape
+    K = dz.shape[1]
+    assert dz.shape[0] == M and w.shape == (K, D) and x.shape == (M, D) and dres.shape == (M, D)
+    assert dz.dtype == w.dtype == x.dtype == dres.dtype == dx.dtype and coef.shape == (M,) and coef.dtype == torch.float32
+    assert coef.is_contiguous() and dx.data_ptr() != x.data_ptr() and dx.data_ptr() != dres.data_ptr()
+    prof = ops.gemm_profile
+    if prof is not None:
+        e0, e1 = torch.cuda.Event(enable_timing=True), torch.cuda.Event(enable_timing=True)
+        e0.record()
+    lib().call("mh_gemm_normbwd", _p(dz), _rowmajor(dz), _p(w), _rowmajor(w), _p(x), _rowmajor(x), _p(dres), _rowmajor(dres),
+               _p(coef), _p(dx), _rowmajor(dx), M, D, K, dt(dx), _stream())
+    if prof is not None:
+        e1.record()
+        prof.append((e0, e1, 2.0 * M * D * K, (M, D, K, 1, 0, 1, "+normbwd")))
+    return dx
```

New measurement: 356,500 events/s. Within noise of the previous version (-0.8%).
